# nghiant03/spine-vision

Hardware: AMD Instinct MI355X
Metric: images/sec training, ConvNeXt-base 512x512 loc, bs32, at 1/2/4/8 MI355X (higher is better)
Workload: dtype bf16; 1 GPU; CoordinateRegressor(convnext_base) localization train step fwd+bwd+allreduce+clip+AdamW; image_size=512, batch_per_gpu=32, global_batch=32, parallelism=dp1, hip_graph=False

## Files before the change

include/sv_kernels.h:

```cpp
#ifndef SV_KERNELS_H
#define SV_KERNELS_H

#include <stdint.h>

#ifdef __cplusplus
extern "C" {
#endif

typedef struct ihipStream_t* sv_stream_t;

typedef enum { SV_F32 = 0, SV_BF16 = 1 } sv_dtype;

typedef enum {
  SV_OK = 0,
  SV_ERR_INVALID_ARG = 1,
  SV_ERR_UNSUPPORTED = 2,
  SV_ERR_LAUNCH = 3
} sv_status;

int sv_version(void);
const char* sv_last_error_string(void);
const char* sv_build_target(void);

typedef struct sv_ctx sv_ctx;
typedef struct sv_ctx_info {
  int32_t device;
  int32_t compute_units;
  int32_t lds_bytes_per_wg;
  int32_t xcds;
  int32_t lds_raised_kernels;
  int32_t refs;
  char arch[32];
} sv_ctx_info;
int sv_ctx_create(int32_t device, sv_ctx** out);
int sv_ctx_destroy(sv_ctx* ctx);
int sv_ctx_get_info(const sv_ctx* ctx, sv_ctx_info* out);

int sv_stream_create_cu_reserved(int32_t device, const int32_t* reserved, int32_t n_reserved, sv_stream_t* out);

typedef enum {
  SV_EPI_STORE = 0,
  SV_EPI_BIAS_GELU2 = 1,
  SV_EPI_BIAS_GAMMA_RES = 2,
  SV_EPI_GELU_GRAD = 3,
  SV_EPI_SLAB = 4,
  SV_EPI_BIAS_GELU_DUAL = 5,
  SV_EPI_MUL_AUX = 6,
  SV_EPI_BIAS_GELU = 7,
  SV_EPI_STORE_STATS = 8,
  SV_EPI_STORE_BN_BWD = 9,
  SV_EPI_LN_BWD = 10
} sv_epilogue;

typedef struct {
  const float* mean;
  const float* rstd;
  const float* gamma;
  const float* beta;
} sv_bn_ref;

typedef struct {
  int32_t impl;
  int32_t grid_cap;
  int32_t wg_per_cu;
  int32_t priority;
} sv_gemm_policy;

typedef struct {
  int32_t M, N, K;
  const void* A; int32_t a_dtype; int32_t a_kmajor; int64_t lda;
  const void* B; int32_t b_dtype; int32_t b_kmajor; int64_t ldb;
  const float* a_scale_k;
  int32_t epilogue;
  void* C; int32_t c_dtype; int64_t ldc;
  void* C2; int32_t c2_dtype;
  const float* bias;
  const float* gamma;
  const void* aux; int32_t aux_dtype; int64_t ld_aux;
  int32_t split_k;
  int32_t compute;
  const sv_bn_ref* bn;
  sv_gemm_policy policy;
  float* fold_out; int64_t fold_ld; int32_t fold_accumulate; int32_t* fold_counters;
} sv_gemm_desc;

int sv_gemm(const sv_gemm_desc* d, sv_stream_t stream);
int sv_gemm_slab_finish(const float* slab, int32_t split, int32_t M, int32_t N, void* C, int32_t c_dtype, int64_t ldc,
                        int32_t accumulate, float* stats, sv_stream_t stream);
int sv_gemm_slab_finish_bn_bwd(const float* slab, int32_t split, int32_t M, int32_t N, void* C, const void* y,
                               const sv_bn_ref* bn, float* part, sv_stream_t stream);

int sv_mlp_fwd(const uint16_t* y, const uint16_t* w1, const float* b1, const uint16_t* w2, const float* b2,
               const float* gamma, const float* x, float* x_out, uint16_t* gelu_grad, uint16_t* gelu_out, int64_t M,
               int32_t C, sv_stream_t stream);

int sv_mlp_bwd_nparts(int64_t M, int32_t C);
int sv_mlp_bwd(const uint16_t* d, const uint16_t* w2t, const uint16_t* gelu_grad, const uint16_t* w1t, const uint16_t* z,
               const float* mean, const float* rstd, const float* lnw, uint16_t* dh, uint16_t* dz, float* ln_part,
               int64_t M, int32_t C, sv_stream_t stream);

int sv_layernorm_fwd(const void* x, int32_t x_dtype, const float* w, const float* b, void* y,
                     int32_t y_dtype, float* mean, float* rstd, int64_t rows, int32_t C, float eps,
                     sv_stream_t stream);
int sv_layernorm_bwd_nparts(int64_t rows, int32_t C);
int sv_layernorm_bwd(const void* dy, int32_t dy_dtype, const void* x, int32_t x_dtype, const float* mean,
                     const float* rstd, const float* w, void* dx, int32_t dx_dtype, int32_t accumulate,
                     float* dw_part, float* db_part, int64_t rows, int32_t C, sv_stream_t stream);

int sv_grn_nparts(int64_t HW, int32_t n);
int sv_grn_stats(const void* a, int32_t dtype, float* part, int32_t B, int64_t HW, int32_t n, sv_stream_t stream);
int sv_grn_finish(const float* part, int32_t nparts, const float* gamma, float* G, float* N, float* scale, float* D,
                  int32_t B, int32_t n, float eps, sv_stream_t stream);
int sv_grn_apply(const void* a, int32_t dtype, const float* scale, const float* beta, void* u, int32_t B, int64_t HW,
                 int32_t n, sv_stream_t stream);
int sv_grn_bwd_stats(const void* du, const void* a, int32_t dtype, float* s_part, float* d_part, int32_t B,
                     int64_t HW, int32_t n, sv_stream_t stream);
int sv_grn_bwd_finish(float* s_part, float* d_part, int32_t nparts, const float* gamma, const float* G,
                      const float* N, const float* D, float* k, float* dgamma, float* dbeta, int32_t accumulate,
                      int32_t B, int32_t n, sv_stream_t stream);
int sv_grn_bwd_apply(const void* du, const void* a, const void* gh, int32_t dtype, const float* scale, const float* k,
                     void* dh, int32_t B, int64_t HW, int32_t n, sv_stream_t stream);

int sv_dwconv7_ln_fwd(const void* x, int32_t x_dtype, const float* wdw, const float* bdw,
                      const float* lnw, const float* lnb, float eps, void* z, int32_t z_dtype, void* y,
                      int32_t y_dtype, float* mean, float* rstd, int32_t B, int32_t H, int32_t W,
                      int32_t C, sv_stream_t stream);
int sv_diag_group_sum(const float* in, float* xlane, float* shuffle, int64_t n, int32_t lanes, sv_stream_t stream);
int sv_dwconv7_ln_fused_ok(int32_t B, int32_t H, int32_t W, int32_t C, int32_t x_dtype, int32_t z_dtype,
                           int32_t y_dtype);
int sv_dwconv7_bwd_data(const void* dz, int32_t dz_dtype, const float* wdw, float* dx, uint16_t* dx_bf16,
                        int32_t accumulate, int32_t B, int32_t H, int32_t W, int32_t C, sv_stream_t stream);
int sv_dwconv7_bwd_weight_nparts(int32_t B, int32_t H, int32_t W, int32_t C);
int sv_dwconv7_bwd_weight(const void* dz, int32_t dz_dtype, const void* x, int32_t x_dtype, float* dw_part,
                          float* db_part, int32_t B, int32_t H, int32_t W, int32_t C,
                          sv_stream_t stream);

int sv_dwconv7_fwd_mfma(const void* x, int32_t x_dtype, const float* wdw, const float* bdw, uint16_t* z, int32_t B,
                        int32_t H, int32_t W, int32_t C, sv_stream_t stream);
int sv_dwconv7_bwd_data_mfma(const uint16_t* dz, const float* wdw, float* dx, uint16_t* dx_bf16, int32_t accumulate,
                             int32_t B, int32_t H, int32_t W, int32_t C, sv_stream_t stream);
int sv_dwconv7_bwd_weight_mfma_nparts(int32_t B, int32_t H, int32_t W, int32_t C);
int sv_dwconv7_bwd_weight_mfma(const uint16_t* dz, const void* x, int32_t x_dtype, float* dw_part, float* db_part,
                               int32_t B, int32_t H, int32_t W, int32_t C, sv_stream_t stream);

int sv_stem_patchify_ln_fwd(const float* img, const float* w, const float* b, const float* lnw,
                            const float* lnb, float eps, void* y, int32_t y_dtype, float* mean,
                            float* rstd, int32_t B, int32_t H, int32_t W, int32_t C,
                            sv_stream_t stream);
int sv_stem_patchify_ln_bwd_nparts(int32_t B, int32_t H, int32_t W, int32_t C);
int sv_stem_patchify_ln_bwd(const float* img, const float* w, const float* b, const float* lnw,
                            const float* mean, const float* rstd, const float* dy, float* dw_part,
                            float* db_part, float* dlnw_part, float* dlnb_part, int32_t B, int32_t H,
                            int32_t W, int32_t C, sv_stream_t stream);

typedef enum { SV_IMG_F32_NCHW = 0, SV_IMG_U8_GRAY = 1, SV_IMG_U8_HWC = 2  } sv_image_kind;
int sv_stem_patchify(const void* img, int32_t img_kind, const float* norm_mean, const float* norm_std,
                     uint16_t* patches, int32_t B, int32_t H, int32_t W, sv_stream_t stream);
int sv_stem_weight_pack(const float* w, uint16_t* wpack, int32_t C, sv_stream_t stream);
int sv_normalize_u8_gray(const uint8_t* img, const float* norm_mean, const float* norm_std, float* out,
                         int32_t B, int32_t H, int32_t W, sv_stream_t stream);

int sv_augment_u8(const uint8_t* in, uint8_t* out, int32_t B, int32_t H, int32_t W, int32_t C, const double* params,
                  int32_t* row_sums, sv_stream_t stream);

int sv_resize_u8(const uint8_t* src, const int64_t* desc, const int32_t* coef, int32_t B, int32_t H, int32_t W,
                 int32_t C, uint8_t* dst, sv_stream_t stream);

int sv_downsample_ln_patch2_fwd(const float* x, const float* lnw, const float* lnb, float eps,
                                void* patches, int32_t p_dtype, float* mean, float* rstd, int32_t B,
                                int32_t H, int32_t W, int32_t C, sv_stream_t stream);
int sv_downsample_ln_patch2_bwd_nparts(int32_t B, int32_t H, int32_t W, int32_t C);
int sv_downsample_ln_patch2_bwd(const float* dpatches, const float* x, const float* mean,
                                const float* rstd, const float* lnw, float* dx, uint16_t* dx_bf16, float* dlnw_part,
                                float* dlnb_part, int32_t B, int32_t H, int32_t W, int32_t C,
                                sv_stream_t stream);

int sv_pool_ln_fwd(const float* x, const float* lnw, const float* lnb, float eps, float* pooled,
                   float* feat, float* mean, float* rstd, int32_t B, int32_t HW, int32_t C,
                   sv_stream_t stream);
int sv_pool_ln_bwd(const float* dfeat, const float* pooled, const float* mean, const float* rstd,
                   const float* lnw, float* dx, uint16_t* dx_bf16, float* dlnw_part, float* dlnb_part, int32_t B,
                   int32_t HW, int32_t C, sv_stream_t stream);

#define SV_MAX_RED_SEGS 8
typedef struct {
  const float* part;
  float* out;
  int64_t n;
  int32_t P;
  int32_t accumulate;
} sv_red_seg;
int sv_reduce_partials_multi(const sv_red_seg* segs, int32_t nseg, float alpha, sv_stream_t stream);

int sv_reduce_partials_pair(const float* part_a, int64_t n_a, float* out_a, const float* part_b, int64_t n_b,
                            float* out_b, int32_t P, float alpha, int32_t accumulate, sv_stream_t stream);
int sv_reduce_partials(const float* part, int32_t P, int32_t group, int64_t n, float* out, float alpha,
                       int32_t accumulate, sv_stream_t stream);
int sv_reduce_partials_bf16(const uint16_t* part, int32_t P, int64_t n, float* out, float alpha, int32_t accumulate,
                            sv_stream_t stream);
int sv_colsum_nparts(int64_t rows, int32_t C);
int sv_colsum(const void* x, int32_t x_dtype, int64_t rows, int32_t C, float* part,
              sv_stream_t stream);
int sv_layerscale_wgrad_finish(const float* G, const float* cs, const float* W2, const float* gamma,
                               const float* b2, float* dW2, float* dgamma, float* db2, int32_t C,
                               int32_t K4, sv_stream_t stream);

int sv_layerscale_wgrad_reduce_ws(int32_t C, int32_t K4);
int sv_layerscale_wgrad_reduce(const float* slab, const float* cs_part, int32_t P, const float* W2,
                               const float* gamma, const float* b2, float* dW2, float* dgamma, float* db2,
                               float* ws, int32_t C, int32_t K4, sv_stream_t stream);
int sv_layerscale_wgrad_reduce_bf16(const uint16_t* slab, const float* cs_part, int32_t P, const float* W2,
                                    const float* gamma, const float* b2, float* dW2, float* dgamma, float* db2, int32_t C,
                                    int32_t K4, sv_stream_t stream);
int sv_layerscale_wgrad_fold_finish(const float* G, const float* cs_part, int32_t P, const float* W2, const float* gamma,
                                    const float* b2, float* dW2, float* dgamma, float* db2, int32_t C, int32_t K4,
                                    sv_stream_t stream);

int sv_sqnorm_nparts(int64_t n);
int sv_sqnorm_partial(const float* g, int64_t n, float* part, sv_stream_t stream);
int sv_clip_coef(const float* part, int32_t nparts, float max_norm, float* out, sv_stream_t stream);
int sv_adamw_flat(float* p, const float* g, float* m, float* v, uint16_t* p_bf16, int64_t n,
                  float lr, float beta1, float beta2, float eps, float weight_decay, int32_t step,
                  const float* grad_scale, sv_stream_t stream);
int sv_adamw_flat_dev(float* p, const float* g, float* m, float* v, uint16_t* p_bf16, int64_t n, float beta1,
                      float beta2, float eps, float weight_decay, const float* hyper, const float* grad_scale,
                      sv_stream_t stream);
int sv_transpose_scale_bf16(const float* W, const float* scale, uint16_t* out, int32_t rows, int32_t cols,
                            sv_stream_t stream);
int sv_scale_rows_bf16(const float* W, const float* scale, uint16_t* out, int32_t rows, int32_t cols,
                       sv_stream_t stream);
int sv_cast_f32_bf16(const float* x, uint16_t* y, int64_t n, sv_stream_t stream);

typedef struct sv_conv_shape {
  int32_t B, H, W, Cs;
  int32_t Cout;
  int32_t KH, KW, stride, pad;
  int32_t Cin;
} sv_conv_shape;
int sv_conv_weight_pack(const float* w, void* wp, int32_t dtype, const sv_conv_shape* s, sv_stream_t stream);
// ... 259 lines not shown
```

spine-vision_amd/backbone/convnext.py:

```python

from __future__ import annotations

import os
from dataclasses import dataclass, field
from typing import Callable

import torch
import torch.nn as nn

from .. import kernels as K
from .. import native as nv
from ._explicit import ExplicitBackward

CONVNEXT_CFGS = {
    "convnext_tiny": ((3, 3, 9, 3), (96, 192, 384, 768)),
    "convnext_small": ((3, 3, 27, 3), (96, 192, 384, 768)),
    "convnext_base": ((3, 3, 27, 3), (128, 256, 512, 1024)),
    "convnext_large": ((3, 3, 27, 3), (192, 384, 768, 1536)),
    "convnextv2_base": ((3, 3, 27, 3), (128, 256, 512, 1024)),
    "convnextv2_large": ((3, 3, 27, 3), (192, 384, 768, 1536)),
}


def _comm_cap(device, reserve: int) -> int:
# ... 28 lines not shown


class _GrnMlp(nn.Module):
    def __init__(self, dim: int, hidden: int) -> None:
        super().__init__()
        self.fc1 = nn.Linear(dim, hidden)
        self.grn = _Grn(hidden)
        self.fc2 = nn.Linear(hidden, dim)


class ConvNeXtV2Block(nn.Module):

    def __init__(self, dim: int) -> None:
        super().__init__()
        self.conv_dw = nn.Conv2d(dim, dim, kernel_size=7, padding=3, groups=dim, bias=True)
        self.norm = nn.LayerNorm(dim, eps=1e-6)
        self.mlp = _GrnMlp(dim, 4 * dim)


class ConvNeXtStage(nn.Module):
    def __init__(self, in_chs: int, out_chs: int, depth: int, downsample: bool, block=ConvNeXtBlock) -> None:
        super().__init__()
        if downsample:
            self.downsample = nn.Sequential(nn.LayerNorm(in_chs, eps=1e-6), nn.Conv2d(in_chs, out_chs, 2, stride=2))
        else:
            self.downsample = nn.Identity()
        self.blocks = nn.Sequential(*[block(out_chs) for _ in range(depth)])


class _Head(nn.Module):
    def __init__(self, dim: int) -> None:
        super().__init__()
        self.norm = nn.LayerNorm(dim, eps=1e-6)


@dataclass
class _Tape:

    img: torch.Tensor
    stem: tuple = ()
    stages: list = field(default_factory=list)
    pool: tuple = ()
    out_shape: tuple = ()
    wcache: dict = field(default_factory=dict)
    w2g: dict = field(default_factory=dict)
    wt: dict = field(default_factory=dict)
    w2g_ready: object = None


class _ConvNeXtFn(torch.autograd.Function):
    @staticmethod
    def forward(ctx, x, anchor, model):
        feat, tape = model._forward_impl(x, save=True)
        ctx.model = model
        ctx.tape = tape
        return feat

    @staticmethod
    def backward(ctx, dfeat):
        ctx.model._backward_impl(ctx.tape, dfeat)
        ctx.tape = None
        return None, None, None


_TAIL_MAIN = int(os.environ.get("SV_TAIL_MAIN", "0"))


class _WgradSchedule:

    def __init__(self, model, main, side, lean: bool, pol) -> None:
        self.model, self.main, self.side, self.lean, self.pol = model, main, side, lean, pol
        cap = pol.grid_cap
        if model.side_grid_cap is not None:
            cap = min(model.side_grid_cap, cap) if cap > 0 else model.side_grid_cap
        self.spol = nv.policy(impl=model.side_impl, grid_cap=cap, wg_per_cu=pol.wg_per_cu, priority=model.side_prio)
        self.queue: list = []
        self.pending: list = []
        self.tail: list = []

    def _run(self, jobs, pol) -> None:
        for job, ready in jobs:
            job(pol)
            if ready:
                self.model._ready(ready)

    def submit(self, job, operands, ready=None) -> None:
        if self.lean:
            self.queue.append((job, ready))
        elif self.side is None:
            self._run([(job, ready)], self.pol)
        else:
            self.side.wait_event(self.main.record_event())
            for t_ in operands:
                t_.record_stream(self.side)
            with torch.cuda.stream(self.side):
                self._run([(job, ready)], self.spol)

    def handoff(self) -> None:
        if self.lean:
            nv.handoff(self.main, self.side)

    def flush(self, tail: bool) -> None:
        if not self.lean:
            return
        queue, self.queue = self.queue, []
        n = 1 if tail else len(queue)
        with torch.cuda.stream(self.side):
            self._run(queue[:n], self.spol)
            self.pending.append((self.side.record_event(), queue))
        self.tail += queue[n:]

    def run_tail(self) -> None:
        self._run(self.tail, self.pol)
        self.tail.clear()


class ConvNeXtHip(ExplicitBackward, nn.Module):
    def __init__(self, depths=(3, 3, 27, 3), dims=(128, 256, 512, 1024), ls_init_value: float = 1e-6,
                 precision: str = "bf16", use_grn: bool = False) -> None:
        super().__init__()
        if precision not in ("bf16", "fp32"):
            raise ValueError(f"precision must be 'bf16' or 'fp32', got {precision!r}")
        self.depths, self.dims = tuple(depths), tuple(dims)
        self.precision = precision
        self.use_grn = bool(use_grn)
        self.stem = nn.Sequential(nn.Conv2d(3, dims[0], kernel_size=4, stride=4), nn.LayerNorm(dims[0], eps=1e-6))
        stages = []
        prev = dims[0]
        for i, (d, c) in enumerate(zip(depths, dims)):
            stages.append(ConvNeXtStage(prev, c, d, downsample=i > 0,
                                        block=ConvNeXtV2Block if self.use_grn else ConvNeXtBlock))
            prev = c
        self.stages = nn.Sequential(*stages)
        if self.use_grn:
            self.register_buffer("ls_ones", torch.ones(max(dims)), persistent=False)
        self.norm_pre = nn.Identity()
        self.head = _Head(prev)
        self.num_features = self.head_hidden_size = prev
        self.grad_ready_hook: Callable[[list], None] | None = None
        self._shadow: dict[int, torch.Tensor] | None = None
        self.overlap_wgrad = os.environ.get("SV_SIDE_STREAM", "1") != "0"
        self.side_wg_per_cu = 1
        self.lean_sync = os.environ.get("SV_LEAN_SYNC", "1") != "0"
        self._side: dict = {}
        self.graph_safe = False
        self.comm_reserve_cus = 0
        self.comm_cu_mask = False
        self.merge_folds = os.environ.get("SV_MERGED_FOLDS", "1") != "0"
        cap = os.environ.get("SV_SIDE_GRID_CAP")
        self.side_grid_cap: int | None = int(cap) if cap else None
        self.side_impl = int(os.environ.get("SV_WGRAD_IMPL", "0"))
        self.main_bwd_cap = int(os.environ.get("SV_MAIN_BWD_CAP", "0"))
        self.wgrad_target = int(os.environ.get("SV_CNX_WGRAD_WGS", "256"))
        self.side_prio = int(os.environ.get("SV_SIDE_PRIO", "1"))
        self.fused_mlp = os.environ.get("SV_FUSED_MLP", "1") != "0"
        self.fused_mlp_c = tuple(int(c) for c in os.environ.get("SV_FUSED_MLP_C", "128,192,256").split(",") if c)
        self.fused_mlp_bwd = os.environ.get("SV_FUSED_MLP_BWD", "1") != "0"
        self.param_gate = None
        self._init_weights()

    def param_gate_groups(self) -> list[nn.Module]:
        return [self.stem, *self.stages, self.head]

    def _init_weights(self) -> None:
        for m in self.modules():
            if isinstance(m, (nn.Conv2d, nn.Linear)):
                nn.init.trunc_normal_(m.weight, std=0.02)
                if m.bias is not None:
                    nn.init.zeros_(m.bias)

    @property
    def compute_bf16(self) -> bool:
        return self.precision == "bf16"

    @property
    def act_dtype(self) -> torch.dtype:
        return torch.bfloat16 if self.compute_bf16 else torch.float32

    def set_weight_shadow(self, shadow: dict[int, torch.Tensor] | None) -> None:
        self._shadow = shadow

    def gemm_weight_params(self) -> list[nn.Parameter]:
        ps = [self.stem[0].weight]
        for st in self.stages:
            if not isinstance(st.downsample, nn.Identity):
                ps.append(st.downsample[1].weight)
            for blk in st.blocks:
                ps += [blk.mlp.fc1.weight, blk.mlp.fc2.weight]
        return ps

    def _w(self, p: torch.Tensor, cache: dict) -> torch.Tensor:
        if not self.compute_bf16:
            return p.detach()
        if self._shadow is not None and id(p) in self._shadow:
            return self._shadow[id(p)]
        k = id(p)
        if k not in cache:
            cache[k] = K.cast_bf16(p.detach().contiguous())
        return cache[k]

    def forward(self, x: torch.Tensor) -> torch.Tensor:
        if not x.is_cuda:
            raise RuntimeError("ConvNeXtHip runs on the MI355X kernel library only (got a CPU tensor)")
        if x.dtype == torch.uint8:
            x = x.contiguous() if self.compute_bf16 else K.normalize_u8_gray(x.contiguous())
        else:
            x = x.float().contiguous()
        need_grad = torch.is_grad_enabled() and any(p.requires_grad for p in self.parameters())
        if need_grad:
            anchor = torch.zeros((), device=x.device, requires_grad=True)
            return _ConvNeXtFn.apply(x, anchor, self)
        feat, _ = self._forward_impl(x, save=False)
        return feat

    def forward_features(self, x: torch.Tensor) -> torch.Tensor:
        return self.forward(x)

    @torch.no_grad()
    def _forward_impl(self, img: torch.Tensor, save: bool):
        bf = self.compute_bf16
        act = self.act_dtype
        tape = _Tape(img=img) if save else None
        cache: dict = tape.wcache if save else {}
        stem_conv, stem_ln = self.stem[0], self.stem[1]
        gate = self.param_gate
        if gate is not None:
            gate.wait(self.stem)
        if save and bf and self.overlap_wgrad and not self.use_grn:
            main = torch.cuda.current_stream()
            side = self._side_stream(main.device)
            blocks = [blk for st in self.stages for blk in st.blocks]
            fused_b = {id(blk) for blk in blocks if self._fused_bwd(blk)}
            for blk in blocks:
                if id(blk) in fused_b:
                    w1, w2 = blk.mlp.fc1.weight, blk.mlp.fc2.weight
                    tape.wt[id(blk)] = (torch.empty(w2.shape[1], w2.shape[0], device=img.device, dtype=torch.bfloat16),
                                        torch.empty(w1.shape[1], w1.shape[0], device=img.device, dtype=torch.bfloat16))
                else:
                    tape.w2g[id(blk)] = torch.empty(blk.mlp.fc2.weight.shape, device=img.device, dtype=torch.bfloat16)
            side.wait_event(main.record_event())
            if gate is not None:
                gate.wait_all(side)
            with torch.cuda.stream(side):
                for blk in blocks:
                    if id(blk) in fused_b:
                        w2t, w1t = tape.wt[id(blk)]
                        K.transpose_scale_bf16(blk.mlp.fc2.weight.detach(), blk.gamma.detach(), out=w2t)
                        K.transpose_scale_bf16(blk.mlp.fc1.weight.detach(), None, out=w1t)
                    else:
                        K.scale_rows_bf16(blk.mlp.fc2.weight.detach(), blk.gamma.detach(), out=tape.w2g[id(blk)])
            tape.w2g_ready = side.record_event()
        if bf:
            B, H0, W0 = img.shape[0], img.shape[-2], img.shape[-1]
            C0 = stem_conv.weight.shape[0]
            patches = K.stem_patchify(img)
            z0 = torch.empty(patches.shape[0], C0, device=img.device, dtype=act)
            K.linear_fwd(patches, K.stem_weight_pack(stem_conv.weight.detach()), out=z0, bias=stem_conv.bias,
                         compute_bf16=True)
            x2d, s_mean, s_rstd = K.layernorm_fwd(z0, stem_ln.weight, stem_ln.bias, out_dtype=torch.float32)
            x = x2d.view(B, H0 // 4, W0 // 4, C0)
            if save:
                tape.stem = (patches, z0, s_mean, s_rstd)
        else:
            x, s_mean, s_rstd = K.stem_fwd(img, stem_conv.weight, stem_conv.bias, stem_ln.weight, stem_ln.bias)
            if save:
                tape.stem = (s_mean, s_rstd)
        for st in self.stages:
            if gate is not None:
                gate.wait(st)
            ds_saved = None
            if not isinstance(st.downsample, nn.Identity):
                ln, conv = st.downsample[0], st.downsample[1]
                B, H, W, C = x.shape
                patches, d_mean, d_rstd = K.downsample_fwd(x, ln.weight, ln.bias, act_dtype=act)
                Cout = conv.weight.shape[0]
                wds = self._w(conv.weight, cache).reshape(Cout, 4 * C)
                xn = torch.empty(B, H // 2, W // 2, Cout, device=x.device, dtype=torch.float32)
                K.linear_fwd(patches, wds, out=xn.view(-1, Cout), bias=conv.bias, compute_bf16=bf)
                if save:
                    ds_saved = (x, patches, d_mean, d_rstd)
                x = xn
            blocks_saved = []
            for blk in st.blocks:
                B, H, W, C = x.shape
                M = B * H * W
                z, y, mean, rstd = K.dwconv7_ln_fwd(x, blk.conv_dw.weight, blk.conv_dw.bias, blk.norm.weight,
                                                    blk.norm.bias, act_dtype=act, save_z=save)
                w1 = self._w(blk.mlp.fc1.weight, cache)
                w2 = self._w(blk.mlp.fc2.weight, cache)
                if bf and self.fused_mlp and not self.use_grn and C in K.MLP_FUSED_C and C in self.fused_mlp_c:
                    xo = torch.empty(B, H, W, C, device=x.device, dtype=torch.float32)
                    gh = torch.empty(M, 4 * C, device=x.device, dtype=act) if save else None
                    a = torch.empty(M, 4 * C, device=x.device, dtype=act) if save else None
                    K.mlp_fwd(y, w1, blk.mlp.fc1.bias, w2, blk.mlp.fc2.bias, blk.gamma, x.view(M, C), out=xo.view(M, C),
                              gelu_grad=gh, gelu_out=a)
                    if save:
                        blocks_saved.append((x, z, y, mean, rstd, gh, a, None))
                    x = xo
                    continue
                a = torch.empty(M, 4 * C, device=x.device, dtype=act)
                if save:
                    gh = torch.empty(M, 4 * C, device=x.device, dtype=act)
                    K.linear_fwd(y, w1, out=gh, out2=a, bias=blk.mlp.fc1.bias, epilogue=nv.SV_EPI_BIAS_GELU_DUAL,
                                 compute_bf16=bf)
                else:
                    gh = None
                    K.linear_fwd(y, w1, out=a, bias=blk.mlp.fc1.bias, epilogue=nv.SV_EPI_BIAS_GELU,
                                 compute_bf16=bf)
                xo = torch.empty(B, H, W, C, device=x.device, dtype=torch.float32)
                grn_saved = None
                if self.use_grn:
                    grn = blk.mlp.grn
                    u, gst = K.grn_fwd(a, B, grn.weight, grn.bias, inplace=not save)
                    grn_saved = (u, gst)
                    K.linear_fwd(u, w2, out=xo.view(M, C), bias=blk.mlp.fc2.bias, gamma=self.ls_ones[:C],
                                 residual=x.view(M, C), epilogue=nv.SV_EPI_BIAS_GAMMA_RES, compute_bf16=bf)
                else:
                    K.linear_fwd(a, w2, out=xo.view(M, C), bias=blk.mlp.fc2.bias, gamma=blk.gamma,
                                 residual=x.view(M, C), epilogue=nv.SV_EPI_BIAS_GAMMA_RES, compute_bf16=bf)
                if save:
                    blocks_saved.append((x, z, y, mean, rstd, gh, a, grn_saved))
                x = xo
            if save:
                tape.stages.append((ds_saved, blocks_saved))
        if gate is not None:
            gate.wait_all()
        feat, pooled, p_mean, p_rstd = K.pool_ln_fwd(x, self.head.norm.weight, self.head.norm.bias)
        if save:
            tape.pool = (pooled, p_mean, p_rstd)
            tape.out_shape = tuple(x.shape)
            if tape.w2g_ready is not None:
                torch.cuda.current_stream().wait_event(tape.w2g_ready)
                tape.w2g_ready = None
        return feat, tape

    def _fused_bwd(self, blk) -> bool:
        return (self.fused_mlp_bwd and not self.use_grn and self.compute_bf16 and self.overlap_wgrad and self.lean_sync
                and blk.conv_dw.weight.shape[0] in K.MLP_BWD_FUSED_C)

    def _fc2_params(self, blk) -> list:
        if self.use_grn:
            return [blk.mlp.fc2.weight, blk.mlp.fc2.bias, blk.mlp.grn.weight, blk.mlp.grn.bias]
        return [blk.mlp.fc2.weight, blk.mlp.fc2.bias, blk.gamma]

    @staticmethod
    def _rest_params(blk) -> list:
        return [blk.conv_dw.weight, blk.conv_dw.bias, blk.norm.weight, blk.norm.bias, blk.mlp.fc1.weight,
                blk.mlp.fc1.bias]

    def _grn_dgrad(self, blk, dsrc, a, gh, grn_saved, dh, cache, pol) -> None:
        bf = self.compute_bf16
        w2 = self._w(blk.mlp.fc2.weight, cache) if bf else blk.mlp.fc2.weight.detach()
        K.linear_dgrad(dsrc, w2, out=dh, compute_bf16=bf, policy=pol)
        grn, gst = blk.mlp.grn, grn_saved[1]
        K.grn_bwd(dh, a, gh, gst[0].shape[0], grn.weight, gst, dgamma=self._grad(grn.weight),
                  dbeta=self._grad(grn.bias))

    def _block_backward(self, blk, saved, d, db, cache, tape, sched: _WgradSchedule, tail: bool = False):
        bf, act, g = self.compute_bf16, self.act_dtype, self._grad
        main, side, pol = sched.main, sched.side, sched.pol
        x, z, y, mean, rstd, gh, a, grn_saved = saved
        B, H, W, C = x.shape
        M = B * H * W
        fc1, fc2 = blk.mlp.fc1, blk.mlp.fc2
        dsrc = db.view(M, C) if bf else d.view(M, C)
        u = grn_saved[0] if self.use_grn else a
        fc2_ps, rest_ps = self._fc2_params(blk), self._rest_params(blk)
        folds: list | None = [] if self.merge_folds else None

        def fc2_wgrad(policy):
            if self.use_grn:
                K.linear_wgrad(dsrc, u, out=g(fc2.weight), accumulate=True, bias_out=g(fc2.bias), compute_bf16=bf,
                               policy=policy, wgrad_target=self.wgrad_target)
            else:
                K.layerscale_wgrad(dsrc, a, fc2.weight.detach(), blk.gamma.detach(), fc2.bias.detach(),
                                   dw2=g(fc2.weight), dgamma=g(blk.gamma), db2=g(fc2.bias), compute_bf16=bf,
                                   policy=policy, wgrad_target=self.wgrad_target)

        def fc1_wgrad(policy):
            K.linear_wgrad(dh, y, out=g(fc1.weight), accumulate=True, bias_out=g(fc1.bias), compute_bf16=bf,
                           defer=folds, policy=policy, wgrad_target=self.wgrad_target)

        def rest_wgrad(policy):
            ln_finish(record=not sched.lean, defer=folds)
            K.dwconv7_bwd_weight(dz4, x, dw=g(blk.conv_dw.weight), db=g(blk.conv_dw.bias), defer=folds)
            if folds is not None:
                K.reduce_multi(folds)

        sched.submit(fc2_wgrad, (dsrc, u), ready=fc2_ps if tail else None)
        ev_w2 = side.record_event() if side is not None and not bf else None
        dh = torch.empty(M, 4 * C, device=d.device, dtype=act)
        wt = tape.wt.pop(id(blk), None)
        if wt is not None:
            dz = torch.empty(M, C, device=d.device, dtype=torch.bfloat16)
            part, P = K.mlp_bwd(dsrc, wt[0], gh, wt[1], z.view(M, C), mean, rstd, blk.norm.weight, dh=dh, dz=dz)
            dw_ln, db_ln = g(blk.norm.weight), g(blk.norm.bias)

            def ln_finish(record: bool = True, defer: list | None = None):
                if defer is not None:
                    defer += [(part[0], dw_ln, P, True), (part[1], db_ln, P, True)]
                else:
                    K.reduce_pair(part[0], dw_ln, part[1], db_ln, P)
        elif self.use_grn:
            self._grn_dgrad(blk, dsrc, a, gh, grn_saved, dh, cache, pol)
        elif bf:
            w2g = tape.w2g.pop(id(blk), None)
            if w2g is None:
                w2g = K.scale_rows_bf16(fc2.weight.detach(), blk.gamma.detach())
            K.linear_dgrad(dsrc, w2g, out=dh, epilogue=nv.SV_EPI_MUL_AUX, aux=gh, compute_bf16=True, policy=pol)
        else:
            K.linear_dgrad(dsrc, fc2.weight.detach(), out=dh, epilogue=nv.SV_EPI_MUL_AUX, a_scale_k=blk.gamma, aux=gh,
                           compute_bf16=False, policy=pol)
        sched.submit(fc1_wgrad, (dh, y))
        if wt is None:
            w1 = self._w(fc1.weight, cache)
            fused = K.linear_dgrad_ln(dh, w1, z.view(M, C), mean, rstd, blk.norm.weight, dw=g(blk.norm.weight),
                                      db=g(blk.norm.bias), policy=pol) if bf else None
            if fused is not None:
                dz, ln_finish = fused
            else:
                dy = torch.empty(M, C, device=d.device, dtype=act)
                K.linear_dgrad(dh, w1, out=dy, compute_bf16=bf, policy=pol)
                dz, ln_finish = K.layernorm_bwd(dy, z.view(M, C), mean, rstd, blk.norm.weight, dw=g(blk.norm.weight),
                                                db=g(blk.norm.bias), out_dtype=act, defer_reduce=True)
        dz4 = dz.view(B, H, W, C)
        sched.submit(rest_wgrad, (dz, x), ready=rest_ps if tail else rest_ps + fc2_ps)
        sched.handoff()
        if side is not None and bf:
            db = torch.empty_like(db)
        elif side is not None:
            main.wait_event(ev_w2)
        K.dwconv7_bwd_data(dz4, blk.conv_dw.weight, d, accumulate=True, dx_bf16=db)
        sched.flush(tail)
        return d, db

    @torch.no_grad()
    def _backward_impl(self, tape: _Tape, dfeat: torch.Tensor) -> None:
        bf = self.compute_bf16
        cache: dict = tape.wcache
        g = self._grad
        hn = self.head.norm
        main = torch.cuda.current_stream()
        side = self._side_stream(main.device) if self.overlap_wgrad else None
        comm_cap = _comm_cap(main.device, self.comm_reserve_cus)
        if self.main_bwd_cap > 0:
            comm_cap = min(comm_cap, self.main_bwd_cap) if comm_cap > 0 else self.main_bwd_cap
        pol = nv.policy(grid_cap=comm_cap, wg_per_cu=self.side_wg_per_cu if side is not None else 0)
        sched = _WgradSchedule(self, main, side, side is not None and bf and self.lean_sync, pol)
        d, db = K.pool_ln_bwd(dfeat.float(), *tape.pool, hn.weight, tape.out_shape, dlnw=g(hn.weight),
                              dlnb=g(hn.bias), with_bf16=bf)
        if tape.w2g_ready is not None:
            main.wait_event(tape.w2g_ready)
        self._ready([hn.weight, hn.bias])
        for st, (ds_saved, blocks_saved) in zip(reversed(list(self.stages)), reversed(tape.stages)):
            for bi in range(len(blocks_saved) - 1, -1, -1):
                blk, saved = st.blocks[bi], blocks_saved[bi]
                blocks_saved[bi] = None
                tail = sched.lean and _TAIL_MAIN > 0 and st is self.stages[0] and bi == 0
                d, db = self._block_backward(blk, saved, d, db, cache, tape, sched, tail=tail)
                self._release_side(main, sched.pending)
                if _TAIL_MAIN == 2:
                    sched.run_tail()
            if ds_saved is not None:
                x_prev, patches, d_mean, d_rstd = ds_saved
                ln, conv = st.downsample[0], st.downsample[1]
                B, H, W, C = x_prev.shape
                Cout = conv.weight.shape[0]
                Mo = B * (H // 2) * (W // 2)
                dsrc = db.view(Mo, Cout) if bf else d.view(Mo, Cout)
                wds = self._w(conv.weight, cache).reshape(Cout, 4 * C)
                dpatch = torch.empty(Mo, 4 * C, device=d.device, dtype=torch.float32)
                K.linear_dgrad(dsrc, wds, out=dpatch, compute_bf16=bf, policy=pol)
                K.linear_wgrad(dsrc, patches, out=g(conv.weight), accumulate=True, bias_out=g(conv.bias),
                               compute_bf16=bf, policy=pol)
                d, db = K.downsample_bwd(dpatch, x_prev, d_mean, d_rstd, ln.weight, dlnw=g(ln.weight),
                                         dlnb=g(ln.bias), with_bf16=bf)
                self._ready([ln.weight, ln.bias, conv.weight, conv.bias])
        conv, ln = self.stem[0], self.stem[1]
        if bf:
            patches, z0, s_mean, s_rstd = tape.stem
            C0 = conv.weight.shape[0]
            dz0 = K.layernorm_bwd(d.view(-1, C0), z0, s_mean, s_rstd, ln.weight, dw=g(ln.weight), db=g(ln.bias),
                                  out_dtype=torch.bfloat16)
            K.linear_wgrad(dz0, patches, out=g(conv.weight).view(C0, 48), accumulate=True, bias_out=g(conv.bias),
                           compute_bf16=True, cols=48, policy=pol)
        else:
            s_mean, s_rstd = tape.stem
            K.stem_bwd(tape.img, conv.weight, conv.bias, ln.weight, s_mean, s_rstd, d, dw=g(conv.weight),
                       db=g(conv.bias), dlnw=g(ln.weight), dlnb=g(ln.bias))
        sched.run_tail()
        if side is not None:
            main.wait_stream(side)
            sched.pending.clear()
        self._ready([conv.weight, conv.bias, ln.weight, ln.bias])

    _RELEASE_BATCH = int(os.environ.get("SV_RELEASE_BATCH", "4"))

    @classmethod
    def _release_side(cls, main, pending: list) -> None:
        while pending and pending[0][0].query():
            pending.pop(0)
        if len(pending) >= 2 * cls._RELEASE_BATCH:
            main.wait_event(pending[cls._RELEASE_BATCH - 1][0])
            del pending[:cls._RELEASE_BATCH]


def create_convnext(name: str, precision: str = "bf16") -> ConvNeXtHip:
    key = name.split(".")[0]
    if key not in CONVNEXT_CFGS:
        raise ValueError(f"unsupported ConvNeXt variant {name!r}")
    depths, dims = CONVNEXT_CFGS[key]
    return ConvNeXtHip(depths, dims, precision=precision, use_grn=key.startswith("convnextv2"))
```

spine-vision_amd/csrc/gemm.hip:

```cpp
#include "common.h"
#include "gemm_common.h"
#include "mfma_v1.h"

#include <stdlib.h>

namespace sv {


template <bool BF16, typename T, bool KMAJ>
struct Stage {
  static constexpr int EPC = BF16 ? 8 : 4;
  static constexpr int CHUNKS = BM * BKT / EPC;
  static constexpr int PER_THREAD = CHUNKS / kGemmThreads;
  uint4 r[PER_THREAD];

  __device__ __forceinline__ void load(const T* __restrict__ p, int64_t ld, int row0, int k0, int R, int K,
                                       const float* __restrict__ scale) {
#pragma unroll
    for (int s = 0; s < PER_THREAD; ++s) {
      const int q = threadIdx.x + kGemmThreads * s;
      int row, kk;
      if (KMAJ) {
        constexpr int CPR = BKT / EPC;
        row = q / CPR;
// ... 190 lines not shown
  }

  if (do_cs && threadIdx.x < BM && m0 + (int)threadIdx.x < e.M) colsum[(size_t)split * e.M + m0 + threadIdx.x] = csum;

  wave_tile_epilogue(acc, reinterpret_cast<float*>(smem) + wid * 16 * EPI_LD, m0 + wm * 64, n0 + wn * 64, e, split);
}

template <bool BF16, typename TA, typename TB, bool AK, bool BKM>
static int launch(const sv_gemm_desc* d, hipStream_t s) {
  const int tilesM = ceil_div(d->M, BM), tilesN = ceil_div(d->N, BN);
  int split = d->epilogue == SV_EPI_SLAB ? (d->split_k < 1 ? 1 : d->split_k) : 1;
  int kper = ceil_div(ceil_div(d->K, split), BKT) * BKT;
  EpiArgs e{d->M, d->N, d->epilogue, d->C, d->c_dtype, d->ldc, d->C2, d->c2_dtype, d->bias, d->gamma,
            d->aux, d->aux_dtype, d->ld_aux};
  constexpr size_t main_lds = 2 * (size_t)(Img<BF16, AK>::BYTES + Img<BF16, BKM>::BYTES);
  constexpr size_t epi_lds = 4 * 16 * EPI_LD * sizeof(float);
  constexpr size_t lds = main_lds > epi_lds ? main_lds : epi_lds;
  dim3 grid(tilesM * tilesN, 1, split);
  if (const int rc_ = ensure_lds_attr(reinterpret_cast<const void*>(&gemm_kernel<BF16, TA, TB, AK, BKM>), (int)lds, s)) return rc_;
  gemm_kernel<BF16, TA, TB, AK, BKM><<<grid, kGemmThreads, lds, s>>>(
      reinterpret_cast<const TA*>(d->A), d->lda, reinterpret_cast<const TB*>(d->B), d->ldb, d->a_scale_k, d->K,
      kper, tilesM, tilesN, e, d->epilogue == SV_EPI_SLAB ? reinterpret_cast<float*>(d->C2) : nullptr);
  return check_launch("sv_gemm");
}

template <bool BF16, typename TA, typename TB>
static int launch_layout(const sv_gemm_desc* d, hipStream_t s) {
  if (d->a_kmajor && d->b_kmajor) return launch<BF16, TA, TB, true, true>(d, s);
  if (d->a_kmajor && !d->b_kmajor) return launch<BF16, TA, TB, true, false>(d, s);
  if (!d->a_kmajor && d->b_kmajor) return launch<BF16, TA, TB, false, true>(d, s);
  return launch<BF16, TA, TB, false, false>(d, s);
}

static bool al16(const void* p) { return ((uintptr_t)p & 15) == 0; }

}

using namespace sv;

extern "C" int sv_gemm(const sv_gemm_desc* d, sv_stream_t stream) {
  SV_REQUIRE(d, "sv_gemm: null descriptor");
  SV_REQUIRE(d->A && d->B && d->C, "sv_gemm: null operand");
  SV_REQUIRE(d->M >= 0 && d->N >= 0 && d->K >= 0, "sv_gemm: negative size");
  SV_REQUIRE(d->epilogue >= SV_EPI_STORE && d->epilogue <= SV_EPI_LN_BWD, "sv_gemm: bad epilogue %d", d->epilogue);
  SV_REQUIRE(d->policy.impl == 0 || d->policy.impl == 2 || d->policy.impl == 3 || d->policy.impl == 8 || d->policy.impl == 9,
             "sv_gemm: policy.impl must be 0, 2, 3, 8 or 9 (got %d)", d->policy.impl);
  SV_REQUIRE(d->policy.grid_cap >= 0 && d->policy.wg_per_cu >= 0 && d->policy.wg_per_cu <= 2 &&
                 (d->policy.priority == 0 || d->policy.priority == 1),
             "sv_gemm: bad policy (grid_cap >= 0, wg_per_cu 0..2, priority 0/1)");
  if (d->M == 0 || d->N == 0) return SV_OK;
  const bool bf = d->compute == SV_BF16;
  SV_REQUIRE(bf || d->compute == SV_F32, "sv_gemm: bad compute type");
  SV_REQUIRE(bf || (d->a_dtype == SV_F32 && d->b_dtype == SV_F32), "sv_gemm: f32 compute needs f32 operands");
  const int vec = bf ? 8 : 4;
  SV_REQUIRE((d->a_kmajor ? d->K : d->M) % vec == 0, "sv_gemm: A contiguous dim not a multiple of %d", vec);
  SV_REQUIRE((d->b_kmajor ? d->K : d->N) % vec == 0, "sv_gemm: B contiguous dim not a multiple of %d", vec);
  SV_REQUIRE(d->lda % vec == 0 && d->ldb % vec == 0, "sv_gemm: lda/ldb must be multiples of %d", vec);
  SV_REQUIRE(al16(d->A) && al16(d->B) && al16(d->C), "sv_gemm: operands must be 16-byte aligned");
  SV_REQUIRE(d->N % 4 == 0, "sv_gemm: N must be a multiple of 4");
  if (d->epilogue == SV_EPI_SLAB) {
    SV_REQUIRE(d->c_dtype == SV_F32 || (bf && d->c_dtype == SV_BF16 && !d->fold_out && d->N % 8 == 0),
               "sv_gemm: slab epilogue writes f32 (bf16 slabs: bf16 compute, N %% 8 == 0, no in-kernel fold)");
    SV_REQUIRE(!d->C2 || d->c2_dtype == SV_F32, "sv_gemm: slab colsum output is f32");
  } else {
    SV_REQUIRE(d->ldc % 4 == 0, "sv_gemm: ldc must be a multiple of 4");
  }
  if (d->epilogue == SV_EPI_BIAS_GELU2 || d->epilogue == SV_EPI_BIAS_GELU_DUAL)
    SV_REQUIRE(d->C2 && al16(d->C2), "sv_gemm: GELU epilogue needs an aligned C2");
  if (d->epilogue == SV_EPI_BIAS_GAMMA_RES) SV_REQUIRE(d->gamma && d->aux, "sv_gemm: gamma/residual missing");
  if (d->epilogue == SV_EPI_STORE_STATS)
    SV_REQUIRE(bf && d->C2 && al16(d->C2) && d->N % 8 == 0, "sv_gemm: STORE_STATS needs bf16, an aligned C2, N %% 8 == 0");
  if (d->epilogue == SV_EPI_GELU_GRAD || d->epilogue == SV_EPI_MUL_AUX) SV_REQUIRE(d->aux, "sv_gemm: aux missing");
  if (d->epilogue == SV_EPI_STORE_BN_BWD)
    SV_REQUIRE(bf && d->c_dtype == SV_BF16 && d->C2 && d->N % 8 == 0 && d->aux && d->aux_dtype == SV_BF16 && !d->bias &&
                   d->bn && d->bn->mean && d->bn->rstd && d->bn->gamma && d->bn->beta,
               "sv_gemm: STORE_BN_BWD needs bf16 C and aux, C2, N %% 8 == 0, no bias and the bn parameters");
  if (d->epilogue == SV_EPI_LN_BWD)
    SV_REQUIRE(bf && d->c_dtype == SV_BF16 && d->C2 && al16(d->C2) && d->aux && d->aux_dtype == SV_BF16 && d->bn &&
                   d->bn->mean && d->bn->rstd && d->bn->gamma && d->fold_out && d->fold_counters && al16(d->fold_out),
               "sv_gemm: LN_BWD needs bf16 C and aux (z), C2, the bn mean / rstd / gamma and the exchange workspace");
  if (d->aux) SV_REQUIRE(d->ld_aux % 4 == 0 && al16(d->aux), "sv_gemm: aux must be aligned");
  if (d->fold_out && d->epilogue != SV_EPI_LN_BWD)
    SV_REQUIRE(d->epilogue == SV_EPI_SLAB && bf && d->fold_counters && d->fold_ld == d->N && al16(d->fold_out),
               "sv_gemm: fold_out needs SV_EPI_SLAB (bf16), fold_counters, fold_ld == N and a 16-byte aligned output");
  if (d->a_scale_k) SV_REQUIRE(al16(d->a_scale_k), "sv_gemm: a_scale_k must be aligned");
  hipStream_t s = (hipStream_t)stream;
  if (!bf) return launch_layout<false, float, float>(d, s);
  const int impl = d->policy.impl;
  const int wpc = d->policy.wg_per_cu;
  if (d->epilogue == SV_EPI_STORE_BN_BWD) {
    const int rc = launch_gemm3(d, s);
    SV_REQUIRE(rc != SV_ERR_UNSUPPORTED, "sv_gemm: STORE_BN_BWD needs K %% 32 == 0, bf16 operands, k-major A, m-major B");
    return rc;
  }
  if (d->epilogue == SV_EPI_LN_BWD) return launch_gemm9(d, s);
  if (d->epilogue == SV_EPI_STORE_STATS) {
    const long t9 = (long)ceil_div(d->M, 256) * ceil_div(d->N, 256);
    if ((impl == 0 || impl == 9) && d->N >= 256 && t9 >= 256 && d->a_kmajor) {
      const int rc9 = launch_gemm9(d, s);
      if (rc9 != SV_ERR_UNSUPPORTED) return rc9;
    }
    const int rc = launch_gemm3(d, s);
    SV_REQUIRE(rc != SV_ERR_UNSUPPORTED, "sv_gemm: STORE_STATS needs K %% 32 == 0 and bf16 operands");
    return rc;
  }
  {
    const bool heavy_epi = d->epilogue == SV_EPI_BIAS_GELU2 || d->epilogue == SV_EPI_BIAS_GELU_DUAL ||
                           d->epilogue == SV_EPI_GELU_GRAD || d->epilogue == SV_EPI_MUL_AUX ||
                           d->epilogue == SV_EPI_BIAS_GELU;
    const long tiles8 = (long)ceil_div(d->M, 256) * ceil_div(d->N, 256);
    const bool v8_shape = tiles8 >= 256 && (d->epilogue == SV_EPI_BIAS_GELU_DUAL || d->epilogue == SV_EPI_BIAS_GELU ||
                                            ((d->epilogue == SV_EPI_BIAS_GAMMA_RES) && d->K >= 2048));
    const int split9 = d->epilogue == SV_EPI_SLAB ? (d->split_k < 1 ? 1 : d->split_k) : 1;
    const bool v9_slab = d->epilogue == SV_EPI_SLAB && (d->M < d->N ? d->M : d->N) >= 128 &&
                         (d->M > d->N ? d->M : d->N) >= 256 && tiles8 * split9 >= 128;
    const bool v9_shape = v9_slab || (d->epilogue != SV_EPI_SLAB && d->epilogue != SV_EPI_BIAS_GELU2 && d->N >= 256 &&
                                      tiles8 >= 256);
    const bool v9_pick = impl == 0 && v9_shape;
    int rc = SV_ERR_UNSUPPORTED;
    if (d->epilogue == SV_EPI_SLAB && d->c_dtype == SV_BF16) {
      rc = launch_gemm9(d, s);
      SV_REQUIRE(rc != SV_ERR_UNSUPPORTED, "sv_gemm: bf16 slabs need the v9 weight-gradient layout (N/M-major A)");
      return rc;
    }
    if (impl == 9 || v9_pick) rc = launch_gemm9(d, s);
    if (rc != SV_ERR_UNSUPPORTED) return rc;
    if (d->fold_out) {
      sv_gemm_desc dd = *d;
      dd.fold_out = nullptr;
      dd.fold_counters = nullptr;
      if (int r = sv_gemm(&dd, stream)) return r;
      const int split = d->split_k < 1 ? 1 : d->split_k;
      return sv_reduce_partials(reinterpret_cast<const float*>(d->C), split, split, (int64_t)d->M * d->N, d->fold_out,
                                1.0f, d->fold_accumulate, stream);
    }
    if ((impl == 0 || impl == 9) && !wpc && v8_shape) rc = launch_gemm8(d, s);
    else if (impl == 8) rc = launch_gemm8(d, s);
    else if (impl == 2) rc = launch_gemm2(d, s);
    else if (impl == 3) rc = launch_gemm3(d, s);
    else if (d->epilogue == SV_EPI_SLAB) rc = launch_gemm3(d, s, wpc ? "32x3" : "32x4");
    else if (heavy_epi || (d->epilogue == SV_EPI_STORE && d->K <= 2048)) rc = launch_gemm3(d, s);
    else if (wpc) rc = launch_gemm3(d, s);
    else rc = launch_gemm2(d, s);
    if (rc != SV_ERR_UNSUPPORTED) return rc;
  }
  const bool a32 = d->a_dtype == SV_F32, b32 = d->b_dtype == SV_F32;
  SV_REQUIRE((a32 || d->a_dtype == SV_BF16) && (b32 || d->b_dtype == SV_BF16), "sv_gemm: bad operand dtype");
  if (!a32 && !b32) return launch_layout<true, uint16_t, uint16_t>(d, s);
  if (a32 && !b32) return launch_layout<true, float, uint16_t>(d, s);
  if (!a32 && b32) return launch_layout<true, uint16_t, float>(d, s);
  return launch_layout<true, float, float>(d, s);
}

namespace sv {
namespace {
constexpr int SF_THREADS = 256;
__global__ void __launch_bounds__(SF_THREADS) slab_finish_kernel(const float* __restrict__ slab, int split, int M, int N,
                                                                 void* __restrict__ C, int c_dtype, int64_t ldc,
                                                                 int accumulate, float* __restrict__ stats) {
  const int q = threadIdx.x & 15, ph = threadIdx.x >> 4;
  const int n = blockIdx.x * 64 + q * 4, m0 = blockIdx.y * 64;
  const size_t sstride = (size_t)M * N;
  float4 s1 = make_float4(0.f, 0.f, 0.f, 0.f), s2 = s1;
  if (n < N) {
#pragma unroll
    for (int i = 0; i < 4; ++i) {
      const int m = m0 + ph + 16 * i;
      if (m >= M) break;
      const float* p = slab + (size_t)m * N + n;
      float4 v = *reinterpret_cast<const float4*>(p);
      for (int sl = 1; sl < split; ++sl) {
        const float4 w = *reinterpret_cast<const float4*>(p + sl * sstride);
        v.x += w.x; v.y += w.y; v.z += w.z; v.w += w.w;
      }
      const size_t ci = (size_t)m * ldc + n;
      if (c_dtype == SV_F32) {
        float4* cp = reinterpret_cast<float4*>(reinterpret_cast<float*>(C) + ci);
        if (accumulate) {
          const float4 o = *cp;
          v.x += o.x; v.y += o.y; v.z += o.z; v.w += o.w;
        }
        *cp = v;
      } else {
        uint2* cp = reinterpret_cast<uint2*>(reinterpret_cast<uint16_t*>(C) + ci);
        if (accumulate) {
          const uint2 o = *cp;
          v.x += __uint_as_float(o.x << 16); v.y += __uint_as_float(o.x & 0xffff0000u);
          v.z += __uint_as_float(o.y << 16); v.w += __uint_as_float(o.y & 0xffff0000u);
        }
        const uint2 u = make_uint2(pack2bf(v.x, v.y), pack2bf(v.z, v.w));
        *cp = u;
        v = make_float4(__uint_as_float(u.x << 16), __uint_as_float(u.x & 0xffff0000u), __uint_as_float(u.y << 16),
                        __uint_as_float(u.y & 0xffff0000u));
      }
      if (stats) {
        s1.x += v.x; s1.y += v.y; s1.z += v.z; s1.w += v.w;
        s2.x = fmaf(v.x, v.x, s2.x); s2.y = fmaf(v.y, v.y, s2.y); s2.z = fmaf(v.z, v.z, s2.z); s2.w = fmaf(v.w, v.w, s2.w);
      }
    }
  }
  if (!stats) return;
  __shared__ float4 red[2][SF_THREADS];
  red[0][threadIdx.x] = s1;
  red[1][threadIdx.x] = s2;
  __syncthreads();
  if (ph == 0 && n < N) {
    for (int k = 1; k < 16; ++k) {
      const float4 a = red[0][k * 16 + q], b = red[1][k * 16 + q];
      s1.x += a.x; s1.y += a.y; s1.z += a.z; s1.w += a.w;
      s2.x += b.x; s2.y += b.y; s2.z += b.z; s2.w += b.w;
    }
    float* o = stats + (size_t)blockIdx.y * 2 * N;
    *reinterpret_cast<float4*>(o + n) = s1;
    *reinterpret_cast<float4*>(o + N + n) = s2;
  }
}

__global__ void __launch_bounds__(SF_THREADS) slab_finish_bnb_kernel(const float* __restrict__ slab, int split, int M,
                                                                     int N, uint16_t* __restrict__ C,
                                                                     const uint16_t* __restrict__ y, sv_bn_ref bn,
                                                                     float* __restrict__ part) {
  const int q = threadIdx.x & 15, ph = threadIdx.x >> 4;
  const int n = blockIdx.x * 64 + q * 4, m0 = blockIdx.y * 64;
  const size_t sstride = (size_t)M * N;
  float s1[4] = {0.f, 0.f, 0.f, 0.f}, s2[4] = {0.f, 0.f, 0.f, 0.f};
  if (n < N) {
    const float4 mu4 = *reinterpret_cast<const float4*>(bn.mean + n), rs4 = *reinterpret_cast<const float4*>(bn.rstd + n);
    const float4 ga4 = *reinterpret_cast<const float4*>(bn.gamma + n), be4 = *reinterpret_cast<const float4*>(bn.beta + n);
    const float mu[4] = {mu4.x, mu4.y, mu4.z, mu4.w}, rs[4] = {rs4.x, rs4.y, rs4.z, rs4.w};
    const float ga[4] = {ga4.x, ga4.y, ga4.z, ga4.w}, be[4] = {be4.x, be4.y, be4.z, be4.w};
#pragma unroll
    for (int i = 0; i < 4; ++i) {
      const int m = m0 + ph + 16 * i;
      if (m >= M) break;
      const float* p = slab + (size_t)m * N + n;
      float4 v = *reinterpret_cast<const float4*>(p);
      for (int sl = 1; sl < split; ++sl) {
        const float4 w = *reinterpret_cast<const float4*>(p + sl * sstride);
        v.x += w.x; v.y += w.y; v.z += w.z; v.w += w.w;
      }
      const size_t ci = (size_t)m * N + n;
      const uint2 u = make_uint2(pack2bf(v.x, v.y), pack2bf(v.z, v.w));
      *reinterpret_cast<uint2*>(C + ci) = u;
      const uint2 yu = *reinterpret_cast<const uint2*>(y + ci);
      const float o[4] = {__uint_as_float(u.x << 16), __uint_as_float(u.x & 0xffff0000u), __uint_as_float(u.y << 16),
                          __uint_as_float(u.y & 0xffff0000u)};
      const float yv[4] = {__uint_as_float(yu.x << 16), __uint_as_float(yu.x & 0xffff0000u),
                           __uint_as_float(yu.y << 16), __uint_as_float(yu.y & 0xffff0000u)};
#pragma unroll
      for (int j = 0; j < 4; ++j) {
        const float g = fmaf(ga[j] * rs[j], yv[j] - mu[j], be[j]) > 0.f ? o[j] : 0.f;
        s1[j] += g;
        s2[j] = fmaf(g, (yv[j] - mu[j]) * rs[j], s2[j]);
      }
    }
  }
  __shared__ float4 red[2][SF_THREADS];
  red[0][threadIdx.x] = make_float4(s1[0], s1[1], s1[2], s1[3]);
  red[1][threadIdx.x] = make_float4(s2[0], s2[1], s2[2], s2[3]);
  __syncthreads();
  if (ph == 0 && n < N) {
    float4 a1 = red[0][q], a2 = red[1][q];
    for (int k = 1; k < 16; ++k) {
      const float4 a = red[0][k * 16 + q], b = red[1][k * 16 + q];
      a1.x += a.x; a1.y += a.y; a1.z += a.z; a1.w += a.w;
      a2.x += b.x; a2.y += b.y; a2.z += b.z; a2.w += b.w;
    }
    float* o = part + (size_t)blockIdx.y * 2 * N;
    *reinterpret_cast<float4*>(o + n) = a1;
    *reinterpret_cast<float4*>(o + N + n) = a2;
  }
}
}
}

extern "C" int sv_gemm_slab_finish_bn_bwd(const float* slab, int32_t split, int32_t M, int32_t N, void* C, const void* y,
                                          const sv_bn_ref* bn, float* part, sv_stream_t stream) {
  SV_REQUIRE(slab && C && y && bn && part && bn->mean && bn->rstd && bn->gamma && bn->beta,
             "sv_gemm_slab_finish_bn_bwd: null pointer");
  SV_REQUIRE(split >= 1 && M >= 0 && N >= 0 && N % 4 == 0, "sv_gemm_slab_finish_bn_bwd: bad sizes (N multiple of 4)");
  SV_REQUIRE(al16(slab) && al16(C) && al16(y) && al16(part) && al16(bn->mean) && al16(bn->rstd) && al16(bn->gamma) &&
                 al16(bn->beta),
             "sv_gemm_slab_finish_bn_bwd: operands must be 16-byte aligned");
  if (M == 0 || N == 0) return SV_OK;
  const dim3 grid((unsigned)ceil_div(N, 64), (unsigned)ceil_div(M, 64));
  sv::slab_finish_bnb_kernel<<<grid, sv::SF_THREADS, 0, (hipStream_t)stream>>>(
      slab, split, M, N, reinterpret_cast<uint16_t*>(C), reinterpret_cast<const uint16_t*>(y), *bn, part);
  return check_launch("sv_gemm_slab_finish_bn_bwd");
}

extern "C" int sv_gemm_slab_finish(const float* slab, int32_t split, int32_t M, int32_t N, void* C, int32_t c_dtype,
                                   int64_t ldc, int32_t accumulate, float* stats, sv_stream_t stream) {
  SV_REQUIRE(slab && C, "sv_gemm_slab_finish: null pointer");
  SV_REQUIRE(split >= 1 && M >= 0 && N >= 0 && N % 4 == 0 && ldc % 4 == 0 && ldc >= N,
             "sv_gemm_slab_finish: bad sizes (N, ldc multiples of 4)");
  SV_REQUIRE(c_dtype == SV_F32 || c_dtype == SV_BF16, "sv_gemm_slab_finish: bad C dtype");
  SV_REQUIRE(!stats || c_dtype == SV_BF16, "sv_gemm_slab_finish: statistics are of bf16 outputs");
  SV_REQUIRE(al16(slab) && al16(C) && (!stats || al16(stats)), "sv_gemm_slab_finish: operands must be 16-byte aligned");
  if (M == 0 || N == 0) return SV_OK;
  const dim3 grid((unsigned)ceil_div(N, 64), (unsigned)ceil_div(M, 64));
  sv::slab_finish_kernel<<<grid, sv::SF_THREADS, 0, (hipStream_t)stream>>>(slab, split, M, N, C, c_dtype, ldc,
                                                                           accumulate, stats);
  return check_launch("sv_gemm_slab_finish");
}
```

spine-vision_amd/csrc/gemm9.hip:

```cpp
#include "common.h"
#include "gemm_common.h"

#include <stdlib.h>

namespace sv {
namespace g9 {

#ifdef SV_CLOCK_STAMPS
__device__ unsigned long long g_stamps[1024][4];
__device__ __forceinline__ void stamp(int slot) {
  const unsigned long long t = __builtin_amdgcn_s_memtime(), r = __builtin_amdgcn_s_memrealtime();
  if (threadIdx.x == 0 && blockIdx.x < 1024) {
    volatile unsigned long long* p = g_stamps[blockIdx.x];
    p[2 * slot] = t;
    p[2 * slot + 1] = r;
  }
}
#else
__device__ __forceinline__ void stamp(int) {}
#endif

#ifndef SV_G9_PRIO
#define SV_G9_PRIO 0
#endif

constexpr int BM = 256, BN = 256, BK = 64, THREADS = 512, NW = 8;
constexpr int FM = 8, FN = 4;
constexpr int A_BYTES = BM * BK * 2, B_BYTES = BN * BK * 2, BUF_BYTES = A_BYTES + B_BYTES;
template <bool AK>
constexpr int lds_bytes() { return AK ? 2 * BUF_BYTES : 3 * A_BYTES + 2 * B_BYTES; }
template <bool AK>
__device__ __forceinline__ int a_off(int g) { return AK ? (g & 1) * BUF_BYTES : (g % 3) * A_BYTES; }
template <bool AK>
__device__ __forceinline__ int b_off(int g) { return AK ? (g & 1) * BUF_BYTES + A_BYTES : 3 * A_BYTES + (g & 1) * B_BYTES; }
constexpr uint32_t OOB = 0x80000000u;

typedef __attribute__((address_space(3))) void lds_void;
typedef __attribute__((address_space(3))) s16x4 lds_s16x4;
typedef unsigned int u32x4 __attribute__((ext_vector_type(4)));
typedef unsigned int u32x2 __attribute__((ext_vector_type(2)));

__device__ __forceinline__ int kswz(int row) { return (row >> 1) & 7; }
__device__ __forceinline__ int mswz(int r) { return ((r & 3) << 1) ^ (((r >> 3) & 1) << 3); }
__device__ __forceinline__ int perm8(int rho) {
  return (rho & ~31) | (((rho & 15) >> 2) << 3) | (((rho >> 4) & 1) << 2) | (rho & 3);
}

template <int CPOL = 0>
__device__ __forceinline__ void dma(__amdgpu_buffer_rsrc_t r, uint32_t voff, uint32_t soff, char* dst) {
  __builtin_amdgcn_raw_ptr_buffer_load_lds(r, (lds_void*)dst, 16, voff, soff, 0, CPOL);
}
#ifndef SV_G9_AUXBF_CPOL
#define SV_G9_AUXBF_CPOL 0
#endif
#ifndef SV_G9_SLAB_B_CPOL
#define SV_G9_SLAB_B_CPOL 0
#endif
template <bool PERM>
__device__ __forceinline__ uint32_t vbase_k(int64_t ld, int row0, int wid) {
  const int lane = threadIdx.x & 63;
  const int row = 8 * wid + (lane >> 3), ch = lane & 7;
  return (uint32_t)(((int64_t)(row0 + (PERM ? perm8(row) : row)) * ld + ((ch ^ kswz(row)) << 3)) * 2);
}
__device__ __forceinline__ uint32_t vbase_m(int64_t ld, int col0, int wid) {
  const int lane = threadIdx.x & 63;
  const int krow = 2 * wid + (lane >> 5), ch = lane & 31;
  return (uint32_t)(((int64_t)krow * ld + col0 + ((ch ^ mswz(krow)) << 3)) * 2);
}

__device__ __forceinline__ bf16x8 frag_k(const char* __restrict__ region, int base, int kh) {
  const int l = threadIdx.x & 63;
  const int row = base + (l & 15), ch = kh * 4 + (l >> 4);
  return *reinterpret_cast<const bf16x8*>(region + row * 128 + ((ch ^ kswz(row)) << 4));
}
__device__ __forceinline__ bf16x8 frag_tr(const char* __restrict__ region, int ch, int hf, int kh) {
  const int l = threadIdx.x & 63;
  const int g = l >> 4, q = (l >> 2) & 3;
  const int r0 = kh * 32 + 8 * g + q, r1 = r0 + 4;
  const char* a0 = region + r0 * 512 + ((ch ^ mswz(r0)) << 4) + hf * 8;
  const char* a1 = region + r1 * 512 + ((ch ^ mswz(r1)) << 4) + hf * 8;
  s16x4 lo = __builtin_amdgcn_ds_read_tr16_b64_v4i16((lds_s16x4*)a0);
  s16x4 hi = __builtin_amdgcn_ds_read_tr16_b64_v4i16((lds_s16x4*)a1);
  typedef short s16x8 __attribute__((ext_vector_type(8)));
  s16x8 v = {lo[0], lo[1], lo[2], lo[3], hi[0], hi[1], hi[2], hi[3]};
  return __builtin_bit_cast(bf16x8, v);
}
__device__ __forceinline__ bf16x8 frag_m(const char* __restrict__ region, int base, int kh) {
  const int p = threadIdx.x & 3;
  return frag_tr(region, (base >> 3) + (p >> 1), p & 1, kh);
}

template <int N>
__device__ __forceinline__ void vm_wait() {
  asm volatile("s_waitcnt vmcnt(%0)" ::"n"(N) : "memory");
}
__device__ __forceinline__ void lgkm0() { asm volatile("s_waitcnt lgkmcnt(0)" ::: "memory"); }
__device__ __forceinline__ void bar() {
  asm volatile("" ::: "memory");
  __builtin_amdgcn_s_barrier();
  asm volatile("" ::: "memory");
}

struct Geo {
  int m0, n0, kbeg, split;
};

struct Ext {
  uint32_t c, c2, aux, a, b;
};

struct Fold {
  float* out;
  int64_t ld;
  int acc;
  int* cnt;
};
constexpr int kFoldNone = 0, kFoldLast = 1, kFoldSpread = 2;
constexpr int kSC1 = 16;
#ifndef SV_G9_GRAD_CPOL
#define SV_G9_GRAD_CPOL 2
#endif
#ifndef SV_GELU_PK
#define SV_GELU_PK 1
#endif
#ifndef SV_G9_C2_CPOL
#define SV_G9_C2_CPOL 0
#endif

__device__ __forceinline__ __amdgpu_buffer_rsrc_t rsrc(const void* p, uint32_t bytes) {
  return __builtin_amdgcn_make_buffer_rsrc(const_cast<void*>(p), (short)0, (int)bytes, 0x00020000);
}

__device__ __forceinline__ float4 lds_f4(const float* p) {
  typedef float f32x4_t __attribute__((ext_vector_type(4)));
  f32x4_t v;
  const uint32_t a = (uint32_t)(size_t)(const __attribute__((address_space(3))) char*)(p);
  asm volatile("ds_read_b128 %0, %1\n\ts_waitcnt lgkmcnt(0)" : "=v"(v) : "v"(a) : "memory");
  return make_float4(v.x, v.y, v.z, v.w);
}

__device__ __forceinline__ u32x4 pack8(const float (&v)[8]) {
  return u32x4{pack2bf(v[0], v[1]), pack2bf(v[2], v[3]), pack2bf(v[4], v[5]), pack2bf(v[6], v[7])};
}

template <int EPI, bool P8>
struct EpiCount {
  static constexpr int CH = P8 ? 2 : 4;
  static constexpr int OUTS = (EPI == SV_EPI_BIAS_GELU_DUAL) ? 2 : 1;
  static constexpr int AUX = (EPI == SV_EPI_MUL_AUX || EPI == SV_EPI_GELU_GRAD) ? CH
                             : EPI == SV_EPI_BIAS_GAMMA_RES ? (P8 ? 2 * CH : CH)
                                                            : 0;
#ifdef SV_DIAG_NOSTORE
  static constexpr int E = 0;
#else
  static constexpr int E = FM * (CH * OUTS + AUX);
#endif
};

template <int EPI, bool P8, bool AK, int FOLD = kFoldNone>
__device__ __forceinline__ void epilogue(const f32x4 (&acc)[FM][FN], const EpiArgs& e, const Ext& x, int m_w, int n_w,
                                         int split, const float* lbias) {
#ifdef SV_DIAG_NOSTORE
  float sink = 0.f;
#pragma unroll
  for (int i = 0; i < FM; ++i)
#pragma unroll
    for (int j = 0; j < FN; ++j) sink += acc[i][j][0] + acc[i][j][1] + acc[i][j][2] + acc[i][j][3];
  asm volatile("" ::"v"(sink));
  return;
#endif
  constexpr int CH = P8 ? 2 : 4, CW = P8 ? 8 : 4;
  const int l = threadIdx.x & 63, ml = l & 15, gq = l >> 4;
  int n[CH];
  bool okn[CH];
#pragma unroll
  for (int c = 0; c < CH; ++c) {
    n[c] = n_w + (P8 ? 32 * c + 8 * gq : 16 * c + 4 * gq);
    okn[c] = n[c] < e.N;
  }
  const bool slab = EPI == SV_EPI_SLAB;
  const bool has_bias = !slab && EPI != SV_EPI_GELU_GRAD && EPI != SV_EPI_MUL_AUX;
  float bias[CH][CW], gam[CH][CW];
#pragma unroll
  for (int c = 0; c < CH; ++c)
#pragma unroll
    for (int w = 0; w < CW; ++w) bias[c][w] = 0.f, gam[c][w] = 1.f;
  const int wcol = n_w & 255;
  auto ld_vec = [&](const float* g, int lo, int c, float (&dst)[CH][CW]) {
#pragma unroll
    for (int w = 0; w < CW; w += 4) {
      float4 b;
      if (lbias) b = lds_f4(lbias + lo + wcol + (n[c] - n_w) + w);
      else b = okn[c] ? *reinterpret_cast<const float4*>(g + n[c] + w) : make_float4(0.f, 0.f, 0.f, 0.f);
      dst[c][w] = b.x, dst[c][w + 1] = b.y, dst[c][w + 2] = b.z, dst[c][w + 3] = b.w;
    }
  };
  if (has_bias && e.bias) {
#pragma unroll
    for (int c = 0; c < CH; ++c) ld_vec(e.bias, 0, c, bias);
  }
  if (EPI == SV_EPI_BIAS_GAMMA_RES && e.gamma) {
#pragma unroll
    for (int c = 0; c < CH; ++c) ld_vec(e.gamma, 256, c, gam);
  }
  const int64_t ldc = slab ? e.N : e.ldc;
  const char* cbase = reinterpret_cast<const char*>(e.C);
  if (slab) cbase += (size_t)split * e.M * e.N * (P8 ? 2 : 4);
  const auto rc = rsrc(cbase, x.c);
  const auto rc2 = rsrc(e.C2 ? e.C2 : e.C, x.c2);
  constexpr int CS = P8 ? 2 : 4;
  constexpr bool AUXBF = EPI == SV_EPI_MUL_AUX || EPI == SV_EPI_GELU_GRAD;
  constexpr bool AUXF = EPI == SV_EPI_BIAS_GAMMA_RES;
  const auto ra = rsrc(e.aux ? e.aux : e.C, x.aux);
#ifndef SV_G9_AUXB
#define SV_G9_AUXB 1
#endif
  constexpr int HALF = AUXF ? (SV_G9_AUXB && AK ? FM / 2 : FM / 4) : (AUXBF && SV_G9_AUXB ? FM : FM / 2);
  constexpr bool kStats = EPI == SV_EPI_STORE_STATS;
  static_assert(!kStats || (P8 && HALF == 4), "statistics need bf16 output and 64-row batches");
  float st1[kStats ? CH : 1][kStats ? 8 : 1], st2[kStats ? CH : 1][kStats ? 8 : 1];
#pragma unroll
  for (int hb = 0; hb < FM / HALF; ++hb) {
    if constexpr (kStats) {
#pragma unroll
      for (int c = 0; c < CH; ++c)
#pragma unroll
        for (int w = 0; w < 8; ++w) st1[c][w] = st2[c][w] = 0.f;
    }
    u32x4 raw[HALF][CH][AUXF && P8 ? 2 : 1];
    if constexpr (AUXBF || AUXF) {
#pragma unroll
      for (int ii = 0; ii < HALF; ++ii) {
        const int m = m_w + 16 * (hb * HALF + ii) + ml;
#pragma unroll
        for (int c = 0; c < CH; ++c) {
          const uint32_t base = okn[c] && m < e.M ? (uint32_t)((m * e.ld_aux + n[c]) * (AUXF ? 4 : 2)) : OOB;
          if constexpr (AUXBF && P8) {
            raw[ii][c][0] = __builtin_amdgcn_raw_buffer_load_b128(ra, base, 0, SV_G9_AUXBF_CPOL);
          } else if constexpr (AUXBF) {
            const u32x2 t = __builtin_amdgcn_raw_buffer_load_b64(ra, base, 0, SV_G9_AUXBF_CPOL);
            raw[ii][c][0] = u32x4{t.x, t.y, 0u, 0u};
          } else if constexpr (P8) {
            raw[ii][c][0] = __builtin_amdgcn_raw_buffer_load_b128(ra, base, 0, 0);
            raw[ii][c][AUXF && P8 ? 1 : 0] = __builtin_amdgcn_raw_buffer_load_b128(ra, base + 16, 0, 0);
          } else {
            raw[ii][c][0] = __builtin_amdgcn_raw_buffer_load_b128(ra, base, 0, 0);
          }
        }
      }
    }
#pragma unroll
    for (int ii = 0; ii < HALF; ++ii) {
      const int i = hb * HALF + ii;
      const int m = m_w + 16 * i + ml;
#pragma unroll
      for (int c = 0; c < CH; ++c) {
        float v[CW];
        if constexpr (P8) {
#pragma unroll
          for (int r = 0; r < 4; ++r) v[r] = acc[i][2 * c][r], v[4 + r] = acc[i][2 * c + 1][r];
        } else {
// ... 242 lines not shown
  const int P = (e.M + 127) / 128, prow = m_w / 128;
  float s1[FM], s2[FM];
#pragma unroll
  for (int i = 0; i < FM; ++i) s1[i] = s2[i] = 0.f;
#pragma nounroll
  for (int c = 0; c < CH; ++c) {
    float lw[8], pw[8], pb[8];
    lw_of(c, lw);
#pragma unroll
    for (int w = 0; w < 8; ++w) pw[w] = pb[w] = 0.f;
#pragma unroll
    for (int hb = 0; hb < 2; ++hb) {
      asm volatile("" ::: "memory");
      u32x4 zr[FM / 2];
#pragma unroll
      for (int ii = 0; ii < FM / 2; ++ii) zr[ii] = __builtin_amdgcn_raw_buffer_load_b128(rz, zoff(hb * FM / 2 + ii, c), 0, 0);
#pragma unroll
      for (int ii = 0; ii < FM / 2; ++ii) {
        const int i = hb * FM / 2 + ii;
        float d[8], xh[8];
        dy_back(i, c, d);
        z_of(zr[ii], i, xh);
#pragma unroll
        for (int w = 0; w < 8; ++w) {
          const float g = d[w] * lw[w];
          s1[i] += g;
          s2[i] += g * xh[w];
          pw[w] += d[w] * xh[w];
          pb[w] += d[w];
        }
      }
    }
#pragma unroll
    for (int w = 0; w < 8; ++w)
#pragma unroll
      for (int sh = 1; sh < 16; sh <<= 1) {
        pw[w] += __shfl_xor(pw[w], sh);
        pb[w] += __shfl_xor(pb[w], sh);
      }
    if (ml == 0 && m_w < e.M) {
      float* C2 = reinterpret_cast<float*>(e.C2);
      const int n = n_w + 32 * c + 8 * gq;
      float4* qw = reinterpret_cast<float4*>(C2 + ((size_t)prow) * e.N + n);
      float4* qb = reinterpret_cast<float4*>(C2 + ((size_t)P + prow) * e.N + n);
      qw[0] = make_float4(pw[0], pw[1], pw[2], pw[3]);
      qw[1] = make_float4(pw[4], pw[5], pw[6], pw[7]);
      qb[0] = make_float4(pb[0], pb[1], pb[2], pb[3]);
      qb[1] = make_float4(pb[4], pb[5], pb[6], pb[7]);
    }
  }
  __builtin_amdgcn_sched_barrier(0);
#pragma unroll
  for (int i = 0; i < FM; ++i) {
    s1[i] += __shfl_xor(s1[i], 16);
    s1[i] += __shfl_xor(s1[i], 32);
    s2[i] += __shfl_xor(s2[i], 16);
    s2[i] += __shfl_xor(s2[i], 32);
  }
  if (gq == 0) {
#pragma unroll
    for (int i = 0; i < FM; ++i) {
      float* q = lred + ((wm * 4 + wn) * 128 + 16 * i + ml) * 2;
      q[0] = s1[i], q[1] = s2[i];
    }
  }
  lgkm0();
  bar();
  const int tile_m = m0 / BM, half = n0 / BN;
  const uint32_t xbytes = (uint32_t)(((size_t)((e.M + BM - 1) / BM) * tilesN * BM * 2) * 4);
  const auto rx = rsrc(f.out, xbytes);
  auto xoff = [&](int h, int row) { return (uint32_t)((((size_t)tile_m * tilesN + h) * BM + row) * 8); };
  if (wn == 0 && gq == 0) {
#pragma unroll
    for (int i = 0; i < FM; ++i) {
      const int row = 16 * i + ml;
      float t1 = 0.f, t2 = 0.f;
#pragma unroll
      for (int w4 = 0; w4 < 4; ++w4) {
        const float* q = lred + ((wm * 4 + w4) * 128 + row) * 2;
        t1 += q[0];
        t2 += q[1];
      }
      __builtin_amdgcn_raw_buffer_store_b64(u32x2{__float_as_uint(t1), __float_as_uint(t2)}, rx,
                                            xoff(half, 128 * wm + row), 0, kSC1);
    }
  }
  vm_wait<0>();
  bar();
  int* arrive = f.cnt + 2 * tile_m;
  int* depart = arrive + 1;
  __shared__ int s_ok;
  if (threadIdx.x == 0) {
    __hip_atomic_fetch_add(arrive, 1, __ATOMIC_RELAXED, __HIP_MEMORY_SCOPE_AGENT);
    int ok = 1;
    for (int spin = 0; __hip_atomic_load(arrive, __ATOMIC_RELAXED, __HIP_MEMORY_SCOPE_AGENT) < tilesN; ++spin) {
      if (spin > (1 << 26)) {
        ok = 0;
        break;
      }
      __builtin_amdgcn_s_sleep(2);
    }
    s_ok = ok;
  }
  bar();
  const bool ok = s_ok != 0;
  float S1[FM], S2[FM];
#pragma unroll
  for (int i = 0; i < FM; ++i) S1[i] = S2[i] = 0.f;
  for (int h = 0; h < tilesN; ++h) {
#pragma unroll
    for (int i = 0; i < FM; ++i) {
      const u32x2 v = __builtin_amdgcn_raw_buffer_load_b64(rx, xoff(h, 128 * wm + 16 * i + ml), 0, kSC1);
      S1[i] += __uint_as_float(v.x);
      S2[i] += __uint_as_float(v.y);
    }
  }
  vm_wait<0>();
  bar();
  if (threadIdx.x == 0 && __hip_atomic_fetch_add(depart, 1, __ATOMIC_RELAXED, __HIP_MEMORY_SCOPE_AGENT) == tilesN - 1) {
    __hip_atomic_store(arrive, 0, __ATOMIC_RELAXED, __HIP_MEMORY_SCOPE_AGENT);
    __hip_atomic_store(depart, 0, __ATOMIC_RELAXED, __HIP_MEMORY_SCOPE_AGENT);
  }
  const auto rc = rsrc(e.C, x.c);
#pragma unroll
  for (int hb = 0; hb < 2; ++hb) {
    asm volatile("" ::: "memory");
    u32x4 zr[FM / 2][CH];
#pragma unroll
    for (int ii = 0; ii < FM / 2; ++ii)
#pragma unroll
      for (int c = 0; c < CH; ++c) zr[ii][c] = __builtin_amdgcn_raw_buffer_load_b128(rz, zoff(hb * FM / 2 + ii, c), 0, 0);
#pragma unroll
    for (int ii = 0; ii < FM / 2; ++ii) {
      const int i = hb * FM / 2 + ii;
      const int m = m_w + 16 * i + ml;
      const float a1 = ok ? S1[i] * invC : __builtin_nanf(""), a2 = S2[i] * invC;
#pragma unroll
      for (int c = 0; c < CH; ++c) {
        float d[8], xh[8], o[8], lw[8];
        lw_of(c, lw);
        dy_back(i, c, d);
        z_of(zr[ii][c], i, xh);
#pragma unroll
        for (int w = 0; w < 8; ++w) o[w] = rs[i] * (d[w] * lw[w] - a1 - xh[w] * a2);
        const int n = n_w + 32 * c + 8 * gq;
        const uint32_t off = m < e.M ? (uint32_t)(((size_t)m * e.ldc + n) * 2) : OOB;
        __builtin_amdgcn_raw_buffer_store_b128(pack8(o), rc, off, 0, 0);
      }
    }
  }
  vm_wait<0>();
}

template <bool AK, bool BKM, int EPI, bool P8, int FOLD = kFoldNone>
__global__ void __launch_bounds__(THREADS) __attribute__((amdgpu_waves_per_eu(2, 2)))
gemm9_kernel(const uint16_t* __restrict__ A, int64_t lda, const uint16_t* __restrict__ B, int64_t ldb, int nk, int tilesM,
             int tilesN, int nsplit, EpiArgs e, Ext x, Fold fold) {
  extern __shared__ __attribute__((aligned(16))) char smem[];
  const int wid = __builtin_amdgcn_readfirstlane(threadIdx.x >> 6), wm = wid >> 2, wn = wid & 3;
  const int nwg = tilesM * tilesN, total = nwg * nsplit;
  const int my_tiles = (total - (int)blockIdx.x + (int)gridDim.x - 1) / (int)gridDim.x;
  const int kper = nk * BK;

  auto geo = [&](int it) {
    const int t = blockIdx.x + it * gridDim.x;
    const int xcd = t & 7, loc = t >> 3, q8 = total >> 3, r8 = total & 7;
    const int wgi = (xcd < r8 ? xcd * (q8 + 1) : r8 * (q8 + 1) + (xcd - r8) * q8) + loc;
    const int split = wgi / nwg, wg = wgi - split * nwg;
    Geo gg;
    gg.m0 = (wg / tilesN) * BM;
    gg.n0 = (wg % tilesN) * BN;
    gg.split = split;
    gg.kbeg = split * kper;
    return gg;
  };

  const auto ra = rsrc(A, x.a), rb = rsrc(B, x.b);
  int l_it = 0, l_kt = 0, l_g = 0;
  Geo lg = geo(0);
  uint32_t va = 0, vb = 0;
  auto set_voffs = [&]() {
    va = AK ? vbase_k<false>(lda, lg.m0, wid) : vbase_m(lda, lg.m0, wid);
    vb = BKM ? vbase_k<P8>(ldb, lg.n0, wid) : vbase_m(ldb, lg.n0, wid);
  };
  set_voffs();
  auto issue_part = [&](int part) {
    const int k0 = lg.kbeg + l_kt * BK;
    if (part == 2) {
      char* bb = smem + b_off<AK>(l_g);
      const uint32_t so = BKM ? (uint32_t)k0 * 2 : (uint32_t)((int64_t)k0 * ldb * 2);
      const uint32_t step = (uint32_t)((BKM ? 64 : 16) * ldb * 2);
#pragma unroll
      for (int j = 0; j < 4; ++j)
        dma<EPI == SV_EPI_SLAB ? SV_G9_SLAB_B_CPOL : 0>(rb, vb, so + j * step, bb + (wid + 8 * j) * 1024);
      SV_VMTAG("p2");
    } else if constexpr (AK) {
      char* ab = smem + a_off<AK>(l_g);
      const int h = part == 1 ? 0 : 1;
      const uint32_t so = (uint32_t)k0 * 2 + (uint32_t)(64 * h * lda * 2);
      dma(ra, va, so, ab + (h * 8 + wid) * 1024);
      dma(ra, va, so + (uint32_t)(128 * lda * 2), ab + (h * 8 + 16 + wid) * 1024);
      if (part == 1) SV_VMTAG("p1");
      else SV_VMTAG("p3");
    } else if (part == 1) {
      char* ab = smem + a_off<AK>(l_g);
      const uint32_t so = (uint32_t)((int64_t)k0 * lda * 2), step = (uint32_t)(16 * lda * 2);
#pragma unroll
      for (int j = 0; j < 4; ++j) dma(ra, va, so + j * step, ab + (wid + 8 * j) * 1024);
      SV_VMTAG("p1");
    }
  };
  auto advance = [&]() {
    ++l_g;
    if (++l_kt == nk) {
      if (l_it + 1 < my_tiles) {
        ++l_it;
        l_kt = 0;
        lg = geo(l_it);
        set_voffs();
      } else {
        l_kt = nk - 1;
      }
    }
  };

  constexpr int E = EpiCount<EPI, P8>::E;
  constexpr bool LBIAS = AK && (EPI == SV_EPI_STORE || EPI == SV_EPI_BIAS_GELU_DUAL || EPI == SV_EPI_BIAS_GELU ||
                                EPI == SV_EPI_BIAS_GAMMA_RES || EPI == SV_EPI_STORE_STATS || EPI == SV_EPI_LN_BWD);
  constexpr int W1 = AK ? 10 : 8, W2 = 10;
  constexpr int W1E = W1 + E > 63 ? 63 : W1 + E, W2E = W2 + E > 63 ? 63 : W2 + E;
  const bool do_cs = EPI == SV_EPI_SLAB && !AK && e.C2 != nullptr;
  float cs[2] = {0.f, 0.f};
  auto colsum_frag = [&](const bf16x8 (&af)[4][2], float& acc_cs) {
    bf16x8 f0 = af[0][0], f1 = af[0][1];
    if (wn == 1) f0 = af[1][0], f1 = af[1][1];
    else if (wn == 2) f0 = af[2][0], f1 = af[2][1];
    else if (wn == 3) f0 = af[3][0], f1 = af[3][1];
    const bf16x8 f[2] = {f0, f1};
    typedef __bf16 bf16x2_t __attribute__((ext_vector_type(2)));
    const bf16x2_t ones = {(__bf16)1.0f, (__bf16)1.0f};
#pragma unroll
    for (int kh = 0; kh < 2; ++kh)
#pragma unroll
      for (int q = 0; q < 4; ++q) {
        const bf16x2_t pr = {f[kh][2 * q], f[kh][2 * q + 1]};
        acc_cs = __builtin_amdgcn_fdot2_f32_bf16(pr, ones, acc_cs, false);
      }
  };

  stamp(0);
#pragma unroll
  for (int t = 0; t < 2; ++t) {
    issue_part(1);
    issue_part(2);
    if constexpr (AK) issue_part(3);
    advance();
  }
  vm_wait<8>();
  bar();
  if (wm == 1) bar();
  if constexpr (SV_G9_PRIO == 1) {
    if (wm == 1) __builtin_amdgcn_s_setprio(1);
  }

  int g = 0;
  for (int it = 0; it < my_tiles; ++it) {
    const Geo cg = geo(it);
    f32x4 acc[FM][FN];
#pragma unroll
    for (int i = 0; i < FM; ++i)
#pragma unroll
      for (int j = 0; j < FN; ++j) acc[i][j] = f32x4{0.f, 0.f, 0.f, 0.f};
    cs[0] = cs[1] = 0.f;
    for (int kt = 0; kt < nk; ++kt, ++g) {
      const char* Ab = smem + a_off<AK>(g);
      const char* Bb = smem + b_off<AK>(g);
      bf16x8 af[4][2], bq[2][2][2];
      auto read_a = [&](int qm) {
#pragma unroll
        for (int i = 0; i < 4; ++i)
#pragma unroll
          for (int kh = 0; kh < 2; ++kh)
            af[i][kh] = AK ? frag_k(Ab, wm * 128 + 64 * qm + 16 * i, kh) : frag_m(Ab, wm * 128 + 64 * qm + 16 * i, kh);
      };
      auto read_b = [&](int qn) {
#pragma unroll
        for (int jj = 0; jj < 2; ++jj)
#pragma unroll
          for (int kh = 0; kh < 2; ++kh) {
            const int j = 2 * qn + jj;
            if constexpr (BKM) {
              bq[qn][jj][kh] = frag_k(Bb, wn * 64 + 16 * j, kh);
            } else if constexpr (P8) {
              const int p = threadIdx.x & 3;
              bq[qn][jj][kh] = frag_tr(Bb, wn * 8 + 4 * qn + p, jj, kh);
            } else {
              bq[qn][jj][kh] = frag_m(Bb, wn * 64 + 16 * j, kh);
            }
          }
      };
      auto quad = [&](int qm, int qn) {
        if constexpr (SV_G9_PRIO == 0) __builtin_amdgcn_s_setprio(1);
#pragma unroll
        for (int kh = 0; kh < 2; ++kh)
#pragma unroll
          for (int i = 0; i < 4; ++i)
#pragma unroll
            for (int jj = 0; jj < 2; ++jj)
              acc[4 * qm + i][2 * qn + jj] = __builtin_amdgcn_mfma_f32_16x16x32_bf16(
                  bq[qn][jj][kh], af[i][kh], acc[4 * qm + i][2 * qn + jj], 0, 0, 0);
        if constexpr (SV_G9_PRIO == 0) __builtin_amdgcn_s_setprio(0);
      };
      read_a(0);
      read_b(0);
      if constexpr (LBIAS) {
        if (kt == 0 && wid < 2) {
          const float* src = wid == 0 ? e.bias : e.gamma;
          if (src && (wid == 0 || EPI == SV_EPI_BIAS_GAMMA_RES))
            dma(rsrc(src, (uint32_t)e.N * 4), (uint32_t)(cg.n0 + (threadIdx.x & 63) * 4) * 4, 0,
                smem + lds_bytes<AK>() + (it & 1) * 2048 + wid * 1024);
          SV_VMTAG("bias");
        }
      }
      lgkm0();
      bar();
      quad(0, 0);
      bar();
      read_b(1);
      issue_part(1);
      if (do_cs) colsum_frag(af, cs[0]);
      if (AK) {
        if (it > 0 && kt <= 1) SV_VMWAIT(W2E, "p3:2@epi");
        else SV_VMWAIT(W2, "p3:2");
      }
      lgkm0();
      bar();
      quad(0, 1);
      bar();
      read_a(1);
      issue_part(2);
      lgkm0();
      bar();
      quad(1, 1);
      bar();
      if constexpr (AK) issue_part(3);
      advance();
      if (do_cs) colsum_frag(af, cs[1]);
      if (it > 0 && kt == 0) SV_VMWAIT(W1E, "p1:2@epi p2:2@epi");
      else SV_VMWAIT(W1, "p1:2 p2:2");
      lgkm0();
      bar();
      quad(1, 0);
      bar();
    }
    if (do_cs) {
#pragma unroll
      for (int h = 0; h < 2; ++h) {
        cs[h] += __shfl_xor(cs[h], 16);
        cs[h] += __shfl_xor(cs[h], 32);
        const int m = cg.m0 + wm * 128 + 64 * h + 16 * wn + (threadIdx.x & 15);
        if ((threadIdx.x & 63) < 16 && m < e.M) reinterpret_cast<float*>(e.C2)[(size_t)cg.split * e.M + m] = cs[h];
      }
    }
    if (LBIAS && nk < 2) {
      vm_wait<0>();
      bar();
    }
    if constexpr (FOLD) {
      if (wm == 0) bar();
    }
    if constexpr (EPI == SV_EPI_LN_BWD) {
      if (wm == 0) bar();
      ln_bwd_epilogue(acc, e, x, fold, cg.m0, cg.n0, tilesN, reinterpret_cast<const float*>(smem + lds_bytes<AK>()),
                      reinterpret_cast<float*>(smem + lds_bytes<AK>() + 4096), smem);
      if (wm == 1) bar();
    } else {
      epilogue<EPI, P8, AK, FOLD>(acc, e, x, cg.m0 + wm * 128, cg.n0 + wn * 64, cg.split,
                        LBIAS ? reinterpret_cast<const float*>(smem + lds_bytes<AK>() + (it & 1) * 2048) : nullptr);
    }
    SV_VMTAG("epi");
    if constexpr (FOLD) {
      vm_wait<0>();
      bar();
      static_assert(!AK, "the in-kernel fold is for the weight-gradient layout (N/M-major A)");
      volatile int* flag = reinterpret_cast<volatile int*>(smem + a_off<AK>(g - 1));
      const int tile = (cg.m0 / BM) * tilesN + cg.n0 / BN;
      int* arrive = fold.cnt + 2 * tile;
      int* depart = arrive + 1;
      if constexpr (FOLD == kFoldLast) {
        if (threadIdx.x == 0)
          *flag = __hip_atomic_fetch_add(arrive, 1, __ATOMIC_RELAXED, __HIP_MEMORY_SCOPE_AGENT) == nsplit - 1;
        lgkm0();
        bar();
        if (*flag) {
          fold_tile<2>(e, x, fold, cg.m0, cg.n0, nsplit);
          if (threadIdx.x == 0) __hip_atomic_store(arrive, 0, __ATOMIC_RELAXED, __HIP_MEMORY_SCOPE_AGENT);
        }
      } else {
        if (threadIdx.x == 0) {
          __hip_atomic_fetch_add(arrive, 1, __ATOMIC_RELAXED, __HIP_MEMORY_SCOPE_AGENT);
          while (__hip_atomic_load(arrive, __ATOMIC_RELAXED, __HIP_MEMORY_SCOPE_AGENT) < nsplit)
            __builtin_amdgcn_s_sleep(4);
        }
        bar();
        const int per = (BM + nsplit - 1) / nsplit;
        fold_tile<2>(e, x, fold, cg.m0, cg.n0, nsplit, cg.split * per, cg.split * per + per);
        if (threadIdx.x == 0 &&
            __hip_atomic_fetch_add(depart, 1, __ATOMIC_RELAXED, __HIP_MEMORY_SCOPE_AGENT) == nsplit - 1) {
          __hip_atomic_store(arrive, 0, __ATOMIC_RELAXED, __HIP_MEMORY_SCOPE_AGENT);
          __hip_atomic_store(depart, 0, __ATOMIC_RELAXED, __HIP_MEMORY_SCOPE_AGENT);
        }
      }
      bar();
      if (wm == 1) bar();
    }
  }
  vm_wait<0>();
  if (wm == 0) bar();
  stamp(1);
}

template <bool AK, int EPI, int FOLD = kFoldNone>
constexpr int lds_total() {
  return lds_bytes<AK>() + ((AK && (EPI == SV_EPI_STORE || EPI == SV_EPI_BIAS_GELU_DUAL || EPI == SV_EPI_BIAS_GELU ||
                                   EPI == SV_EPI_BIAS_GAMMA_RES || EPI == SV_EPI_STORE_STATS || EPI == SV_EPI_LN_BWD))
                                ? 4096 : 0) +
         (EPI == SV_EPI_LN_BWD ? kLnRed : 0);
}

template <bool AK, bool BKM, int EPI, bool P8, int FOLD = kFoldNone>
static int launch(const sv_gemm_desc* d, int split, hipStream_t s) {
  const int nk = d->K / split / BK;
  const int tilesM = ceil_div(d->M, BM), tilesN = ceil_div(d->N, BN);
  EpiArgs e{d->M, d->N, d->epilogue, d->C, d->c_dtype, d->ldc, d->C2, d->c2_dtype, d->bias, d->gamma,
            d->aux, d->aux_dtype, d->ld_aux};
  if constexpr (EPI == SV_EPI_LN_BWD) {
    e.bias = d->bn->gamma;
    e.bn_mu = d->bn->mean;
    e.bn_rs = d->bn->rstd;
  }
  const int cs = d->c_dtype == SV_F32 ? 4 : 2;
  Ext x;
  if (EPI == SV_EPI_SLAB) {
    x.c = (uint32_t)((size_t)d->M * d->N * (P8 ? 2 : 4));
  } else {
    x.c = (uint32_t)(((size_t)(d->M - 1) * d->ldc + d->N) * cs);
  }
  x.c2 = d->C2 ? (uint32_t)(((size_t)(d->M - 1) * d->ldc + d->N) * (d->c2_dtype == SV_F32 ? 4 : 2)) : 0u;
  x.aux = d->aux ? (uint32_t)(((size_t)(d->M - 1) * d->ld_aux + d->N) * (d->aux_dtype == SV_F32 ? 4 : 2)) : 0u;
  x.a = (uint32_t)((AK ? (size_t)(d->M - 1) * d->lda + d->K : (size_t)(d->K - 1) * d->lda + d->M) * 2);
  x.b = (uint32_t)((BKM ? (size_t)(d->N - 1) * d->ldb + d->K : (size_t)(d->K - 1) * d->ldb + d->N) * 2);
  constexpr int LDS = lds_total<AK, EPI, FOLD>();
  if (const int rc_ = ensure_lds_attr(reinterpret_cast<const void*>(&gemm9_kernel<AK, BKM, EPI, P8, FOLD>), LDS, s)) return rc_;
  const int total = tilesM * tilesN * split;
  const int grid = policy_grid(&d->policy, total, 1, s);
  const Fold fold{d->fold_out, d->fold_ld, d->fold_accumulate, d->fold_counters};
  if constexpr (EPI == SV_EPI_LN_BWD) {
    int usable = stream_cus(s);
    if (d->policy.grid_cap > 0 && d->policy.grid_cap < usable) usable = d->policy.grid_cap;
    if (grid != total || total > usable) return SV_ERR_UNSUPPORTED;
  }
  if constexpr (FOLD != kFoldNone) {
    int usable = stream_cus(s);
    if (d->policy.grid_cap > 0 && d->policy.grid_cap < usable) usable = d->policy.grid_cap;
    if (grid == total && 2 * total <= usable) {
      constexpr int LDS2 = lds_total<AK, EPI, kFoldSpread>();
      if (const int rc_ = ensure_lds_attr(reinterpret_cast<const void*>(&gemm9_kernel<AK, BKM, EPI, P8, kFoldSpread>), LDS2, s)) return rc_;
      gemm9_kernel<AK, BKM, EPI, P8, kFoldSpread><<<grid, THREADS, LDS2, s>>>(
          reinterpret_cast<const uint16_t*>(d->A), d->lda, reinterpret_cast<const uint16_t*>(d->B), d->ldb, nk, tilesM,
          tilesN, split, e, x, fold);
      return check_launch("sv_gemm(v9, spread fold)");
    }
  }
  gemm9_kernel<AK, BKM, EPI, P8, FOLD><<<grid, THREADS, LDS, s>>>(reinterpret_cast<const uint16_t*>(d->A), d->lda,
                                                                 reinterpret_cast<const uint16_t*>(d->B), d->ldb, nk,
                                                                 tilesM, tilesN, split, e, x, fold);
  return check_launch("sv_gemm(v9)");
}

template <bool AK, bool BKM>
static int launch_epi(const sv_gemm_desc* d, int split, hipStream_t s) {
  const bool bf_out = d->c_dtype == SV_BF16;
  switch (d->epilogue) {
    case SV_EPI_STORE:
      return bf_out ? launch<AK, BKM, SV_EPI_STORE, true>(d, split, s) : launch<AK, BKM, SV_EPI_STORE, false>(d, split, s);
    case SV_EPI_BIAS_GELU_DUAL:
      if (!bf_out || d->c2_dtype != SV_BF16) return SV_ERR_UNSUPPORTED;
      return launch<AK, BKM, SV_EPI_BIAS_GELU_DUAL, true>(d, split, s);
    case SV_EPI_BIAS_GELU:
      if (!bf_out) return SV_ERR_UNSUPPORTED;
      return launch<AK, BKM, SV_EPI_BIAS_GELU, true>(d, split, s);
    case SV_EPI_BIAS_GAMMA_RES:
      if (d->aux_dtype != SV_F32) return SV_ERR_UNSUPPORTED;
      return bf_out ? launch<AK, BKM, SV_EPI_BIAS_GAMMA_RES, true>(d, split, s)
                    : launch<AK, BKM, SV_EPI_BIAS_GAMMA_RES, false>(d, split, s);
    case SV_EPI_MUL_AUX:
      if (d->aux_dtype != SV_BF16) return SV_ERR_UNSUPPORTED;
      return bf_out ? launch<AK, BKM, SV_EPI_MUL_AUX, true>(d, split, s)
                    : launch<AK, BKM, SV_EPI_MUL_AUX, false>(d, split, s);
    case SV_EPI_GELU_GRAD:
      if (d->aux_dtype != SV_BF16) return SV_ERR_UNSUPPORTED;
      return bf_out ? launch<AK, BKM, SV_EPI_GELU_GRAD, true>(d, split, s)
                    : launch<AK, BKM, SV_EPI_GELU_GRAD, false>(d, split, s);
    case SV_EPI_STORE_STATS:
      if (!bf_out || !AK || d->N % 8) return SV_ERR_UNSUPPORTED;
      return launch<AK, BKM, SV_EPI_STORE_STATS, true>(d, split, s);
    case SV_EPI_LN_BWD:
      if constexpr (!AK) {
        return SV_ERR_UNSUPPORTED;
      } else {
        if (!bf_out || d->aux_dtype != SV_BF16 || d->N % BN || d->N > 4 * BN || split != 1 || !d->bn || !d->C2 ||
            !d->fold_out || !d->fold_counters)
          return SV_ERR_UNSUPPORTED;
        return launch<AK, BKM, SV_EPI_LN_BWD, true>(d, split, s);
      }
    case SV_EPI_SLAB:
      if (d->C2 && (AK || d->c2_dtype != SV_F32)) return SV_ERR_UNSUPPORTED;
      if (d->c_dtype == SV_BF16) {
        if constexpr (AK) {
          return SV_ERR_UNSUPPORTED;
        } else {
          if (d->fold_out || d->N % 8) return SV_ERR_UNSUPPORTED;
          return launch<AK, BKM, SV_EPI_SLAB, true>(d, split, s);
        }
      }
      if (d->fold_out) {
        if constexpr (AK) return SV_ERR_UNSUPPORTED;
        else return launch<AK, BKM, SV_EPI_SLAB, false, kFoldLast>(d, split, s);
      }
      return launch<AK, BKM, SV_EPI_SLAB, false>(d, split, s);
    default:
      return SV_ERR_UNSUPPORTED;
  }
}

}

#ifdef SV_CLOCK_STAMPS
extern "C" int sv_diag_clock_stamps(unsigned long long* host, int n) {
  if (n > 1024) n = 1024;
  return hipMemcpyFromSymbol(host, HIP_SYMBOL(g9::g_stamps), (size_t)n * 4 * sizeof(unsigned long long), 0,
                             hipMemcpyDeviceToHost) == hipSuccess ? 0 : 1;
}
#endif

int launch_gemm9(const sv_gemm_desc* d, hipStream_t s) {
  using namespace g9;
  if (d->compute != SV_BF16 || d->a_dtype != SV_BF16 || d->b_dtype != SV_BF16 || d->a_scale_k)
    return SV_ERR_UNSUPPORTED;
  const int split = d->epilogue == SV_EPI_SLAB ? (d->split_k < 1 ? 1 : d->split_k) : 1;
  if (d->K % (split * BK) != 0 || d->N % 8 != 0) return SV_ERR_UNSUPPORTED;
  if (d->epilogue != SV_EPI_SLAB && d->ldc % 8 != 0) return SV_ERR_UNSUPPORTED;
  if (d->aux && d->ld_aux % 8 != 0) return SV_ERR_UNSUPPORTED;
  const size_t lim = (size_t)1 << 31;
  const size_t rows = (size_t)ceil_div(d->M, BM) * BM;
  if (rows * (size_t)(d->epilogue == SV_EPI_SLAB ? d->N : d->ldc) * 4 * (size_t)split >= lim) return SV_ERR_UNSUPPORTED;
  if (d->aux && rows * (size_t)d->ld_aux * 4 >= lim) return SV_ERR_UNSUPPORTED;
  const size_t a_ext = d->a_kmajor ? (size_t)d->M * d->lda : (size_t)d->K * d->lda;
  const size_t b_ext = d->b_kmajor ? (size_t)d->N * d->ldb : (size_t)d->K * d->ldb;
  if ((a_ext + 4096) * 2 >= lim || (b_ext + 4096) * 2 >= lim) return SV_ERR_UNSUPPORTED;
  if (d->a_kmajor && d->b_kmajor) return launch_epi<true, true>(d, split, s);
  if (d->a_kmajor && !d->b_kmajor) return launch_epi<true, false>(d, split, s);
  if (!d->a_kmajor && d->b_kmajor) return launch_epi<false, true>(d, split, s);
  return launch_epi<false, false>(d, split, s);
}

}
```

spine-vision_amd/csrc/gemm_common.h:

```cpp
#pragma once

#include "common.h"

#ifndef SV_STATS_XLANE
#define SV_STATS_XLANE SV_XLANE
#endif

namespace sv {

typedef __bf16 bf16x8 __attribute__((ext_vector_type(8)));
typedef short s16x4 __attribute__((ext_vector_type(4)));
typedef float f32x4 __attribute__((ext_vector_type(4)));

constexpr int EPI_LD = 64 + 4;

struct EpiArgs {
  int M, N;
  int epi;
  void* C; int c_dtype; int64_t ldc;
  void* C2; int c2_dtype;
  const float* bias;
  const float* gamma;
  const void* aux; int aux_dtype; int64_t ld_aux;
  int prio = 0;
// ... 229 lines not shown
      const float* sp = slab + row * EPI_LD + cu;
      float4 va = make_float4(sp[0], sp[1], sp[2], sp[3]);
      float4 vb = make_float4(sp[4], sp[5], sp[6], sp[7]);
      if (slab_out) {
        float* C = reinterpret_cast<float*>(e.C) + (size_t)split * e.M * e.N + (size_t)m * e.N + n;
        if (okn4) {
          st8_any(C, SV_F32, 0, va, vb);
        } else {
          *reinterpret_cast<float4*>(C) = va;
        }
        continue;
      }
      va = add4(va, b0);
      vb = add4(vb, b1);
      float4 oa, ob;
      if (e.epi == SV_EPI_STORE || e.epi == SV_EPI_BIAS_GELU2 || e.epi == SV_EPI_STORE_STATS || kBnb) {
        oa = va;
        ob = vb;
      } else if (e.epi == SV_EPI_BIAS_GELU_DUAL) {
        float4 ga, gb;
        gelu_dual4(va, ga, oa);
        gelu_dual4(vb, gb, ob);
        va = ga;
        vb = gb;
      } else if (e.epi == SV_EPI_BIAS_GELU) {
        oa = gelu4(va);
        ob = gelu4(vb);
      } else if (e.epi == SV_EPI_MUL_AUX) {
        oa = mul4(va, xa[si][h]);
        ob = mul4(vb, xb[si][h]);
      } else if (e.epi == SV_EPI_BIAS_GAMMA_RES) {
        oa = fma4(g0, va, xa[si][h]);
        ob = fma4(g1, vb, xb[si][h]);
      } else {
        oa = ggrad4(va, xa[si][h]);
        ob = ggrad4(vb, xb[si][h]);
      }
      const size_t ci = orow(m) * e.ldc + n;
      if (okn4) st8_any(e.C, e.c_dtype, ci, oa, ob);
      else st4_any(e.C, e.c_dtype, ci, oa);
      if constexpr (kStats) {
        const float o8[8] = {oa.x, oa.y, oa.z, oa.w, ob.x, ob.y, ob.z, ob.w};
#pragma unroll
        for (int j = 0; j < 8; ++j) {
          const float q = e.c_dtype == SV_BF16 ? __uint_as_float((uint32_t)f2bf(o8[j]) << 16) : o8[j];
          cs1[j] += q;
          cs2[j] = fmaf(q, q, cs2[j]);
        }
      }
      if (e.epi == SV_EPI_BIAS_GELU2) {
        if (okn4) st8_any(e.C2, e.c2_dtype, ci, gelu4(va), gelu4(vb));
        else st4_any(e.C2, e.c2_dtype, ci, gelu4(va));
      } else if (e.epi == SV_EPI_BIAS_GELU_DUAL) {
        if (okn4) st8_any(e.C2, e.c2_dtype, ci, va, vb);
        else st4_any(e.C2, e.c2_dtype, ci, va);
      }
    }
    if constexpr (kBnb) {
#pragma unroll
      for (int r = 0; r < 16; ++r) {
        const int m = mb + i * 16 + r;
        if (!bn_ok || m >= e.M) continue;
        const float q = __uint_as_float((uint32_t)f2bf(slab[r * EPI_LD + l]) << 16);
        const float g = fmaf(bn_a, bn_y[r] - bn_mu, bn_be) > 0.f ? q : 0.f;
        bn_s1 += g;
        bn_s2 = fmaf(g, (bn_y[r] - bn_mu) * bn_rs, bn_s2);
      }
    }
    __builtin_amdgcn_fence(__ATOMIC_RELEASE, "workgroup");
    __builtin_amdgcn_wave_barrier();
    __builtin_amdgcn_fence(__ATOMIC_ACQUIRE, "workgroup");
  }
  if constexpr (kBnb) {
    if (bn_ok && mb < e.M) {
      const int prow = (mb >> 6) + (REMAP ? split * e.rm_prow : 0);
      float* P = reinterpret_cast<float*>(e.C2) + (size_t)prow * 2 * e.N + bn_n;
      P[0] = bn_s1;
      P[e.N] = bn_s2;
    }
  }
  if constexpr (kStats) {
#pragma unroll
    for (int j = 0; j < 8; ++j) {
#if SV_STATS_XLANE
      cs1[j] += xlane_xor<8>(cs1[j]);
      cs2[j] += xlane_xor<8>(cs2[j]);
      cs1[j] += xlane_xor<16>(cs1[j]);
      cs2[j] += xlane_xor<16>(cs2[j]);
      cs1[j] += xlane_xor<32>(cs1[j]);
      cs2[j] += xlane_xor<32>(cs2[j]);
#else
#pragma unroll
      for (int off = 8; off < 64; off <<= 1) {
        cs1[j] += __shfl_xor(cs1[j], off);
        cs2[j] += __shfl_xor(cs2[j], off);
      }
#endif
    }
    if (l < 8 && okn && mb < e.M) {
      float* P = reinterpret_cast<float*>(e.C2) + (size_t)(mb >> 6) * 2 * e.N + n;
      *reinterpret_cast<float4*>(P) = make_float4(cs1[0], cs1[1], cs1[2], cs1[3]);
      *reinterpret_cast<float4*>(P + 4) = make_float4(cs1[4], cs1[5], cs1[6], cs1[7]);
      *reinterpret_cast<float4*>(P + e.N) = make_float4(cs2[0], cs2[1], cs2[2], cs2[3]);
      *reinterpret_cast<float4*>(P + e.N + 4) = make_float4(cs2[4], cs2[5], cs2[6], cs2[7]);
    }
  }
}

template <int FM, int PRE = 1, int EPI = -1, int AUXT = -1, bool REMAP = false>
__device__ __forceinline__ void wave_tile_epilogue(const f32x4 (&acc)[FM][4], float* __restrict__ slab, int mb,
                                                   int nb, const EpiArgs& e, int split) {
  static_assert(FM % 4 == 0, "64-row groups");
#pragma unroll
  for (int i0 = 0; i0 < FM; i0 += 4)
    wave_group_epilogue<FM, PRE, 4, 0, EPI, AUXT, REMAP>(acc, i0, slab, mb + 16 * i0, nb, e, split);
}

template <int FM, int FN, int PRE = 1>
__device__ __forceinline__ void wave_tile_epilogue_wide(const f32x4 (&acc)[FM][FN], float* __restrict__ slab, int mb,
                                                        int nb, const EpiArgs& e, int split) {
  static_assert(FM % 4 == 0 && FN % 4 == 0 && FM <= 8 && FN <= 8, "64x64 groups");
  wave_group_epilogue<FM, PRE, FN, 0>(acc, 0, slab, mb, nb, e, split);
  if constexpr (FN >= 8) wave_group_epilogue<FM, PRE, FN, 4>(acc, 0, slab, mb, nb + 64, e, split);
  if constexpr (FM >= 8) {
    wave_group_epilogue<FM, PRE, FN, 0>(acc, 4, slab, mb + 64, nb, e, split);
    if constexpr (FN >= 8) wave_group_epilogue<FM, PRE, FN, 4>(acc, 4, slab, mb + 64, nb + 64, e, split);
  }
}

constexpr int CONV_MAX_TAPS = 64;
struct ConvG {
  int SH, SW, lsc;
  int GH, GW, si;
  uint32_t gw_mul, gw_shift, ghw_mul, ghw_shift;
  int lcout, Tw, Cs;
  int8_t tdy[CONV_MAX_TAPS], tdx[CONV_MAX_TAPS];
  uint8_t twt[CONV_MAX_TAPS];
  uint8_t ctap0[4], ctaps[4];
  uint32_t kw_mul;
  int kw, pad, ntaps;
};
inline void conv_fastdiv(uint32_t D, uint32_t& mul, uint32_t& shift) {
  uint32_t l = 0;
  while ((1ull << l) < D) ++l;
  shift = l;
  mul = (uint32_t)((((1ull << l) - D) << 32) / D + 1);
}
int launch_gemm3_conv(const sv_gemm_desc* d, const ConvG& g, int mode, hipStream_t s);

int launch_gemm2(const sv_gemm_desc* d, hipStream_t s);
int launch_gemm3(const sv_gemm_desc* d, hipStream_t s, const char* cfg = nullptr);
int launch_gemm8(const sv_gemm_desc* d, hipStream_t s);
int launch_gemm9(const sv_gemm_desc* d, hipStream_t s);

}
```

spine-vision_amd/kernels.py:

```python

from __future__ import annotations

import ctypes
import math
import os

import numpy as np
import torch

from . import native as nv
from .native import SV_BF16, SV_F32, call, dt, ptr, value

EPS_LN = 1e-6


class GemmProbe:

    def __init__(self, key: tuple, name: str = "") -> None:
        self.key = key
        self.name = name
        self.events: list[tuple[torch.cuda.Event, torch.cuda.Event]] = []
        self.flops = 0.0
        self.bytes = 0.0
        self.launches = 0
# ... 195 lines not shown
        xch = _LN_XCH[key] = torch.empty(max(tilesM * tilesN * 512, 1 << 18), device=dh2d.device, dtype=torch.float32)
    bn = nv.BnRef(ptr(mean), ptr(rstd), ptr(lnw), None)
    try:
        linear_dgrad(dh2d, w, out=dz, epilogue=nv.SV_EPI_LN_BWD, out2=part, aux=z2d, ld_aux=C, bn=bn, policy=policy,
                     fold=(xch, False, _fold_counters(dh2d.device, tilesM)))
    except RuntimeError as err:
        if "(status 2)" in str(err):
            return None
        raise
    return dz, _ln_partials_finish(part, P, dw, db)


def linear_fwd(x2d, w, *, out, bias=None, epilogue=nv.SV_EPI_STORE, out2=None, gamma=None, residual=None,
               compute_bf16=True, policy=None, split_k=1):
    M, K = x2d.shape
    N = w.shape[0]
    return gemm(x2d, w, M=M, N=N, K=K, a_kmajor=True, b_kmajor=True, lda=K, ldb=K, epilogue=epilogue, C=out,
                C2=out2, bias=bias, gamma=gamma, aux=residual, split_k=split_k, compute_bf16=compute_bf16,
                policy=policy)


def linear_dgrad(dy2d, w, *, out, epilogue=nv.SV_EPI_STORE, a_scale_k=None, aux=None, compute_bf16=True, policy=None,
                 split_k=1, out2=None, bn=None, gamma=None, ld_aux=None, fold=None):
    M, N = dy2d.shape
    K = w.shape[1]
    return gemm(dy2d, w, M=M, N=K, K=N, a_kmajor=True, b_kmajor=False, lda=N, ldb=K, epilogue=epilogue, C=out,
                C2=out2, gamma=gamma, a_scale_k=a_scale_k, aux=aux, ld_aux=ld_aux, split_k=split_k,
                compute_bf16=compute_bf16, bn=bn, policy=policy, fold=fold)


def _wgrad_slabs(dy2d, x2d, K, split, *, bf16_slabs=False, cs=None, fold=None, compute_bf16=True, policy=None):
    M, N = dy2d.shape
    slab = torch.empty(split * N * K, device=dy2d.device, dtype=torch.bfloat16 if bf16_slabs else torch.float32)
    if fold is not None:
        fold = (*fold, _fold_counters(dy2d.device, -(-N // 256) * -(-K // 256)))
    gemm(dy2d, x2d, M=N, N=K, K=M, a_kmajor=False, b_kmajor=False, lda=N, ldb=x2d.shape[1], epilogue=nv.SV_EPI_SLAB,
         C=slab, C2=cs, split_k=split, compute_bf16=compute_bf16, policy=policy, fold=fold)
    return slab


MLP_FUSED_C = (128, 192, 256, 512)


def mlp_fwd(y, w1, b1, w2, b2, gamma, x, *, out, gelu_grad=None, gelu_out=None):
    M, C = y.shape
    H = 4 * C
    _check(C in MLP_FUSED_C, f"mlp_fwd: C = {C} not supported {MLP_FUSED_C}")
    _check(y.dtype == torch.bfloat16 and w1.dtype == torch.bfloat16 and w2.dtype == torch.bfloat16,
           "mlp_fwd: y / w1 / w2 must be bf16")
    _check(tuple(w1.shape) == (H, C) and tuple(w2.shape) == (C, H), "mlp_fwd: weight shapes")
    for t_, n_ in ((b1, H), (b2, C), (gamma, C)):
        _check(t_.dtype == torch.float32 and t_.numel() == n_ and t_.is_contiguous(), "mlp_fwd: bias / gamma")
    _check(x.dtype == torch.float32 and out.dtype == torch.float32 and x.numel() == M * C and out.numel() == M * C,
           "mlp_fwd: x / out must be f32 [M, C]")
    _check(out.data_ptr() != x.data_ptr(), "mlp_fwd: out must not alias x")
    _check((gelu_grad is None) == (gelu_out is None), "mlp_fwd: gelu_grad and gelu_out go together")
    ts = [y, w1, b1, w2, b2, gamma, x, out]
    if gelu_grad is not None:
        for t_ in (gelu_grad, gelu_out):
            _check(t_.dtype == torch.bfloat16 and t_.numel() == M * H, "mlp_fwd: GELU outputs must be bf16 [M, 4C]")
        ts += [gelu_grad, gelu_out]
    _check(all(t_.is_contiguous() and t_.data_ptr() % 16 == 0 for t_ in ts), "mlp_fwd: contiguous 16-B aligned tensors")
    _check(M * H * 2 < 2**31, "mlp_fwd: hidden tensor must be < 2 GiB")
    nb = M * C * (2 + 4 + 4) + 2 * H * C * 2 + (2 * M * H * 2 if gelu_grad is not None else 0)
    _timed_call("mlp_fused", nb, "sv_mlp_fwd", ptr(y), ptr(w1), ptr(b1), ptr(w2), ptr(b2), ptr(gamma), ptr(x), ptr(out),
                ptr(gelu_grad), ptr(gelu_out), M, C, flops=4.0 * M * C * H)
    return out


def transpose_scale_bf16(W: torch.Tensor, scale: torch.Tensor | None = None, out: torch.Tensor | None = None):
    R_, C_ = W.shape
    _check(W.dtype == torch.float32 and W.is_contiguous(), "transpose_scale_bf16: need contiguous f32")
    _check(scale is None or (scale.numel() == R_ and scale.dtype == torch.float32), "transpose_scale_bf16: bad scale")
    if out is None:
        out = torch.empty(C_, R_, device=W.device, dtype=torch.bfloat16)
    _check(tuple(out.shape) == (C_, R_) and out.dtype == torch.bfloat16 and out.is_contiguous(),
           "transpose_scale_bf16: bad out")
    call("sv_transpose_scale_bf16", ptr(W), ptr(scale), ptr(out), R_, C_)
    return out


MLP_BWD_FUSED_C = (128,)


def mlp_bwd(d, w2t, gelu_grad, w1t, z, mean, rstd, lnw, *, dh, dz):
    M, C = d.shape
    H = 4 * C
    _check(C in MLP_BWD_FUSED_C, f"mlp_bwd: C = {C} not supported {MLP_BWD_FUSED_C}")
    for t_, shp in ((d, (M, C)), (w2t, (H, C)), (gelu_grad, (M, H)), (w1t, (C, H)), (z, (M, C)), (dh, (M, H)),
                    (dz, (M, C))):
        _check(t_.dtype == torch.bfloat16 and t_.numel() == shp[0] * shp[1] and t_.is_contiguous(),
               f"mlp_bwd: bf16 [{shp[0]}, {shp[1]}] operand expected")
    for t_, n_ in ((mean, M), (rstd, M), (lnw, C)):
        _check(t_.dtype == torch.float32 and t_.numel() == n_ and t_.is_contiguous(), "mlp_bwd: f32 vector")
    P = value("sv_mlp_bwd_nparts", M, C)
    part = torch.empty(2, P, C, device=d.device, dtype=torch.float32)
    ts = [d, w2t, gelu_grad, w1t, z, mean, rstd, lnw, dh, dz, part]
    _check(all(t_.data_ptr() % 16 == 0 for t_ in ts), "mlp_bwd: 16-B aligned tensors")
    _check(M * H * 2 < 2**31, "mlp_bwd: hidden tensor must be < 2 GiB")
    nb = M * (C * 2 + H * 2 + C * 2 + H * 2 + C * 2 + 8) + 2 * H * C * 2
    _timed_call("mlp_bwd_fused", nb, "sv_mlp_bwd", ptr(d), ptr(w2t), ptr(gelu_grad), ptr(w1t), ptr(z), ptr(mean),
                ptr(rstd), ptr(lnw), ptr(dh), ptr(dz), ptr(part), M, C, flops=4.0 * M * C * H)
    return part, P


_WGRAD_TARGET = 512
_WGRAD9_TARGET = int(os.environ.get("SV_WGRAD9_WGS", "128"))
_WGRAD9_LONG_GFLOP = float(os.environ.get("SV_WGRAD9_LONG_GFLOP", "150"))


def _wgrad_split(tiles: int, K: int) -> int:
    split = max(1, -(-_WGRAD_TARGET // max(tiles, 1)))
    return max(1, min(split, K // 512 if K >= 512 else 1))


def _wgrad_split_for(N: int, K: int, M: int, target: int | None = None) -> int:
    if min(N, K) >= 128 and max(N, K) >= 256:
        tiles9 = -(-N // 256) * -(-K // 256)
        target = (target or _WGRAD9_TARGET) if 2.0 * M * N * K <= _WGRAD9_LONG_GFLOP * 1e9 else 256
        ok = [s_ for s_ in range(1, max(2, 2 * target // tiles9 + 1)) if M % (s_ * 64) == 0 and tiles9 * s_ <= 256]
        if ok:
            return min(ok, key=lambda s_: (abs(tiles9 * s_ - target), s_))
    return _wgrad_split(-(-N // 128) * -(-K // 128), M)


_INKERNEL_FOLD = os.environ.get("SV_INKERNEL_FOLD", "0") != "0"
_FOLD_MAX_SPLIT = int(os.environ.get("SV_FOLD_MAX_SPLIT", "64"))
_FOLD_COUNTERS: dict = {}


def _fold_counters(device, tiles: int) -> torch.Tensor:
    key = (device, nv._stream())
    t = _FOLD_COUNTERS.get(key)
    if t is None or t.numel() < 2 * tiles:
        t = _FOLD_COUNTERS[key] = torch.zeros(max(2 * tiles, 4096), device=device, dtype=torch.int32)
    return t


_WGRAD_BF16_SLABS = os.environ.get("SV_WGRAD_BF16_SLABS", "1") != "0"


def _bf16_slabs(N: int, K: int, M: int, split: int, compute_bf16: bool, policy=None) -> bool:
    return (_WGRAD_BF16_SLABS and compute_bf16 and split > 1 and min(N, K) >= 128 and max(N, K) >= 256
            and K % 8 == 0 and M % (split * 64) == 0 and (policy is None or policy.impl in (0, 9)))


def _fold_ok(split: int, n: int, out: torch.Tensor, compute_bf16: bool) -> bool:
    return (_INKERNEL_FOLD and compute_bf16 and 1 < split <= _FOLD_MAX_SPLIT and n >= 65536 and n % 4 == 0
            and out.dtype == torch.float32 and out.is_contiguous() and out.data_ptr() % 16 == 0)


def linear_wgrad(dy2d, x2d, *, out=None, accumulate=False, bias_out=None, bias_accumulate=True,
                 compute_bf16=True, cols=None, defer: list | None = None, policy=None,
                 wgrad_target: int | None = None) -> torch.Tensor:
    M, N = dy2d.shape
    K = x2d.shape[1] if cols is None else cols
    split = _wgrad_split_for(N, K, M, wgrad_target)
    cs = torch.empty(split * N, device=dy2d.device, dtype=torch.float32) if bias_out is not None else None
    bf16 = (out is not None and _bf16_slabs(N, K, M, split, compute_bf16, policy) and out.is_contiguous()
            and out.numel() == N * K)
    infold = not bf16 and out is not None and _fold_ok(split, N * K, out, compute_bf16)
    if infold:
        _check(out.numel() == N * K, "linear_wgrad: bad out")
    slab = _wgrad_slabs(dy2d, x2d, K, split, bf16_slabs=bf16, cs=cs, fold=(out, accumulate) if infold else None,
                        compute_bf16=compute_bf16, policy=policy)
    if bf16:
        _timed_call("fold", 2.0 * split * N * K + 4.0 * N * K * (1 + int(bool(accumulate))), "sv_reduce_partials_bf16",
                    ptr(slab), split, N * K, ptr(out), 1.0, int(bool(accumulate)))
    if bf16 or infold:
        _colsum_finish(cs, split, bias_out, bias_accumulate, defer)
        return out
    if out is None:
        if split == 1 and not accumulate:
            _colsum_finish(cs, split, bias_out, bias_accumulate, None)
            return slab.view(N, K)
        out = torch.empty(N, K, device=dy2d.device, dtype=torch.float32)
        accumulate = False
    _check(out.numel() == N * K and out.is_contiguous(), "linear_wgrad: bad out")
    if defer is not None:
        defer.append((slab, out, split, accumulate))
        _colsum_finish(cs, split, bias_out, bias_accumulate, defer)
    elif cs is not None and bias_accumulate == accumulate:
        reduce_pair(slab, out, cs, bias_out, split, accumulate=accumulate)
    else:
        _colsum_finish(cs, split, bias_out, bias_accumulate, None)
        reduce_into(slab, split, out, accumulate)
    return out


def _colsum_finish(cs, split, bias_out, accumulate, defer) -> None:
    if cs is None:
        return
    if defer is not None:
        defer.append((cs, bias_out, split, accumulate))
    else:
        reduce_into(cs, split, bias_out, accumulate=accumulate)


def layerscale_wgrad(dsrc2d, a2d, w2, gamma, b2, *, dw2, dgamma, db2, compute_bf16=True, policy=None,
                     wgrad_target: int | None = None):
    M, C = dsrc2d.shape
    K4 = a2d.shape[1]
    split = _wgrad_split_for(C, K4, M, wgrad_target)
    cs = torch.empty(split * C, device=dsrc2d.device, dtype=torch.float32)
    bf16 = _bf16_slabs(C, K4, M, split, compute_bf16, policy)
    G = None if bf16 else torch.empty(C * K4, device=dsrc2d.device, dtype=torch.float32)
    infold = not bf16 and _fold_ok(split, C * K4, G, compute_bf16)
    slab = _wgrad_slabs(dsrc2d, a2d, K4, split, bf16_slabs=bf16, cs=cs, fold=(G, False) if infold else None,
                        compute_bf16=compute_bf16, policy=policy)
    rest = (ptr(cs), split, ptr(w2), ptr(gamma), ptr(b2), ptr(dw2), ptr(dgamma), ptr(db2))
    if bf16:
        _timed_call("fold", 2.0 * split * C * K4 + 8.0 * C * K4 + 4.0 * (split + 4) * C,
                    "sv_layerscale_wgrad_reduce_bf16", ptr(slab), *rest, C, K4)
    elif infold:
        _timed_call("fold", 4.0 * (3 * C * K4 + (split + 4) * C), "sv_layerscale_wgrad_fold_finish", ptr(G), *rest,
                    C, K4)
    else:
        _timed_call("fold", 4.0 * ((split + 2) * C * K4 + (split + 4) * C), "sv_layerscale_wgrad_reduce", ptr(slab),
                    *rest, None, C, K4)


def reduce_into(part: torch.Tensor, nparts: int, out: torch.Tensor, accumulate: bool = True, alpha: float = 1.0):
    reduce_pair(part, out, None, None, nparts, accumulate=accumulate, alpha=alpha)


def reduce_pair(part_a: torch.Tensor, out_a: torch.Tensor, part_b: torch.Tensor | None, out_b: torch.Tensor | None,
                nparts: int, accumulate: bool = True, alpha: float = 1.0):
    na = out_a.numel()
    _check(part_a.numel() >= nparts * na, "reduce_pair: partial buffer a too small")
    _check(out_a.dtype == torch.float32 and out_a.is_contiguous(), "reduce_pair: out must be contiguous f32")
    nb = 0
    if out_b is not None:
        nb = out_b.numel()
        _check(part_b is not None and part_b.numel() >= nparts * nb, "reduce_pair: partial buffer b too small")
        _check(out_b.dtype == torch.float32 and out_b.is_contiguous(), "reduce_pair: out must be contiguous f32")
    moved = 4.0 * (na + nb) * (nparts + 1 + int(bool(accumulate)))
    _timed_call("fold", moved, "sv_reduce_partials_pair", ptr(part_a), na, ptr(out_a), ptr(part_b), nb, ptr(out_b),
                nparts, float(alpha), int(accumulate))


def reduce_multi(segs: list, alpha: float = 1.0) -> None:
    for i in range(0, len(segs), nv.SV_MAX_RED_SEGS):
        chunk = segs[i:i + nv.SV_MAX_RED_SEGS]
        arr = (nv.RedSeg * len(chunk))()
        moved = 0.0
        for j, (part, out, P, acc) in enumerate(chunk):
            n = out.numel()
            _check(out.dtype == torch.float32 and out.is_contiguous() and part.numel() >= P * n,
                   "reduce_multi: bad segment")
            arr[j] = nv.RedSeg(ptr(part), ptr(out), n, int(P), int(bool(acc)))
            moved += 4.0 * n * (P + 1 + int(bool(acc)))
        _timed_call("fold", moved, "sv_reduce_partials_multi", arr, len(chunk), float(alpha))


def _ln_partials_finish(part: torch.Tensor, P: int, dw: torch.Tensor, db: torch.Tensor):
    def finish(record: bool = True, defer: list | None = None):
        if record:
            part.record_stream(torch.cuda.current_stream())
        if defer is not None:
            defer += [(part[0], dw, P, True), (part[1], db, P, True)]
            return
        reduce_pair(part[0], dw, part[1], db, P)
    return finish


def colsum_into(x2d: torch.Tensor, out: torch.Tensor, accumulate: bool = True):
    rows, C = x2d.shape
    P = value("sv_colsum_nparts", rows, C)
    part = torch.empty(P * C, device=x2d.device, dtype=torch.float32)
    call("sv_colsum", ptr(x2d), dt(x2d), rows, C, ptr(part))
    reduce_into(part, P, out, accumulate)


def colsum(x2d: torch.Tensor) -> torch.Tensor:
    out = torch.empty(x2d.shape[1], device=x2d.device, dtype=torch.float32)
    colsum_into(x2d, out, accumulate=False)
    return out


def layernorm_fwd(x2d, w, b, *, out_dtype, eps=EPS_LN):
    rows, C = x2d.shape
    y = torch.empty(rows, C, device=x2d.device, dtype=out_dtype)
    mean = torch.empty(rows, device=x2d.device, dtype=torch.float32)
    rstd = torch.empty_like(mean)
    call("sv_layernorm_fwd", ptr(x2d), dt(x2d), ptr(w), ptr(b), ptr(y), dt(y), ptr(mean), ptr(rstd), rows, C, eps)
    return y, mean, rstd


def layernorm_bwd(dy2d, x2d, mean, rstd, w, *, dw, db, dx=None, accumulate_dx=False, out_dtype=torch.float32,
                  defer_reduce=False):
    rows, C = x2d.shape
    _check(tuple(dy2d.shape) == (rows, C) and dy2d.is_contiguous(), "layernorm_bwd: dy must be contiguous [rows,C]")
    if dx is None:
        dx = torch.empty(rows, C, device=x2d.device, dtype=out_dtype)
    P = value("sv_layernorm_bwd_nparts", rows, C)
    pw = torch.empty(2, P * C, device=x2d.device, dtype=torch.float32)
    nb = rows * C * (dy2d.element_size() + x2d.element_size() + dx.element_size() * (2 if accumulate_dx else 1)) + rows * 8
    _timed_call("ln_bwd", nb, "sv_layernorm_bwd", ptr(dy2d), dt(dy2d), ptr(x2d), dt(x2d), ptr(mean), ptr(rstd), ptr(w),
                ptr(dx), dt(dx), int(accumulate_dx), ptr(pw[0]), ptr(pw[1]), rows, C)
    if defer_reduce:
        return dx, _ln_partials_finish(pw, P, dw, db)
    if dw is not None and db is not None:
        reduce_pair(pw[0], dw, pw[1], db, P)
    elif dw is not None:
        reduce_into(pw[0], P, dw)
    elif db is not None:
        reduce_into(pw[1], P, db)
    return dx


ATTN_TORCH = os.environ.get("SV_ATTN", "") == "torch"
ATTN_HEAD_DIM = 64
ATTN_MAX_N = 256
ATTN_STREAM_MAX_N = 2048


def _attn_geometry(who: str, qkv, B: int, N: int, heads: int, img_rows) -> tuple[int, int]:
    rows = N if img_rows is None else int(img_rows)
    C = heads * ATTN_HEAD_DIM
    _check(B > 0 and heads > 0 and 1 <= N <= rows, f"{who}: need B, heads > 0 and 1 <= N <= img_rows")
    _check(qkv.dim() == 2 and tuple(qkv.shape) == (B * rows, 3 * C) and qkv.is_contiguous()
           and qkv.dtype in (torch.bfloat16, torch.float32),
           f"{who}: qkv must be contiguous bf16 / f32 [{B * rows}, {3 * C}], got {tuple(qkv.shape)} {qkv.dtype}")
    return rows, C


def _attn_views(t2d, B: int, rows: int, N: int, heads: int, parts: int):
    v = t2d.view(B, rows, parts, heads, ATTN_HEAD_DIM)[:, :N].permute(2, 0, 3, 1, 4)
    return tuple(v[i] for i in range(parts))


def _attn_torch_arm(qkv) -> bool:
    return ATTN_TORCH or qkv.dtype == torch.float32


def attn_fwd(qkv, B: int, N: int, heads: int, *, img_rows: int | None = None, scale: float | None = None,
             out: torch.Tensor | None = None, lse: torch.Tensor | None = None, torch_arm: bool | None = None,
             _who: str = "attn_fwd", _max_n: int = ATTN_MAX_N):
    rows, C = _attn_geometry(_who, qkv, B, N, heads, img_rows)
    scale = ATTN_HEAD_DIM ** -0.5 if scale is None else float(scale)
    if out is None:
        out = torch.empty(B * rows, C, device=qkv.device, dtype=qkv.dtype)
    if lse is None:
        lse = torch.empty(B, heads, N, device=qkv.device, dtype=torch.float32)
    _check(tuple(out.shape) == (B * rows, C) and out.is_contiguous() and out.dtype == qkv.dtype, f"{_who}: bad out")
    _check(tuple(lse.shape) == (B, heads, N) and lse.is_contiguous() and lse.dtype == torch.float32, f"{_who}: bad lse")
    if _attn_torch_arm(qkv) if torch_arm is None else (torch_arm or qkv.dtype == torch.float32):
        q, k, v = _attn_views(qkv, B, rows, N, heads, 3)
        s = torch.matmul(q.float(), k.float().transpose(-1, -2)) * scale
        torch.logsumexp(s, dim=-1, out=lse)
        p = torch.exp(s - lse.unsqueeze(-1)).to(qkv.dtype)
        o = out.view(B, rows, heads, ATTN_HEAD_DIM)
        o[:, :N] = torch.matmul(p, v).permute(0, 2, 1, 3)
        if rows > N:
            o[:, N:] = 0
        return out, lse
    _check(N <= _max_n, f"{_who}: N = {N} tokens (at most {_max_n})")
    call("sv_" + _who, ptr(qkv), ptr(out), ptr(lse), B, N, rows, heads, ATTN_HEAD_DIM, scale)
    return out, lse


def attn_stream_fwd(qkv, B: int, N: int, heads: int, *, img_rows: int | None = None, scale: float | None = None,
                    out: torch.Tensor | None = None, lse: torch.Tensor | None = None, torch_arm: bool | None = None):
    return attn_fwd(qkv, B, N, heads, img_rows=img_rows, scale=scale, out=out, lse=lse, torch_arm=torch_arm,
                    _who="attn_stream_fwd", _max_n=ATTN_STREAM_MAX_N)


def attn_bwd(qkv, out, lse, dout, B: int, N: int, heads: int, *, img_rows: int | None = None,
             scale: float | None = None, dqkv: torch.Tensor | None = None, torch_arm: bool | None = None,
             _who: str = "attn_bwd", _max_n: int = ATTN_MAX_N):
    rows, C = _attn_geometry(_who, qkv, B, N, heads, img_rows)
    scale = ATTN_HEAD_DIM ** -0.5 if scale is None else float(scale)
# ... 1905 lines not shown
```

spine-vision_amd/native.py:

```python

from __future__ import annotations

import ctypes
import os
import re
import threading

import torch

_HERE = os.path.dirname(os.path.abspath(__file__))
LIB_PATH = os.environ.get("SV_LIB_PATH") or os.path.join(_HERE, "libsv_kernels.so")
HEADER = os.path.join(os.path.dirname(_HERE), "include", "sv_kernels.h")

SV_F32, SV_BF16 = 0, 1
SV_IMG_F32_NCHW, SV_IMG_U8_GRAY, SV_IMG_U8_HWC = 0, 1, 2
SV_BN_SMALL_MASK, SV_BN_SMALL_RELU, SV_BN_SMALL_DUAL = 0, 1, 2
SV_HEAD_CE, SV_HEAD_BCE = 0, 1
SV_BN_FOLD_CTL_INTS, SV_BN_FOLD_WS_FLOATS = 256, 2 * 2 * 2048 + 2 * 64 * 16 * 64
(SV_EPI_STORE, SV_EPI_BIAS_GELU2, SV_EPI_BIAS_GAMMA_RES, SV_EPI_GELU_GRAD, SV_EPI_SLAB, SV_EPI_BIAS_GELU_DUAL,
 SV_EPI_MUL_AUX, SV_EPI_BIAS_GELU, SV_EPI_STORE_STATS, SV_EPI_STORE_BN_BWD, SV_EPI_LN_BWD) = range(11)

_p = ctypes.c_void_p
_i32 = ctypes.c_int32
_i64 = ctypes.c_int64
_f32 = ctypes.c_float


class BnRef(ctypes.Structure):
    _fields_ = [("mean", _p), ("rstd", _p), ("gamma", _p), ("beta", _p)]


class GemmPolicy(ctypes.Structure):
    _fields_ = [("impl", _i32), ("grid_cap", _i32), ("wg_per_cu", _i32), ("priority", _i32)]

    def __repr__(self) -> str:
        return (f"GemmPolicy(impl={self.impl}, grid_cap={self.grid_cap}, wg_per_cu={self.wg_per_cu}, "
                f"priority={self.priority})")


class CtxInfo(ctypes.Structure):
    _fields_ = [("device", _i32), ("compute_units", _i32), ("lds_bytes_per_wg", _i32), ("xcds", _i32),
                ("lds_raised_kernels", _i32), ("refs", _i32), ("arch", ctypes.c_char * 32)]


def policy(impl: int = 0, grid_cap: int = 0, wg_per_cu: int = 0, priority: int = 0) -> GemmPolicy:
    return GemmPolicy(int(impl), int(grid_cap or 0), int(wg_per_cu), int(priority))


class GemmDesc(ctypes.Structure):
    _fields_ = [
        ("M", _i32), ("N", _i32), ("K", _i32),
        ("A", _p), ("a_dtype", _i32), ("a_kmajor", _i32), ("lda", _i64),
        ("B", _p), ("b_dtype", _i32), ("b_kmajor", _i32), ("ldb", _i64),
        ("a_scale_k", _p),
        ("epilogue", _i32),
        ("C", _p), ("c_dtype", _i32), ("ldc", _i64),
        ("C2", _p), ("c2_dtype", _i32),
        ("bias", _p),
        ("gamma", _p),
        ("aux", _p), ("aux_dtype", _i32), ("ld_aux", _i64),
        ("split_k", _i32),
        ("compute", _i32),
        ("bn", ctypes.POINTER(BnRef)),
        ("policy", GemmPolicy),
        ("fold_out", _p), ("fold_ld", _i64), ("fold_accumulate", _i32), ("fold_counters", _p),
    ]


class RedSeg(ctypes.Structure):
    _fields_ = [("part", _p), ("out", _p), ("n", _i64), ("P", _i32), ("accumulate", _i32)]


class HeadTask(ctypes.Structure):
    _fields_ = [("kind", _i32), ("offset", _i32), ("ncls", _i32), ("weight", _f32), ("label_smoothing", _f32),
                ("target", _p), ("target_dtype", _i32)]


SV_MAX_RED_SEGS = 8


class PackSeg(ctypes.Structure):
    _fields_ = [("w", _p), ("wp", _p), ("Cout", _i32), ("Cin", _i32), ("T", _i32), ("Cs", _i32)]


SV_MAX_PACK_SEGS = 32


class ConvShape(ctypes.Structure):
    _fields_ = [("B", _i32), ("H", _i32), ("W", _i32), ("Cs", _i32), ("Cout", _i32), ("KH", _i32), ("KW", _i32),
                ("stride", _i32), ("pad", _i32), ("Cin", _i32)]


class GConvShape(ctypes.Structure):
    _fields_ = [("B", _i32), ("H", _i32), ("W", _i32), ("C", _i32), ("groups", _i32), ("KH", _i32), ("KW", _i32),
                ("stride", _i32), ("pad", _i32)]


class GConvPackSeg(ctypes.Structure):
    _fields_ = [("w", _p), ("wp_fwd", _p), ("wp_bwd", _p), ("C", _i32), ("groups", _i32)]


SV_MAX_GPACK_SEGS = 32
_GS = ctypes.POINTER(GConvShape)
_CS = ctypes.POINTER(ConvShape)
_POL = ctypes.POINTER(GemmPolicy)

_SIGS = {
    "sv_version": [],
    "sv_ctx_create": [_i32, ctypes.POINTER(_p)],
    "sv_ctx_destroy": [_p],
    "sv_ctx_get_info": [_p, ctypes.POINTER(CtxInfo)],
    "sv_last_error_string": [],
    "sv_build_target": [],
    "sv_gemm": [ctypes.POINTER(GemmDesc), _p],
    "sv_stream_create_cu_reserved": [_i32, ctypes.POINTER(_i32), _i32, ctypes.POINTER(_p)],
    "sv_gemm_slab_finish": [_p, _i32, _i32, _i32, _p, _i32, _i64, _i32, _p, _p],
    "sv_gemm_slab_finish_bn_bwd": [_p, _i32, _i32, _i32, _p, _p, ctypes.POINTER(BnRef), _p, _p],
    "sv_mlp_fwd": [_p, _p, _p, _p, _p, _p, _p, _p, _p, _p, _i64, _i32, _p],
    "sv_mlp_bwd_nparts": [_i64, _i32],
    "sv_mlp_bwd": [_p, _p, _p, _p, _p, _p, _p, _p, _p, _p, _p, _i64, _i32, _p],
    "sv_transpose_scale_bf16": [_p, _p, _p, _i32, _i32, _p],
    "sv_layernorm_fwd": [_p, _i32, _p, _p, _p, _i32, _p, _p, _i64, _i32, _f32, _p],
    "sv_layernorm_bwd_nparts": [_i64, _i32],
    "sv_layernorm_bwd": [_p, _i32, _p, _i32, _p, _p, _p, _p, _i32, _i32, _p, _p, _i64, _i32, _p],
    "sv_grn_nparts": [_i64, _i32],
    "sv_grn_stats": [_p, _i32, _p, _i32, _i64, _i32, _p],
    "sv_grn_finish": [_p, _i32, _p, _p, _p, _p, _p, _i32, _i32, _f32, _p],
    "sv_grn_apply": [_p, _i32, _p, _p, _p, _i32, _i64, _i32, _p],
    "sv_grn_bwd_stats": [_p, _p, _i32, _p, _p, _i32, _i64, _i32, _p],
    "sv_grn_bwd_finish": [_p, _p, _i32, _p, _p, _p, _p, _p, _p, _p, _i32, _i32, _i32, _p],
    "sv_grn_bwd_apply": [_p, _p, _p, _i32, _p, _p, _p, _i32, _i64, _i32, _p],
    "sv_dwconv7_ln_fwd": [_p, _i32, _p, _p, _p, _p, _f32, _p, _i32, _p, _i32, _p, _p, _i32, _i32, _i32, _i32, _p],
    "sv_dwconv7_bwd_data": [_p, _i32, _p, _p, _p, _i32, _i32, _i32, _i32, _i32, _p],
    "sv_dwconv7_fwd_mfma": [_p, _i32, _p, _p, _p, _i32, _i32, _i32, _i32, _p],
    "sv_dwconv7_bwd_data_mfma": [_p, _p, _p, _p, _i32, _i32, _i32, _i32, _i32, _p],
    "sv_dwconv7_bwd_weight_mfma_nparts": [_i32, _i32, _i32, _i32],
    "sv_dwconv7_bwd_weight_mfma": [_p, _p, _i32, _p, _p, _i32, _i32, _i32, _i32, _p],
    "sv_dwconv7_bwd_weight_nparts": [_i32, _i32, _i32, _i32],
    "sv_dwconv7_ln_fused_ok": [_i32, _i32, _i32, _i32, _i32, _i32, _i32],
    "sv_diag_group_sum": [_p, _p, _p, _i64, _i32, _p],
    "sv_dwconv7_bwd_weight": [_p, _i32, _p, _i32, _p, _p, _i32, _i32, _i32, _i32, _p],
    "sv_stem_patchify_ln_fwd": [_p, _p, _p, _p, _p, _f32, _p, _i32, _p, _p, _i32, _i32, _i32, _i32, _p],
    "sv_stem_patchify_ln_bwd_nparts": [_i32, _i32, _i32, _i32],
    "sv_stem_patchify_ln_bwd": [_p, _p, _p, _p, _p, _p, _p, _p, _p, _p, _p, _i32, _i32, _i32, _i32, _p],
    "sv_stem_patchify": [_p, _i32, _p, _p, _p, _i32, _i32, _i32, _p],
    "sv_stem_weight_pack": [_p, _p, _i32, _p],
    "sv_normalize_u8_gray": [_p, _p, _p, _p, _i32, _i32, _i32, _p],
    "sv_augment_u8": [_p, _p, _i32, _i32, _i32, _i32, _p, _p, _p],
    "sv_resize_u8": [_p, _p, _p, _i32, _i32, _i32, _i32, _p, _p],
    "sv_downsample_ln_patch2_fwd": [_p, _p, _p, _f32, _p, _i32, _p, _p, _i32, _i32, _i32, _i32, _p],
    "sv_downsample_ln_patch2_bwd_nparts": [_i32, _i32, _i32, _i32],
    "sv_downsample_ln_patch2_bwd": [_p, _p, _p, _p, _p, _p, _p, _p, _p, _i32, _i32, _i32, _i32, _p],
    "sv_pool_ln_fwd": [_p, _p, _p, _f32, _p, _p, _p, _p, _i32, _i32, _i32, _p],
    "sv_pool_ln_bwd": [_p, _p, _p, _p, _p, _p, _p, _p, _p, _i32, _i32, _i32, _p],
    "sv_reduce_partials": [_p, _i32, _i32, _i64, _p, _f32, _i32, _p],
    "sv_reduce_partials_bf16": [_p, _i32, _i64, _p, _f32, _i32, _p],
    "sv_reduce_partials_pair": [_p, _i64, _p, _p, _i64, _p, _i32, _f32, _i32, _p],
    "sv_reduce_partials_multi": [ctypes.POINTER(RedSeg), _i32, _f32, _p],
    "sv_colsum_nparts": [_i64, _i32],
    "sv_colsum": [_p, _i32, _i64, _i32, _p, _p],
    "sv_layerscale_wgrad_finish": [_p, _p, _p, _p, _p, _p, _p, _p, _i32, _i32, _p],
    "sv_layerscale_wgrad_reduce_ws": [_i32, _i32],
    "sv_layerscale_wgrad_reduce": [_p, _p, _i32, _p, _p, _p, _p, _p, _p, _p, _i32, _i32, _p],
    "sv_layerscale_wgrad_reduce_bf16": [_p, _p, _i32, _p, _p, _p, _p, _p, _p, _i32, _i32, _p],
    "sv_layerscale_wgrad_fold_finish": [_p, _p, _i32, _p, _p, _p, _p, _p, _p, _i32, _i32, _p],
    "sv_sqnorm_nparts": [_i64],
    "sv_sqnorm_partial": [_p, _i64, _p, _p],
    "sv_clip_coef": [_p, _i32, _f32, _p, _p],
    "sv_adamw_flat": [_p, _p, _p, _p, _p, _i64, _f32, _f32, _f32, _f32, _f32, _i32, _p, _p],
    "sv_adamw_flat_dev": [_p, _p, _p, _p, _p, _i64, _f32, _f32, _f32, _f32, _p, _p, _p],
    "sv_scale_rows_bf16": [_p, _p, _p, _i32, _i32, _p],
    "sv_cast_f32_bf16": [_p, _p, _i64, _p],
    "sv_conv_weight_pack": [_p, _p, _i32, _CS, _p],
    "sv_conv_weight_pack_multi": [ctypes.POINTER(PackSeg), _i32, _i32, _p],
    "sv_conv_fwd": [_p, _p, _p, _i32, _i32, _CS, _POL, _p],
    "sv_conv_fwd_stats": [_p, _p, _p, _i32, _i32, _CS, _p, _POL, _p],
    "sv_conv_bwd_data": [_p, _p, _p, _i32, _i32, _i32, _CS, _POL, _p],
    "sv_conv_fwd_split": [_p, _p, _p, _i32, _i32, _CS, _p, _p, _i32, _POL, _p],
    "sv_conv_bwd_data_split": [_p, _p, _p, _i32, _i32, _i32, _CS, _p, _i32, _POL, _p],
    "sv_conv_bwd_data_bn": [_p, _p, _p, _i32, _CS, _p, ctypes.POINTER(BnRef), _p, _p, _i32, _POL, _p],
    "sv_conv_bwd_weight_work_floats": [_CS],
    "sv_conv_bwd_weight": [_p, _p, _p, _p, _i32, _i32, _CS, _POL, _p],
    "sv_gconv_weight_pack": [ctypes.POINTER(GConvPackSeg), _i32, _p],
    "sv_gconv_fwd": [_p, _p, _p, _GS, _p],
    "sv_gconv_bwd_data": [_p, _p, _p, _GS, _p],
    "sv_gconv_bwd_weight_nparts": [_GS],
    "sv_gconv_bwd_weight_work_floats": [_GS],
    "sv_gconv_bwd_weight": [_p, _p, _p, _p, _i32, _GS, _p],
    "sv_attn_fwd": [_p, _p, _p, _i32, _i32, _i64, _i32, _i32, _f32, _p],
    "sv_attn_bwd": [_p, _p, _p, _p, _p, _i32, _i32, _i64, _i32, _i32, _f32, _p],
    "sv_attn_stream_fwd": [_p, _p, _p, _i32, _i32, _i64, _i32, _i32, _f32, _p],
    "sv_attn_stream_bwd": [_p, _p, _p, _p, _p, _p, _i32, _i32, _i64, _i32, _i32, _f32, _p],
    "sv_winattn_bwd_nparts": [_i32, _i32, _i32, _i32, _i32],
    "sv_winattn_fwd": [_p, _p, _p, _p, _i32, _i32, _i32, _i32, _i32, _i32, _i32, _f32, _i64, _p],
    "sv_winattn_bwd": [_p, _p, _p, _p, _p, _p, _p, _i32, _i32, _i32, _i32, _i32, _i32, _i32, _f32, _i64, _p],
    "sv_swin_bias_expand": [_p, _p, _i32, _i32, _p],
    "sv_swin_bias_grad": [_p, _p, _i32, _i32, _i32, _i32, _p],
    "sv_patch_merge": [_p, _p, _i32, _i32, _i32, _i32, _i32, _i64, _p],
    "sv_patch_merge_bwd": [_p, _p, _i32, _i32, _i32, _i32, _i32, _i64, _p],
    "sv_rowscale_add": [_p, _p, _p, _p, _i64, _i64, _i32, _i32, _p],
    "sv_rowscale_cast_bf16": [_p, _p, _p, _i64, _i64, _i32, _i32, _p],
    "sv_patchify16": [_p, _i32, _p, _p, _p, _i32, _i32, _i32, _i32, _i64, _i32, _p],
    "sv_vit_tokens": [_p, _p, _p, _p, _i32, _i32, _i32, _i32, _i32, _p],
    "sv_image_to_nhwc": [_p, _p, _i32, _i32, _i32, _i32, _i32, _i32, _p],
    "sv_image_u8_hwc_to_nhwc": [_p, _p, _p, _p, _i32, _i32, _i32, _i32, _i32, _p],
    "sv_bn_nparts": [_i64, _i32],
    "sv_bn_stats": [_p, _i32, _i64, _i32, _p, _p],
    "sv_bn_stats_finish": [_p, _i32, _p, _i32, _i64, _i32, _f32, _f32, _p, _p, _p, _p, _p, _p, _p, _p],
    "sv_bn_eval_params": [_p, _p, _f32, _p, _p, _i32, _p],
    "sv_bn_act_fwd": [_p, _i32, _p, _p, _p, _p, _p, _i32, _p, _p, _p, _p, _i32, _p, _i32, _i64, _i32, _p],
    "sv_bn_bwd_stats": [_p, _i32, _p, _i32, _p, _i32, _p, _p, _i64, _i32, _p, _p],
    "sv_bn_bwd_stats_mask": [_p, _i32, _p, _i32, _p, _i32, _p, _p, _i64, _i32, _p, _p],
    "sv_bn_bwd_finish": [_p, _i32, _i32, _p, _p, _p, _p, _p, _p],
    "sv_bn_bwd_stats_mask_dual": [_p, _i32, _p, _i32, _p, _i32, _p, _p, _p, _i32, _p, _p, _i64, _i32, _p, _p, _p],
    "sv_bn_bwd_apply_dual": [_p, _i32, _p, _i32, _p, _p, _p, _p, _p, _i32, _p, _p, _p, _p, _p, _p, _i32, _i64, _i32,
                             _p],
    "sv_bn_relu_bwd_stats": [_p, _i32, _p, _i32, _p, _p, _p, _p, _i64, _i32, _p, _p],
    "sv_bn_relu_bwd_apply": [_p, _i32, _p, _i32, _p, _p, _p, _p, _p, _p, _i32, _i64, _i32, _p],
    "sv_bn_relu_bwd_stats_pool": [_p, _i32, _p, _i32, _i32, _i32, _p, _i32, _p, _p, _p, _p, _i32, _p, _p],
    "sv_bn_relu_bwd_apply_pool": [_p, _i32, _p, _i32, _i32, _i32, _p, _i32, _p, _p, _p, _p, _p, _p, _i32, _i32, _p],
    "sv_bn_bwd_apply": [_p, _i32, _p, _i32, _p, _i32, _p, _p, _p, _p, _p, _i32, _p, _i64, _i32, _p],
    "sv_bn_small_ok": [_i64, _i32],
    "sv_bn_bwd_small": [_i32, _p, _i32, _p, _i32, _p, _i32, _p, _p, _p, _p, _p, _i32, _p, _p, _p, _p, _i32, _p, _p,
                        _i32, _p, _p, _p, _p, _i32, _i64, _i32, _p],
    "sv_bn_act_small": [_p, _i32, _p, _i32, _f32, _f32, _p, _p, _p, _p, _p, _p, _p, _p, _i32, _p, _i32, _f32, _f32,
                        _p, _p, _p, _p, _p, _p, _p, _i32, _p, _i32, _i64, _i32, _p],
    "sv_bn_fold_ok": [_i64, _i32, _i32],
    "sv_bn_act_fold": [_p, _i32, _p, _i32, _f32, _f32, _p, _p, _p, _p, _p, _p, _p, _p, _i32, _p, _i32, _f32, _f32,
                       _p, _p, _p, _p, _p, _p, _p, _i32, _p, _i32, _i64, _i32, _p, _p, _p],
    "sv_bn_bwd_apply_fold": [_i32, _p, _i32, _p, _i32, _i32, _p, _i32, _p, _p, _p, _p, _p, _i32, _p, _p, _p, _p, _p,
                             _i32, _p, _p, _i32, _p, _p, _p, _p, _i32, _i64, _i32, _p, _p, _p],
    "sv_head_loss": [_p, _i32, _i32, _p, _i32, _p, _p, _p],
    "sv_relu_mask": [_p, _i32, _p, _i32, _p, _i64, _p],
    "sv_maxpool3s2_fwd": [_p, _i32, _p, _p, _i32, _i32, _i32, _i32, _p],
    "sv_maxpool3s2_bwd": [_p, _i32, _p, _p, _i32, _i32, _i32, _i32, _i32, _p],
    "sv_avgpool_fwd": [_p, _i32, _p, _i32, _i32, _i32, _p],
    "sv_avgpool_bwd": [_p, _p, _i32, _i32, _i32, _i32, _p],
    "sv_se_nparts": [_i32, _i32],
    "sv_se_squeeze": [_p, _i32, _p, _i32, _i32, _i32, _p],
    "sv_se_excite": [_p, _i32, _p, _p, _p, _p, _p, _p, _p, _p, _p, _p, _p, _p, _i32, _i32, _i32, _i32, _p],
    "sv_se_join_fwd": [_p, _i32, _p, _p, _p, _p, _p, _p, _i32, _p, _p, _p, _p, _p, _i32, _i32, _i32, _i32, _p],
    "sv_se_bwd_stats": [_p, _i32, _p, _i32, _p, _i32, _p, _p, _p, _i32, _i32, _i32, _p],
    "sv_se_bwd_gate": [_p, _i32, _p, _p, _p, _p, _p, _p, _p, _p, _p, _p, _p, _p, _p, _p, _p, _p, _p, _p, _p, _i32, _i32,
                       _i32, _i32, _i32, _p],
    "sv_se_bwd_apply": [_p, _i32, _p, _i32, _p, _p, _p, _p, _p, _p, _p, _i32, _i32, _i32, _i32, _p],
    "sv_avgpool2x2_fwd": [_p, _i32, _p, _i32, _i32, _i32, _i32, _p],
    "sv_avgpool2x2_bwd": [_p, _i32, _p, _i32, _i32, _i32, _i32, _i32, _p],
    "sv_mbconv_nparts": [_i64, _i32],
    "sv_mbconv_bn_stats": [_p, _i32, _i64, _i32, _p, _p],
    "sv_bn_silu_fwd": [_p, _i32, _p, _p, _p, _p, _p, _i32, _p, _i32, _i64, _i32, _p],
    "sv_bn_silu_bwd_stats": [_p, _i32, _p, _i32, _p, _p, _p, _p, _i64, _i32, _p, _p],
    "sv_bn_silu_bwd_apply": [_p, _i32, _p, _i32, _p, _p, _p, _p, _p, _p, _i32, _i64, _i32, _p],
    "sv_mbconv_add": [_p, _i32, _p, _i32, _i64, _p],
    "sv_dwconv3_fwd": [_p, _i32, _p, _p, _i32, _i32, _i32, _i32, _i32, _i32, _p],
    "sv_dwconv3_bwd_data": [_p, _i32, _p, _p, _i32, _i32, _i32, _i32, _i32, _i32, _p],
    "sv_dwconv3_bwd_weight_nparts": [_i32, _i32, _i32, _i32, _i32],
    "sv_dwconv3_bwd_weight": [_p, _i32, _p, _i32, _p, _p, _i32, _i32, _i32, _i32, _i32, _i32, _p],
    "sv_mbse_squeeze": [_p, _i32, _p, _p, _p, _p, _p, _i32, _i32, _i32, _p],
    "sv_mbse_excite": [_p, _i32, _p, _p, _p, _p, _p, _p, _p, _p, _i32, _i32, _i32, _i32, _p],
    "sv_mbse_scale": [_p, _i32, _p, _p, _p, _p, _p, _p, _i32, _i32, _i32, _i32, _p],
    "sv_mbse_bwd_stats": [_p, _i32, _p, _i32, _p, _p, _p, _p, _p, _i32, _i32, _i32, _p],
    "sv_mbse_bwd_gate": [_p, _i32, _p, _p, _p, _p, _p, _p, _p, _p, _p, _p, _p, _p, _i32, _i32, _i32, _p],
    "sv_mbse_bwd_apply": [_p, _i32, _p, _i32, _p, _p, _p, _p, _p, _p, _p, _i32, _p, _i32, _i32, _i32, _p],
}
_RESTYPES = {"sv_last_error_string": ctypes.c_char_p, "sv_build_target": ctypes.c_char_p,
             "sv_conv_bwd_weight_work_floats": ctypes.c_int64, "sv_gconv_bwd_weight_work_floats": ctypes.c_int64}
_VALUE_FNS = {n for n in _SIGS if n.endswith(("_nparts", "_ws"))} | {"sv_version", "sv_bn_fold_ok", "sv_dwconv7_ln_fused_ok", "sv_conv_bwd_weight_work_floats",
# ... 195 lines not shown
```

Measured before the change: 1140 images/sec.

## Group fc1 and fc2 weight-gradient GEMMs into one grouped persistent kernel launch

Adds a grouped variant of the gemm9 persistent kernel (sv_gemm_group) that runs the fc2 and fc1 weight-gradient split-K slab GEMMs of each ConvNeXt block in a single launch with a shared split factor. The fc2 wgrad is deferred until dh is ready so both problems are submitted together on the side stream. The aim is to fill the GPU better and cut launch and tail overhead compared with two separate wgrad launches. In exchange, fc2 wgrad starts later, which may reduce its overlap with the main-stream dgrad, and the shared split choice may not suit either GEMM as well as its own split did.

```diff
diff --git a/include/sv_kernels.h b/include/sv_kernels.h
--- a/include/sv_kernels.h
+++ b/include/sv_kernels.h
@@ -85,6 +85,7 @@
 } sv_gemm_desc;
 
 int sv_gemm(const sv_gemm_desc* d, sv_stream_t stream);
+int sv_gemm_group(const sv_gemm_desc* descs, int32_t n, sv_stream_t stream);
 int sv_gemm_slab_finish(const float* slab, int32_t split, int32_t M, int32_t N, void* C, int32_t c_dtype, int64_t ldc,
                         int32_t accumulate, float* stats, sv_stream_t stream);
 int sv_gemm_slab_finish_bn_bwd(const float* slab, int32_t split, int32_t M, int32_t N, void* C, const void* y,
diff --git a/spine-vision_amd/backbone/convnext.py b/spine-vision_amd/backbone/convnext.py
--- a/spine-vision_amd/backbone/convnext.py
+++ b/spine-vision_amd/backbone/convnext.py
@@ -204,6 +204,9 @@
         self.side_impl = int(os.environ.get("SV_WGRAD_IMPL", "0"))
         self.main_bwd_cap = int(os.environ.get("SV_MAIN_BWD_CAP", "0"))
         self.wgrad_target = int(os.environ.get("SV_CNX_WGRAD_WGS", "256"))
+        self.wgrad_group = os.environ.get("SV_CNX_WGRAD_GROUP", "1")
+        if self.wgrad_group not in ("0", "1", "split"):
+            raise ValueError(f"SV_CNX_WGRAD_GROUP must be 0, 1 or split (got {self.wgrad_group!r})")
         self.side_prio = int(os.environ.get("SV_SIDE_PRIO", "1"))
         self.fused_mlp = os.environ.get("SV_FUSED_MLP", "1") != "0"
         self.fused_mlp_c = tuple(int(c) for c in os.environ.get("SV_FUSED_MLP_C", "128,192,256").split(",") if c)
@@ -439,7 +442,22 @@
             if folds is not None:
                 K.reduce_multi(folds)
 
-        sched.submit(fc2_wgrad, (dsrc, u), ready=fc2_ps if tail else None)
+        def fc21_wgrad(policy):
+            if self.use_grn:
+                p2 = dict(dy=dsrc, x=u, out=g(fc2.weight), accumulate=True, bias_out=g(fc2.bias))
+            else:
+                p2 = dict(dy=dsrc, x=a, w2=fc2.weight.detach(), gamma=blk.gamma.detach(), b2=fc2.bias.detach(),
+                          dw2=g(fc2.weight), dgamma=g(blk.gamma), db2=g(fc2.bias))
+            p1 = dict(dy=dh, x=y, out=g(fc1.weight), accumulate=True, bias_out=g(fc1.bias), defer=folds)
+            K.wgrad_group([p2, p1], compute_bf16=bf, policy=policy, wgrad_target=self.wgrad_target,
+                          one_launch=self.wgrad_group == "1")
+
+        grouped = (self.wgrad_group != "0" and bf and dsrc.is_contiguous() and u.is_contiguous() and y.is_contiguous()
+                   and K.wgrad_group_split([(C, 4 * C), (4 * C, C)], M, compute_bf16=bf,
+                                           policy=sched.spol if side is not None else pol,
+                                           target=self.wgrad_target) is not None)
+        if not grouped:
+            sched.submit(fc2_wgrad, (dsrc, u), ready=fc2_ps if tail else None)
         ev_w2 = side.record_event() if side is not None and not bf else None
         dh = torch.empty(M, 4 * C, device=d.device, dtype=act)
         wt = tape.wt.pop(id(blk), None)
@@ -463,7 +481,10 @@
         else:
             K.linear_dgrad(dsrc, fc2.weight.detach(), out=dh, epilogue=nv.SV_EPI_MUL_AUX, a_scale_k=blk.gamma, aux=gh,
                            compute_bf16=False, policy=pol)
-        sched.submit(fc1_wgrad, (dh, y))
+        if grouped:
+            sched.submit(fc21_wgrad, (dsrc, u, dh, y), ready=fc2_ps if tail else None)
+        else:
+            sched.submit(fc1_wgrad, (dh, y))
         if wt is None:
             w1 = self._w(fc1.weight, cache)
             fused = K.linear_dgrad_ln(dh, w1, z.view(M, C), mean, rstd, blk.norm.weight, dw=g(blk.norm.weight),
diff --git a/spine-vision_amd/csrc/gemm.hip b/spine-vision_amd/csrc/gemm.hip
--- a/spine-vision_amd/csrc/gemm.hip
+++ b/spine-vision_amd/csrc/gemm.hip
@@ -366,6 +366,26 @@
   return launch_layout<true, float, float>(d, s);
 }
 
+extern "C" int sv_gemm_group(const sv_gemm_desc* descs, int32_t n, sv_stream_t stream) {
+  SV_REQUIRE(descs && n >= 1, "sv_gemm_group: null descriptors");
+  for (int i = 0; i < n && i < 4; ++i) {
+    const sv_gemm_desc* d = descs + i;
+    SV_REQUIRE(d->A && d->B && d->C, "sv_gemm_group: null operand (problem %d)", i);
+    SV_REQUIRE(d->M >= 0 && d->N >= 0 && d->K >= 0, "sv_gemm_group: negative size (problem %d)", i);
+    SV_REQUIRE(d->policy.impl == 0 || d->policy.impl == 2 || d->policy.impl == 3 || d->policy.impl == 8 || d->policy.impl == 9,
+               "sv_gemm_group: policy.impl must be 0, 2, 3, 8 or 9 (got %d)", d->policy.impl);
+    SV_REQUIRE(d->policy.grid_cap >= 0 && d->policy.wg_per_cu >= 0 && d->policy.wg_per_cu <= 2 &&
+                   (d->policy.priority == 0 || d->policy.priority == 1),
+               "sv_gemm_group: bad policy (grid_cap >= 0, wg_per_cu 0..2, priority 0/1)");
+    SV_REQUIRE(al16(d->A) && al16(d->B) && al16(d->C) && al16(d->C2), "sv_gemm_group: operands must be 16-byte aligned");
+    SV_REQUIRE(d->lda % 8 == 0 && d->ldb % 8 == 0, "sv_gemm_group: lda/ldb must be multiples of 8");
+    SV_REQUIRE((d->a_kmajor ? d->K : d->M) % 8 == 0 && (d->b_kmajor ? d->K : d->N) % 8 == 0,
+               "sv_gemm_group: contiguous dims must be multiples of 8");
+  }
+  if (n < 2 || n > 4 || (descs[0].policy.impl != 0 && descs[0].policy.impl != 9)) return SV_ERR_UNSUPPORTED;
+  return launch_gemm9_group(descs, n, (hipStream_t)stream);
+}
+
 namespace sv {
 namespace {
 constexpr int SF_THREADS = 256;
diff --git a/spine-vision_amd/csrc/gemm9.hip b/spine-vision_amd/csrc/gemm9.hip
--- a/spine-vision_amd/csrc/gemm9.hip
+++ b/spine-vision_amd/csrc/gemm9.hip
@@ -103,10 +103,27 @@
 
 struct Geo {
   int m0, n0, kbeg, split;
+  int p;
 };
 
 struct Ext {
   uint32_t c, c2, aux, a, b;
+};
+
+constexpr int kMaxGroup = 4;
+struct GroupProb {
+  const uint16_t* A;
+  const uint16_t* B;
+  void* C;
+  void* C2;
+  int64_t lda, ldb;
+  int M, N, tilesN, nwg;
+  uint32_t xa, xb, xc;
+  int end;
+};
+struct Group {
+  int total;
+  GroupProb p[kMaxGroup];
 };
 
 struct Fold {
@@ -655,273 +672,12 @@
   vm_wait<0>();
 }
 
-template <bool AK, bool BKM, int EPI, bool P8, int FOLD = kFoldNone>
-__global__ void __launch_bounds__(THREADS) __attribute__((amdgpu_waves_per_eu(2, 2)))
-gemm9_kernel(const uint16_t* __restrict__ A, int64_t lda, const uint16_t* __restrict__ B, int64_t ldb, int nk, int tilesM,
-             int tilesN, int nsplit, EpiArgs e, Ext x, Fold fold) {
-  extern __shared__ __attribute__((aligned(16))) char smem[];
-  const int wid = __builtin_amdgcn_readfirstlane(threadIdx.x >> 6), wm = wid >> 2, wn = wid & 3;
-  const int nwg = tilesM * tilesN, total = nwg * nsplit;
-  const int my_tiles = (total - (int)blockIdx.x + (int)gridDim.x - 1) / (int)gridDim.x;
-  const int kper = nk * BK;
-
-  auto geo = [&](int it) {
-    const int t = blockIdx.x + it * gridDim.x;
-    const int xcd = t & 7, loc = t >> 3, q8 = total >> 3, r8 = total & 7;
-    const int wgi = (xcd < r8 ? xcd * (q8 + 1) : r8 * (q8 + 1) + (xcd - r8) * q8) + loc;
-    const int split = wgi / nwg, wg = wgi - split * nwg;
-    Geo gg;
-    gg.m0 = (wg / tilesN) * BM;
-    gg.n0 = (wg % tilesN) * BN;
-    gg.split = split;
-    gg.kbeg = split * kper;
-    return gg;
-  };
-
-  const auto ra = rsrc(A, x.a), rb = rsrc(B, x.b);
-  int l_it = 0, l_kt = 0, l_g = 0;
-  Geo lg = geo(0);
-  uint32_t va = 0, vb = 0;
-  auto set_voffs = [&]() {
-    va = AK ? vbase_k<false>(lda, lg.m0, wid) : vbase_m(lda, lg.m0, wid);
-    vb = BKM ? vbase_k<P8>(ldb, lg.n0, wid) : vbase_m(ldb, lg.n0, wid);
-  };
-  set_voffs();
-  auto issue_part = [&](int part) {
-    const int k0 = lg.kbeg + l_kt * BK;
-    if (part == 2) {
-      char* bb = smem + b_off<AK>(l_g);
-      const uint32_t so = BKM ? (uint32_t)k0 * 2 : (uint32_t)((int64_t)k0 * ldb * 2);
-      const uint32_t step = (uint32_t)((BKM ? 64 : 16) * ldb * 2);
-#pragma unroll
-      for (int j = 0; j < 4; ++j)
-        dma<EPI == SV_EPI_SLAB ? SV_G9_SLAB_B_CPOL : 0>(rb, vb, so + j * step, bb + (wid + 8 * j) * 1024);
-      SV_VMTAG("p2");
-    } else if constexpr (AK) {
-      char* ab = smem + a_off<AK>(l_g);
-      const int h = part == 1 ? 0 : 1;
-      const uint32_t so = (uint32_t)k0 * 2 + (uint32_t)(64 * h * lda * 2);
-      dma(ra, va, so, ab + (h * 8 + wid) * 1024);
-      dma(ra, va, so + (uint32_t)(128 * lda * 2), ab + (h * 8 + 16 + wid) * 1024);
-      if (part == 1) SV_VMTAG("p1");
-      else SV_VMTAG("p3");
-    } else if (part == 1) {
-      char* ab = smem + a_off<AK>(l_g);
-      const uint32_t so = (uint32_t)((int64_t)k0 * lda * 2), step = (uint32_t)(16 * lda * 2);
-#pragma unroll
-      for (int j = 0; j < 4; ++j) dma(ra, va, so + j * step, ab + (wid + 8 * j) * 1024);
-      SV_VMTAG("p1");
-    }
-  };
-  auto advance = [&]() {
-    ++l_g;
-    if (++l_kt == nk) {
-      if (l_it + 1 < my_tiles) {
-        ++l_it;
-        l_kt = 0;
-        lg = geo(l_it);
-        set_voffs();
-      } else {
-        l_kt = nk - 1;
-      }
-    }
-  };
-
-  constexpr int E = EpiCount<EPI, P8>::E;
-  constexpr bool LBIAS = AK && (EPI == SV_EPI_STORE || EPI == SV_EPI_BIAS_GELU_DUAL || EPI == SV_EPI_BIAS_GELU ||
-                                EPI == SV_EPI_BIAS_GAMMA_RES || EPI == SV_EPI_STORE_STATS || EPI == SV_EPI_LN_BWD);
-  constexpr int W1 = AK ? 10 : 8, W2 = 10;
-  constexpr int W1E = W1 + E > 63 ? 63 : W1 + E, W2E = W2 + E > 63 ? 63 : W2 + E;
-  const bool do_cs = EPI == SV_EPI_SLAB && !AK && e.C2 != nullptr;
-  float cs[2] = {0.f, 0.f};
-  auto colsum_frag = [&](const bf16x8 (&af)[4][2], float& acc_cs) {
-    bf16x8 f0 = af[0][0], f1 = af[0][1];
-    if (wn == 1) f0 = af[1][0], f1 = af[1][1];
-    else if (wn == 2) f0 = af[2][0], f1 = af[2][1];
-    else if (wn == 3) f0 = af[3][0], f1 = af[3][1];
-    const bf16x8 f[2] = {f0, f1};
-    typedef __bf16 bf16x2_t __attribute__((ext_vector_type(2)));
-    const bf16x2_t ones = {(__bf16)1.0f, (__bf16)1.0f};
-#pragma unroll
-    for (int kh = 0; kh < 2; ++kh)
-#pragma unroll
-      for (int q = 0; q < 4; ++q) {
-        const bf16x2_t pr = {f[kh][2 * q], f[kh][2 * q + 1]};
-        acc_cs = __builtin_amdgcn_fdot2_f32_bf16(pr, ones, acc_cs, false);
-      }
-  };
-
-  stamp(0);
-#pragma unroll
-  for (int t = 0; t < 2; ++t) {
-    issue_part(1);
-    issue_part(2);
-    if constexpr (AK) issue_part(3);
-    advance();
-  }
-  vm_wait<8>();
-  bar();
-  if (wm == 1) bar();
-  if constexpr (SV_G9_PRIO == 1) {
-    if (wm == 1) __builtin_amdgcn_s_setprio(1);
-  }
-
-  int g = 0;
-  for (int it = 0; it < my_tiles; ++it) {
-    const Geo cg = geo(it);
-    f32x4 acc[FM][FN];
-#pragma unroll
-    for (int i = 0; i < FM; ++i)
-#pragma unroll
-      for (int j = 0; j < FN; ++j) acc[i][j] = f32x4{0.f, 0.f, 0.f, 0.f};
-    cs[0] = cs[1] = 0.f;
-    for (int kt = 0; kt < nk; ++kt, ++g) {
-      const char* Ab = smem + a_off<AK>(g);
-      const char* Bb = smem + b_off<AK>(g);
-      bf16x8 af[4][2], bq[2][2][2];
-      auto read_a = [&](int qm) {
-#pragma unroll
-        for (int i = 0; i < 4; ++i)
-#pragma unroll
-          for (int kh = 0; kh < 2; ++kh)
-            af[i][kh] = AK ? frag_k(Ab, wm * 128 + 64 * qm + 16 * i, kh) : frag_m(Ab, wm * 128 + 64 * qm + 16 * i, kh);
-      };
-      auto read_b = [&](int qn) {
-#pragma unroll
-        for (int jj = 0; jj < 2; ++jj)
-#pragma unroll
-          for (int kh = 0; kh < 2; ++kh) {
-            const int j = 2 * qn + jj;
-            if constexpr (BKM) {
-              bq[qn][jj][kh] = frag_k(Bb, wn * 64 + 16 * j, kh);
-            } else if constexpr (P8) {
-              const int p = threadIdx.x & 3;
-              bq[qn][jj][kh] = frag_tr(Bb, wn * 8 + 4 * qn + p, jj, kh);
-            } else {
-              bq[qn][jj][kh] = frag_m(Bb, wn * 64 + 16 * j, kh);
-            }
-          }
-      };
-      auto quad = [&](int qm, int qn) {
-        if constexpr (SV_G9_PRIO == 0) __builtin_amdgcn_s_setprio(1);
-#pragma unroll
-        for (int kh = 0; kh < 2; ++kh)
-#pragma unroll
-          for (int i = 0; i < 4; ++i)
-#pragma unroll
-            for (int jj = 0; jj < 2; ++jj)
-              acc[4 * qm + i][2 * qn + jj] = __builtin_amdgcn_mfma_f32_16x16x32_bf16(
-                  bq[qn][jj][kh], af[i][kh], acc[4 * qm + i][2 * qn + jj], 0, 0, 0);
-        if constexpr (SV_G9_PRIO == 0) __builtin_amdgcn_s_setprio(0);
-      };
-      read_a(0);
-      read_b(0);
-      if constexpr (LBIAS) {
-        if (kt == 0 && wid < 2) {
-          const float* src = wid == 0 ? e.bias : e.gamma;
-          if (src && (wid == 0 || EPI == SV_EPI_BIAS_GAMMA_RES))
-            dma(rsrc(src, (uint32_t)e.N * 4), (uint32_t)(cg.n0 + (threadIdx.x & 63) * 4) * 4, 0,
-                smem + lds_bytes<AK>() + (it & 1) * 2048 + wid * 1024);
-          SV_VMTAG("bias");
-        }
-      }
-      lgkm0();
-      bar();
-      quad(0, 0);
-      bar();
-      read_b(1);
-      issue_part(1);
-      if (do_cs) colsum_frag(af, cs[0]);
-      if (AK) {
-        if (it > 0 && kt <= 1) SV_VMWAIT(W2E, "p3:2@epi");
-        else SV_VMWAIT(W2, "p3:2");
-      }
-      lgkm0();
-      bar();
-      quad(0, 1);
-      bar();
-      read_a(1);
-      issue_part(2);
-      lgkm0();
-      bar();
-      quad(1, 1);
-      bar();
-      if constexpr (AK) issue_part(3);
-      advance();
-      if (do_cs) colsum_frag(af, cs[1]);
-      if (it > 0 && kt == 0) SV_VMWAIT(W1E, "p1:2@epi p2:2@epi");
-      else SV_VMWAIT(W1, "p1:2 p2:2");
-      lgkm0();
-      bar();
-      quad(1, 0);
-      bar();
-    }
-    if (do_cs) {
-#pragma unroll
-      for (int h = 0; h < 2; ++h) {
-        cs[h] += __shfl_xor(cs[h], 16);
-        cs[h] += __shfl_xor(cs[h], 32);
-        const int m = cg.m0 + wm * 128 + 64 * h + 16 * wn + (threadIdx.x & 15);
-        if ((threadIdx.x & 63) < 16 && m < e.M) reinterpret_cast<float*>(e.C2)[(size_t)cg.split * e.M + m] = cs[h];
-      }
-    }
-    if (LBIAS && nk < 2) {
-      vm_wait<0>();
-      bar();
-    }
-    if constexpr (FOLD) {
-      if (wm == 0) bar();
-    }
-    if constexpr (EPI == SV_EPI_LN_BWD) {
-      if (wm == 0) bar();
-      ln_bwd_epilogue(acc, e, x, fold, cg.m0, cg.n0, tilesN, reinterpret_cast<const float*>(smem + lds_bytes<AK>()),
-                      reinterpret_cast<float*>(smem + lds_bytes<AK>() + 4096), smem);
-      if (wm == 1) bar();
-    } else {
-      epilogue<EPI, P8, AK, FOLD>(acc, e, x, cg.m0 + wm * 128, cg.n0 + wn * 64, cg.split,
-                        LBIAS ? reinterpret_cast<const float*>(smem + lds_bytes<AK>() + (it & 1) * 2048) : nullptr);
-    }
-    SV_VMTAG("epi");
-    if constexpr (FOLD) {
-      vm_wait<0>();
-      bar();
-      static_assert(!AK, "the in-kernel fold is for the weight-gradient layout (N/M-major A)");
-      volatile int* flag = reinterpret_cast<volatile int*>(smem + a_off<AK>(g - 1));
-      const int tile = (cg.m0 / BM) * tilesN + cg.n0 / BN;
-      int* arrive = fold.cnt + 2 * tile;
-      int* depart = arrive + 1;
-      if constexpr (FOLD == kFoldLast) {
-        if (threadIdx.x == 0)
-          *flag = __hip_atomic_fetch_add(arrive, 1, __ATOMIC_RELAXED, __HIP_MEMORY_SCOPE_AGENT) == nsplit - 1;
-        lgkm0();
-        bar();
-        if (*flag) {
-          fold_tile<2>(e, x, fold, cg.m0, cg.n0, nsplit);
-          if (threadIdx.x == 0) __hip_atomic_store(arrive, 0, __ATOMIC_RELAXED, __HIP_MEMORY_SCOPE_AGENT);
-        }
-      } else {
-        if (threadIdx.x == 0) {
-          __hip_atomic_fetch_add(arrive, 1, __ATOMIC_RELAXED, __HIP_MEMORY_SCOPE_AGENT);
-          while (__hip_atomic_load(arrive, __ATOMIC_RELAXED, __HIP_MEMORY_SCOPE_AGENT) < nsplit)
-            __builtin_amdgcn_s_sleep(4);
-        }
-        bar();
-        const int per = (BM + nsplit - 1) / nsplit;
-        fold_tile<2>(e, x, fold, cg.m0, cg.n0, nsplit, cg.split * per, cg.split * per + per);
-        if (threadIdx.x == 0 &&
-            __hip_atomic_fetch_add(depart, 1, __ATOMIC_RELAXED, __HIP_MEMORY_SCOPE_AGENT) == nsplit - 1) {
-          __hip_atomic_store(arrive, 0, __ATOMIC_RELAXED, __HIP_MEMORY_SCOPE_AGENT);
-          __hip_atomic_store(depart, 0, __ATOMIC_RELAXED, __HIP_MEMORY_SCOPE_AGENT);
-        }
-      }
-      bar();
-      if (wm == 1) bar();
-    }
-  }
-  vm_wait<0>();
-  if (wm == 0) bar();
-  stamp(1);
-}
+#define SV_G9_GROUPED 0
+#include "gemm9_kernel.h"
+#undef SV_G9_GROUPED
+#define SV_G9_GROUPED 1
+#include "gemm9_kernel.h"
+#undef SV_G9_GROUPED
 
 template <bool AK, int EPI, int FOLD = kFoldNone>
 constexpr int lds_total() {
@@ -1037,7 +793,61 @@
   }
 }
 
-}
+static bool group_member_ok(const sv_gemm_desc* d, int split) {
+  if (d->compute != SV_BF16 || d->a_dtype != SV_BF16 || d->b_dtype != SV_BF16 || d->a_scale_k) return false;
+  if (d->epilogue != SV_EPI_SLAB || d->c_dtype != SV_BF16 || d->a_kmajor || d->b_kmajor || d->fold_out) return false;
+  if (d->C2 && d->c2_dtype != SV_F32) return false;
+  if (d->M <= 0 || d->N <= 0 || d->K % (split * BK) != 0 || d->N % 8 != 0) return false;
+  const size_t lim = (size_t)1 << 31;
+  const size_t rows = (size_t)ceil_div(d->M, BM) * BM;
+  if (rows * (size_t)d->N * 4 * (size_t)split >= lim) return false;
+  if (((size_t)d->K * d->lda + 4096) * 2 >= lim || ((size_t)d->K * d->ldb + 4096) * 2 >= lim) return false;
+  return true;
+}
+
+static int launch_group(const sv_gemm_desc* descs, int n, hipStream_t s) {
+  if (n < 2 || n > kMaxGroup) return SV_ERR_UNSUPPORTED;
+  const sv_gemm_desc& d0 = descs[0];
+  const int split = d0.split_k < 1 ? 1 : d0.split_k;
+  Group g{};
+  int total = 0;
+  for (int i = 0; i < n; ++i) {
+    const sv_gemm_desc& d = descs[i];
+    if (d.K != d0.K || (d.split_k < 1 ? 1 : d.split_k) != split || d.policy.impl != d0.policy.impl ||
+        d.policy.grid_cap != d0.policy.grid_cap || d.policy.wg_per_cu != d0.policy.wg_per_cu ||
+        d.policy.priority != d0.policy.priority)
+      return SV_ERR_UNSUPPORTED;
+    if (!group_member_ok(&d, split)) return SV_ERR_UNSUPPORTED;
+    GroupProb& q = g.p[i];
+    q.A = reinterpret_cast<const uint16_t*>(d.A);
+    q.B = reinterpret_cast<const uint16_t*>(d.B);
+    q.C = d.C;
+    q.C2 = d.C2;
+    q.lda = d.lda, q.ldb = d.ldb;
+    q.M = d.M, q.N = d.N;
+    q.tilesN = ceil_div(d.N, BN);
+    q.nwg = ceil_div(d.M, BM) * q.tilesN;
+    q.xa = (uint32_t)(((size_t)(d.K - 1) * d.lda + d.M) * 2);
+    q.xb = (uint32_t)(((size_t)(d.K - 1) * d.ldb + d.N) * 2);
+    q.xc = (uint32_t)((size_t)d.M * d.N * 2);
+    total += q.nwg * split;
+    q.end = total;
+  }
+  for (int i = n; i < kMaxGroup; ++i) {
+    g.p[i] = g.p[n - 1];
+    g.p[i].end = total;
+  }
+  g.total = total;
+  constexpr int LDS = lds_total<false, SV_EPI_SLAB>();
+  if (const int rc_ = ensure_lds_attr(reinterpret_cast<const void*>(&gemm9_group_kernel<true>), LDS, s)) return rc_;
+  const int grid = policy_grid(&d0.policy, total, 1, s);
+  gemm9_group_kernel<true><<<grid, THREADS, LDS, s>>>(d0.K / split / BK, split, g);
+  return check_launch("sv_gemm_group(v9)");
+}
+
+}
+
+int launch_gemm9_group(const sv_gemm_desc* descs, int n, hipStream_t s) { return g9::launch_group(descs, n, s); }
 
 #ifdef SV_CLOCK_STAMPS
 extern "C" int sv_diag_clock_stamps(unsigned long long* host, int n) {
diff --git a/spine-vision_amd/csrc/gemm9_kernel.h b/spine-vision_amd/csrc/gemm9_kernel.h
--- /dev/null
+++ b/spine-vision_amd/csrc/gemm9_kernel.h
@@ -0,0 +1,324 @@
+#if !SV_G9_GROUPED
+template <bool AK, bool BKM, int EPI, bool P8, int FOLD = kFoldNone>
+__global__ void __launch_bounds__(THREADS) __attribute__((amdgpu_waves_per_eu(2, 2)))
+gemm9_kernel(const uint16_t* __restrict__ A, int64_t lda, const uint16_t* __restrict__ B, int64_t ldb, int nk, int tilesM,
+             int tilesN, int nsplit, EpiArgs e, Ext x, Fold fold) {
+#else
+template <bool P8>
+__global__ void __launch_bounds__(THREADS) __attribute__((amdgpu_waves_per_eu(2, 2)))
+gemm9_group_kernel(int nk, int nsplit, Group grp) {
+  constexpr bool AK = false, BKM = false;
+  constexpr int EPI = SV_EPI_SLAB, FOLD = kFoldNone;
+  static_assert(P8, "the grouped launch writes bf16 slabs");
+  const uint16_t* A = nullptr;
+  const uint16_t* B = nullptr;
+  int64_t lda = 0, ldb = 0;
+  const int tilesM = 0, tilesN = 0;
+  EpiArgs e{};
+  e.epi = SV_EPI_SLAB, e.c_dtype = SV_BF16, e.c2_dtype = SV_F32;
+  Ext x{};
+  const Fold fold{};
+#endif
+  extern __shared__ __attribute__((aligned(16))) char smem[];
+  const int wid = __builtin_amdgcn_readfirstlane(threadIdx.x >> 6), wm = wid >> 2, wn = wid & 3;
+#if SV_G9_GROUPED
+  const int nwg = 0, total = grp.total;
+#else
+  const int nwg = tilesM * tilesN, total = nwg * nsplit;
+#endif
+  const int my_tiles = (total - (int)blockIdx.x + (int)gridDim.x - 1) / (int)gridDim.x;
+  const int kper = nk * BK;
+
+  auto geo = [&](int it) {
+    const int t = blockIdx.x + it * gridDim.x;
+    const int xcd = t & 7, loc = t >> 3, q8 = total >> 3, r8 = total & 7;
+    const int wgi = (xcd < r8 ? xcd * (q8 + 1) : r8 * (q8 + 1) + (xcd - r8) * q8) + loc;
+#if SV_G9_GROUPED
+    Geo gg;
+    {
+      const int p = (wgi >= grp.p[0].end) + (wgi >= grp.p[1].end) + (wgi >= grp.p[2].end);
+      const int u = wgi - (p ? grp.p[p - 1].end : 0);
+      const int pn = grp.p[p].nwg, ptn = grp.p[p].tilesN;
+      const int split = u / pn, wg = u - split * pn;
+      gg.m0 = (wg / ptn) * BM;
+      gg.n0 = (wg % ptn) * BN;
+      gg.split = split;
+      gg.kbeg = split * kper;
+      gg.p = p;
+    }
+#else
+    const int split = wgi / nwg, wg = wgi - split * nwg;
+    Geo gg;
+    gg.m0 = (wg / tilesN) * BM;
+    gg.n0 = (wg % tilesN) * BN;
+    gg.split = split;
+    gg.kbeg = split * kper;
+#endif
+    return gg;
+  };
+
+#if SV_G9_GROUPED
+  auto ra = rsrc(A, x.a), rb = rsrc(B, x.b);
+#else
+  const auto ra = rsrc(A, x.a), rb = rsrc(B, x.b);
+#endif
+  int l_it = 0, l_kt = 0, l_g = 0;
+  Geo lg = geo(0);
+  uint32_t va = 0, vb = 0;
+  auto set_voffs = [&]() {
+#if SV_G9_GROUPED
+    const GroupProb& q = grp.p[lg.p];
+    lda = q.lda, ldb = q.ldb;
+    ra = rsrc(q.A, q.xa), rb = rsrc(q.B, q.xb);
+#endif
+    va = AK ? vbase_k<false>(lda, lg.m0, wid) : vbase_m(lda, lg.m0, wid);
+    vb = BKM ? vbase_k<P8>(ldb, lg.n0, wid) : vbase_m(ldb, lg.n0, wid);
+  };
+  set_voffs();
+  auto issue_part = [&](int part) {
+    const int k0 = lg.kbeg + l_kt * BK;
+    if (part == 2) {
+      char* bb = smem + b_off<AK>(l_g);
+      const uint32_t so = BKM ? (uint32_t)k0 * 2 : (uint32_t)((int64_t)k0 * ldb * 2);
+      const uint32_t step = (uint32_t)((BKM ? 64 : 16) * ldb * 2);
+#pragma unroll
+      for (int j = 0; j < 4; ++j)
+        dma<EPI == SV_EPI_SLAB ? SV_G9_SLAB_B_CPOL : 0>(rb, vb, so + j * step, bb + (wid + 8 * j) * 1024);
+      SV_VMTAG("p2");
+    } else if constexpr (AK) {
+      char* ab = smem + a_off<AK>(l_g);
+      const int h = part == 1 ? 0 : 1;
+      const uint32_t so = (uint32_t)k0 * 2 + (uint32_t)(64 * h * lda * 2);
+      dma(ra, va, so, ab + (h * 8 + wid) * 1024);
+      dma(ra, va, so + (uint32_t)(128 * lda * 2), ab + (h * 8 + 16 + wid) * 1024);
+      if (part == 1) SV_VMTAG("p1");
+      else SV_VMTAG("p3");
+    } else if (part == 1) {
+      char* ab = smem + a_off<AK>(l_g);
+      const uint32_t so = (uint32_t)((int64_t)k0 * lda * 2), step = (uint32_t)(16 * lda * 2);
+#pragma unroll
+      for (int j = 0; j < 4; ++j) dma(ra, va, so + j * step, ab + (wid + 8 * j) * 1024);
+      SV_VMTAG("p1");
+    }
+  };
+  auto advance = [&]() {
+    ++l_g;
+    if (++l_kt == nk) {
+      if (l_it + 1 < my_tiles) {
+        ++l_it;
+        l_kt = 0;
+        lg = geo(l_it);
+        set_voffs();
+      } else {
+        l_kt = nk - 1;
+      }
+    }
+  };
+
+  constexpr int E = EpiCount<EPI, P8>::E;
+  constexpr bool LBIAS = AK && (EPI == SV_EPI_STORE || EPI == SV_EPI_BIAS_GELU_DUAL || EPI == SV_EPI_BIAS_GELU ||
+                                EPI == SV_EPI_BIAS_GAMMA_RES || EPI == SV_EPI_STORE_STATS || EPI == SV_EPI_LN_BWD);
+  constexpr int W1 = AK ? 10 : 8, W2 = 10;
+  constexpr int W1E = W1 + E > 63 ? 63 : W1 + E, W2E = W2 + E > 63 ? 63 : W2 + E;
+#if SV_G9_GROUPED
+  bool do_cs = false;
+#else
+  const bool do_cs = EPI == SV_EPI_SLAB && !AK && e.C2 != nullptr;
+#endif
+  float cs[2] = {0.f, 0.f};
+  auto colsum_frag = [&](const bf16x8 (&af)[4][2], float& acc_cs) {
+    bf16x8 f0 = af[0][0], f1 = af[0][1];
+    if (wn == 1) f0 = af[1][0], f1 = af[1][1];
+    else if (wn == 2) f0 = af[2][0], f1 = af[2][1];
+    else if (wn == 3) f0 = af[3][0], f1 = af[3][1];
+    const bf16x8 f[2] = {f0, f1};
+    typedef __bf16 bf16x2_t __attribute__((ext_vector_type(2)));
+    const bf16x2_t ones = {(__bf16)1.0f, (__bf16)1.0f};
+#pragma unroll
+    for (int kh = 0; kh < 2; ++kh)
+#pragma unroll
+      for (int q = 0; q < 4; ++q) {
+        const bf16x2_t pr = {f[kh][2 * q], f[kh][2 * q + 1]};
+        acc_cs = __builtin_amdgcn_fdot2_f32_bf16(pr, ones, acc_cs, false);
+      }
+  };
+
+  stamp(0);
+#pragma unroll
+  for (int t = 0; t < 2; ++t) {
+    issue_part(1);
+    issue_part(2);
+    if constexpr (AK) issue_part(3);
+    advance();
+  }
+  vm_wait<8>();
+  bar();
+  if (wm == 1) bar();
+  if constexpr (SV_G9_PRIO == 1) {
+    if (wm == 1) __builtin_amdgcn_s_setprio(1);
+  }
+
+  int g = 0;
+  for (int it = 0; it < my_tiles; ++it) {
+    const Geo cg = geo(it);
+#if SV_G9_GROUPED
+    {
+      const GroupProb& q = grp.p[cg.p];
+      e.M = q.M, e.N = q.N, e.C = q.C, e.C2 = q.C2;
+      do_cs = q.C2 != nullptr;
+    }
+    x.c = grp.p[cg.p].xc;
+#endif
+    f32x4 acc[FM][FN];
+#pragma unroll
+    for (int i = 0; i < FM; ++i)
+#pragma unroll
+      for (int j = 0; j < FN; ++j) acc[i][j] = f32x4{0.f, 0.f, 0.f, 0.f};
+    cs[0] = cs[1] = 0.f;
+    for (int kt = 0; kt < nk; ++kt, ++g) {
+      const char* Ab = smem + a_off<AK>(g);
+      const char* Bb = smem + b_off<AK>(g);
+      bf16x8 af[4][2], bq[2][2][2];
+      auto read_a = [&](int qm) {
+#pragma unroll
+        for (int i = 0; i < 4; ++i)
+#pragma unroll
+          for (int kh = 0; kh < 2; ++kh)
+            af[i][kh] = AK ? frag_k(Ab, wm * 128 + 64 * qm + 16 * i, kh) : frag_m(Ab, wm * 128 + 64 * qm + 16 * i, kh);
+      };
+      auto read_b = [&](int qn) {
+#pragma unroll
+        for (int jj = 0; jj < 2; ++jj)
+#pragma unroll
+          for (int kh = 0; kh < 2; ++kh) {
+            const int j = 2 * qn + jj;
+            if constexpr (BKM) {
+              bq[qn][jj][kh] = frag_k(Bb, wn * 64 + 16 * j, kh);
+            } else if constexpr (P8) {
+              const int p = threadIdx.x & 3;
+              bq[qn][jj][kh] = frag_tr(Bb, wn * 8 + 4 * qn + p, jj, kh);
+            } else {
+              bq[qn][jj][kh] = frag_m(Bb, wn * 64 + 16 * j, kh);
+            }
+          }
+      };
+      auto quad = [&](int qm, int qn) {
+        if constexpr (SV_G9_PRIO == 0) __builtin_amdgcn_s_setprio(1);
+#pragma unroll
+        for (int kh = 0; kh < 2; ++kh)
+#pragma unroll
+          for (int i = 0; i < 4; ++i)
+#pragma unroll
+            for (int jj = 0; jj < 2; ++jj)
+              acc[4 * qm + i][2 * qn + jj] = __builtin_amdgcn_mfma_f32_16x16x32_bf16(
+                  bq[qn][jj][kh], af[i][kh], acc[4 * qm + i][2 * qn + jj], 0, 0, 0);
+        if constexpr (SV_G9_PRIO == 0) __builtin_amdgcn_s_setprio(0);
+      };
+      read_a(0);
+      read_b(0);
+      if constexpr (LBIAS) {
+        if (kt == 0 && wid < 2) {
+          const float* src = wid == 0 ? e.bias : e.gamma;
+          if (src && (wid == 0 || EPI == SV_EPI_BIAS_GAMMA_RES))
+            dma(rsrc(src, (uint32_t)e.N * 4), (uint32_t)(cg.n0 + (threadIdx.x & 63) * 4) * 4, 0,
+                smem + lds_bytes<AK>() + (it & 1) * 2048 + wid * 1024);
+          SV_VMTAG("bias");
+        }
+      }
+      lgkm0();
+      bar();
+      quad(0, 0);
+      bar();
+      read_b(1);
+      issue_part(1);
+      if (do_cs) colsum_frag(af, cs[0]);
+      if (AK) {
+        if (it > 0 && kt <= 1) SV_VMWAIT(W2E, "p3:2@epi");
+        else SV_VMWAIT(W2, "p3:2");
+      }
+      lgkm0();
+      bar();
+      quad(0, 1);
+      bar();
+      read_a(1);
+      issue_part(2);
+      lgkm0();
+      bar();
+      quad(1, 1);
+      bar();
+      if constexpr (AK) issue_part(3);
+      advance();
+      if (do_cs) colsum_frag(af, cs[1]);
+      if (it > 0 && kt == 0) SV_VMWAIT(W1E, "p1:2@epi p2:2@epi");
+      else SV_VMWAIT(W1, "p1:2 p2:2");
+      lgkm0();
+      bar();
+      quad(1, 0);
+      bar();
+    }
+    if (do_cs) {
+#pragma unroll
+      for (int h = 0; h < 2; ++h) {
+        cs[h] += __shfl_xor(cs[h], 16);
+        cs[h] += __shfl_xor(cs[h], 32);
+        const int m = cg.m0 + wm * 128 + 64 * h + 16 * wn + (threadIdx.x & 15);
+        if ((threadIdx.x & 63) < 16 && m < e.M) reinterpret_cast<float*>(e.C2)[(size_t)cg.split * e.M + m] = cs[h];
+      }
+    }
+    if (LBIAS && nk < 2) {
+      vm_wait<0>();
+      bar();
+    }
+    if constexpr (FOLD) {
+      if (wm == 0) bar();
+    }
+    if constexpr (EPI == SV_EPI_LN_BWD) {
+      if (wm == 0) bar();
+      ln_bwd_epilogue(acc, e, x, fold, cg.m0, cg.n0, tilesN, reinterpret_cast<const float*>(smem + lds_bytes<AK>()),
+                      reinterpret_cast<float*>(smem + lds_bytes<AK>() + 4096), smem);
+      if (wm == 1) bar();
+    } else {
+      epilogue<EPI, P8, AK, FOLD>(acc, e, x, cg.m0 + wm * 128, cg.n0 + wn * 64, cg.split,
+                        LBIAS ? reinterpret_cast<const float*>(smem + lds_bytes<AK>() + (it & 1) * 2048) : nullptr);
+    }
+    SV_VMTAG("epi");
+    if constexpr (FOLD) {
+      vm_wait<0>();
+      bar();
+      static_assert(!AK, "the in-kernel fold is for the weight-gradient layout (N/M-major A)");
+      volatile int* flag = reinterpret_cast<volatile int*>(smem + a_off<AK>(g - 1));
+      const int tile = (cg.m0 / BM) * tilesN + cg.n0 / BN;
+      int* arrive = fold.cnt + 2 * tile;
+      int* depart = arrive + 1;
+      if constexpr (FOLD == kFoldLast) {
+        if (threadIdx.x == 0)
+          *flag = __hip_atomic_fetch_add(arrive, 1, __ATOMIC_RELAXED, __HIP_MEMORY_SCOPE_AGENT) == nsplit - 1;
+        lgkm0();
+        bar();
+        if (*flag) {
+          fold_tile<2>(e, x, fold, cg.m0, cg.n0, nsplit);
+          if (threadIdx.x == 0) __hip_atomic_store(arrive, 0, __ATOMIC_RELAXED, __HIP_MEMORY_SCOPE_AGENT);
+        }
+      } else {
+        if (threadIdx.x == 0) {
+          __hip_atomic_fetch_add(arrive, 1, __ATOMIC_RELAXED, __HIP_MEMORY_SCOPE_AGENT);
+          while (__hip_atomic_load(arrive, __ATOMIC_RELAXED, __HIP_MEMORY_SCOPE_AGENT) < nsplit)
+            __builtin_amdgcn_s_sleep(4);
+        }
+        bar();
+        const int per = (BM + nsplit - 1) / nsplit;
+        fold_tile<2>(e, x, fold, cg.m0, cg.n0, nsplit, cg.split * per, cg.split * per + per);
+        if (threadIdx.x == 0 &&
+            __hip_atomic_fetch_add(depart, 1, __ATOMIC_RELAXED, __HIP_MEMORY_SCOPE_AGENT) == nsplit - 1) {
+          __hip_atomic_store(arrive, 0, __ATOMIC_RELAXED, __HIP_MEMORY_SCOPE_AGENT);
+          __hip_atomic_store(depart, 0, __ATOMIC_RELAXED, __HIP_MEMORY_SCOPE_AGENT);
+        }
+      }
+      bar();
+      if (wm == 1) bar();
+    }
+  }
+  vm_wait<0>();
+  if (wm == 0) bar();
+  stamp(1);
+}
diff --git a/spine-vision_amd/csrc/gemm_common.h b/spine-vision_amd/csrc/gemm_common.h
--- a/spine-vision_amd/csrc/gemm_common.h
+++ b/spine-vision_amd/csrc/gemm_common.h
@@ -405,5 +405,6 @@
 int launch_gemm3(const sv_gemm_desc* d, hipStream_t s, const char* cfg = nullptr);
 int launch_gemm8(const sv_gemm_desc* d, hipStream_t s);
 int launch_gemm9(const sv_gemm_desc* d, hipStream_t s);
-
-}
+int launch_gemm9_group(const sv_gemm_desc* descs, int n, hipStream_t s);
+
+}
diff --git a/spine-vision_amd/kernels.py b/spine-vision_amd/kernels.py
--- a/spine-vision_amd/kernels.py
+++ b/spine-vision_amd/kernels.py
@@ -371,10 +371,11 @@
 
 def linear_wgrad(dy2d, x2d, *, out=None, accumulate=False, bias_out=None, bias_accumulate=True,
                  compute_bf16=True, cols=None, defer: list | None = None, policy=None,
-                 wgrad_target: int | None = None) -> torch.Tensor:
+                 wgrad_target: int | None = None, split: int | None = None) -> torch.Tensor:
     M, N = dy2d.shape
     K = x2d.shape[1] if cols is None else cols
-    split = _wgrad_split_for(N, K, M, wgrad_target)
+    if split is None:
+        split = _wgrad_split_for(N, K, M, wgrad_target)
     cs = torch.empty(split * N, device=dy2d.device, dtype=torch.float32) if bias_out is not None else None
     bf16 = (out is not None and _bf16_slabs(N, K, M, split, compute_bf16, policy) and out.is_contiguous()
             and out.numel() == N * K)
@@ -384,9 +385,8 @@
     slab = _wgrad_slabs(dy2d, x2d, K, split, bf16_slabs=bf16, cs=cs, fold=(out, accumulate) if infold else None,
                         compute_bf16=compute_bf16, policy=policy)
     if bf16:
-        _timed_call("fold", 2.0 * split * N * K + 4.0 * N * K * (1 + int(bool(accumulate))), "sv_reduce_partials_bf16",
-                    ptr(slab), split, N * K, ptr(out), 1.0, int(bool(accumulate)))
-    if bf16 or infold:
+        return _linear_wgrad_fold_bf16(slab, cs, split, N, K, out, accumulate, bias_out, bias_accumulate, defer)
+    if infold:
         _colsum_finish(cs, split, bias_out, bias_accumulate, defer)
         return out
     if out is None:
@@ -407,6 +407,13 @@
     return out
 
 
+def _linear_wgrad_fold_bf16(slab, cs, split, N, K, out, accumulate, bias_out, bias_accumulate, defer):
+    _timed_call("fold", 2.0 * split * N * K + 4.0 * N * K * (1 + int(bool(accumulate))), "sv_reduce_partials_bf16",
+                ptr(slab), split, N * K, ptr(out), 1.0, int(bool(accumulate)))
+    _colsum_finish(cs, split, bias_out, bias_accumulate, defer)
+    return out
+
+
 def _colsum_finish(cs, split, bias_out, accumulate, defer) -> None:
     if cs is None:
         return
@@ -417,10 +424,11 @@
 
 
 def layerscale_wgrad(dsrc2d, a2d, w2, gamma, b2, *, dw2, dgamma, db2, compute_bf16=True, policy=None,
-                     wgrad_target: int | None = None):
+                     wgrad_target: int | None = None, split: int | None = None):
     M, C = dsrc2d.shape
     K4 = a2d.shape[1]
-    split = _wgrad_split_for(C, K4, M, wgrad_target)
+    if split is None:
+        split = _wgrad_split_for(C, K4, M, wgrad_target)
     cs = torch.empty(split * C, device=dsrc2d.device, dtype=torch.float32)
     bf16 = _bf16_slabs(C, K4, M, split, compute_bf16, policy)
     G = None if bf16 else torch.empty(C * K4, device=dsrc2d.device, dtype=torch.float32)
@@ -429,14 +437,105 @@
                         compute_bf16=compute_bf16, policy=policy)
     rest = (ptr(cs), split, ptr(w2), ptr(gamma), ptr(b2), ptr(dw2), ptr(dgamma), ptr(db2))
     if bf16:
-        _timed_call("fold", 2.0 * split * C * K4 + 8.0 * C * K4 + 4.0 * (split + 4) * C,
-                    "sv_layerscale_wgrad_reduce_bf16", ptr(slab), *rest, C, K4)
+        _layerscale_fold_bf16(slab, rest, split, C, K4)
     elif infold:
         _timed_call("fold", 4.0 * (3 * C * K4 + (split + 4) * C), "sv_layerscale_wgrad_fold_finish", ptr(G), *rest,
                     C, K4)
     else:
         _timed_call("fold", 4.0 * ((split + 2) * C * K4 + (split + 4) * C), "sv_layerscale_wgrad_reduce", ptr(slab),
                     *rest, None, C, K4)
+
+
+def _layerscale_fold_bf16(slab, rest, split, C, K4) -> None:
+    _timed_call("fold", 2.0 * split * C * K4 + 8.0 * C * K4 + 4.0 * (split + 4) * C,
+                "sv_layerscale_wgrad_reduce_bf16", ptr(slab), *rest, C, K4)
+
+
+def wgrad_group_split(shapes, M: int, *, compute_bf16: bool = True, policy=None, target: int | None = None):
+    shapes = list(shapes)
+    if not 2 <= len(shapes) <= 4 or any(min(N, K) < 128 or max(N, K) < 256 for N, K in shapes):
+        return None
+    tiles = sum(-(-N // 256) * -(-K // 256) for N, K in shapes)
+    long_ = any(2.0 * M * N * K > _WGRAD9_LONG_GFLOP * 1e9 for N, K in shapes)
+    target = 256 if long_ else (target or _WGRAD9_TARGET)
+    ok = [s_ for s_ in range(1, max(2, 2 * target // tiles + 1)) if M % (s_ * 64) == 0 and tiles * s_ <= 256]
+    if not ok:
+        return None
+    split = min(ok, key=lambda s_: (abs(tiles * s_ - target), s_))
+    if not all(_bf16_slabs(N, K, M, split, compute_bf16, policy) for N, K in shapes):
+        return None
+    return split
+
+
+def wgrad_group(probs: list, *, compute_bf16=True, policy=None, wgrad_target: int | None = None,
+                one_launch: bool = True) -> None:
+    def separate(split):
+        for p_ in probs:
+            kw = {k_: v_ for k_, v_ in p_.items() if k_ not in ("dy", "x")}
+            fn = layerscale_wgrad if "gamma" in p_ else linear_wgrad
+            fn(p_["dy"], p_["x"], **kw, compute_bf16=compute_bf16, policy=policy, wgrad_target=wgrad_target, split=split)
+
+    M = probs[0]["dy"].shape[0]
+    shapes = [(p_["dy"].shape[1], p_["x"].shape[1]) for p_ in probs]
+    split = None
+    if all(p_["dy"].shape[0] == M and p_["x"].shape[0] == M and p_["dy"].is_contiguous() and p_["x"].is_contiguous()
+           for p_ in probs) and all("gamma" in p_ or (p_.get("out") is not None and p_["out"].is_contiguous()
+                                                       and p_["out"].numel() == N * K)
+                                    for p_, (N, K) in zip(probs, shapes)):
+        split = wgrad_group_split(shapes, M, compute_bf16=compute_bf16, policy=policy, target=wgrad_target)
+    if split is None or not one_launch:
+        separate(split)
+        return
+    dev = probs[0]["dy"].device
+    descs = (nv.GemmDesc * len(probs))()
+    bufs = []
+    flops = nbytes = 0.0
+    units = 0
+    for d, p_, (N, K) in zip(descs, probs, shapes):
+        dy, x = p_["dy"], p_["x"]
+        _check(dy.dtype == torch.bfloat16 and x.dtype == torch.bfloat16, "wgrad_group: bf16 operands")
+        slab = torch.empty(split * N * K, device=dev, dtype=torch.bfloat16)
+        cs = (torch.empty(split * N, device=dev, dtype=torch.float32)
+              if "gamma" in p_ or p_.get("bias_out") is not None else None)
+        bufs.append((slab, cs))
+        d.M, d.N, d.K = N, K, M
+        d.A, d.a_dtype, d.a_kmajor, d.lda = ptr(dy), SV_BF16, 0, N
+        d.B, d.b_dtype, d.b_kmajor, d.ldb = ptr(x), SV_BF16, 0, K
+        d.epilogue = nv.SV_EPI_SLAB
+        d.C, d.c_dtype, d.ldc = ptr(slab), SV_BF16, K
+        if cs is not None:
+            d.C2, d.c2_dtype = ptr(cs), SV_F32
+        d.split_k = split
+        d.compute = SV_BF16
+        if policy is not None:
+            d.policy = policy
+        flops += 2.0 * M * N * K
+        nbytes += 2.0 * M * (N + K) + 4.0 * N * K + (4.0 * N if cs is not None else 0.0)
+        units += -(-N // 256) * -(-K // 256) * split
+    probes = [p_ for p_ in PROBES if p_.matches(False, False, True, nv.SV_EPI_SLAB)]
+    if probes:
+        ev0, ev1 = torch.cuda.Event(enable_timing=True), torch.cuda.Event(enable_timing=True)
+        ev0.record()
+        call("sv_gemm_group", descs, len(probs))
+        ev1.record()
+        cus = _device_cus(dev)
+        cap = policy.grid_cap if policy is not None and policy.grid_cap > 0 else cus
+        for pr in probes:
+            pr.events.append((ev0, ev1))
+            pr.shares.append(min(units, cap, cus) / cus)
+            pr.flops += flops
+            pr.bytes += nbytes
+            pr.launches += 1
+    else:
+        call("sv_gemm_group", descs, len(probs))
+    for p_, (N, K), (slab, cs) in zip(probs, shapes, bufs):
+        if "gamma" in p_:
+            rest = (ptr(cs), split, ptr(p_["w2"]), ptr(p_["gamma"]), ptr(p_["b2"]), ptr(p_["dw2"]), ptr(p_["dgamma"]),
+                    ptr(p_["db2"]))
+            _layerscale_fold_bf16(slab, rest, split, N, K)
+        else:
+            _linear_wgrad_fold_bf16(slab, cs, split, N, K, p_["out"], p_.get("accumulate", False), p_.get("bias_out"),
+                                    p_.get("bias_accumulate", True), p_.get("defer"))
 
 
 def reduce_into(part: torch.Tensor, nparts: int, out: torch.Tensor, accumulate: bool = True, alpha: float = 1.0):
diff --git a/spine-vision_amd/native.py b/spine-vision_amd/native.py
--- a/spine-vision_amd/native.py
+++ b/spine-vision_amd/native.py
@@ -113,6 +113,7 @@
     "sv_last_error_string": [],
     "sv_build_target": [],
     "sv_gemm": [ctypes.POINTER(GemmDesc), _p],
+    "sv_gemm_group": [ctypes.POINTER(GemmDesc), _i32, _p],
     "sv_stream_create_cu_reserved": [_i32, ctypes.POINTER(_i32), _i32, ctypes.POINTER(_p)],
     "sv_gemm_slab_finish": [_p, _i32, _i32, _i32, _p, _i32, _i64, _i32, _p, _p],
     "sv_gemm_slab_finish_bn_bwd": [_p, _i32, _i32, _i32, _p, _p, ctypes.POINTER(BnRef), _p, _p],
```

Measured after the change: 1166 images/sec, median of 6. +2.3%, better.
